# kondratevakate/mri-epilepsy-diagnosis

Measured on AMD Instinct MI355X. Metric: MRI volumes/sec (fwd+bwd) 3D U-Net @160x192x160, higher is better.
Workload: dtype f32; 1 GPU; unet.UNet(c0=8, 3 enc blocks, BN+PReLU, trilinear) fwd+softmax-Dice+bwd+AdamW, batch 2 x 1x160x192x160 fp32 per GPU (BASELINE configs[1]); global_batch=2, parallelism=dp1, launch=eager

## Files before the change

### include/mri3d.h

```cpp
#ifndef MRI3D_H
#define MRI3D_H

#include <stddef.h>
#include <stdint.h>

#ifdef __cplusplus
extern "C" {
#endif

typedef void* mri3d_stream_t;

enum { MRI3D_OK = 0, MRI3D_EINVAL = -1, MRI3D_ENOTSUP = -2, MRI3D_ELAUNCH = -3, MRI3D_EWORKSPACE = -4 };
enum { MRI3D_F32 = 0, MRI3D_BF16 = 1 };
enum { MRI3D_ACT_NONE = 0, MRI3D_ACT_RELU = 1, MRI3D_ACT_LEAKY = 2, MRI3D_ACT_PRELU = 3 };
enum { MRI3D_UP_NEAREST = 0, MRI3D_UP_TRILINEAR = 1 };
enum { MRI3D_PASS_FWD = 0, MRI3D_PASS_DGRAD = 1, MRI3D_PASS_WGRAD = 2 };

int mri3d_version(void);
const char* mri3d_last_error(void);

typedef struct Mri3dConvGeom {
    int32_t n;
    int32_t di, hi, wi, ci;
    int32_t dout, ho, wo, co;
    int32_t kd, kh, kw;
    int32_t sd, sh, sw;
    int32_t pd, ph, pw;
    int32_t dd, dh, dw;
    int32_t x_ld, y_ld;
    int32_t dtype;
} Mri3dConvGeom;

size_t mri3d_conv3d_workspace_bytes(const Mri3dConvGeom* g, int pass);

int mri3d_conv3d_fwd(const Mri3dConvGeom* g, const void* x, const void* w, const void* bias, void* y,
                     void* workspace, size_t ws_bytes, mri3d_stream_t stream);
int32_t mri3d_conv3d_fwd_stats_blocks(const Mri3dConvGeom* g);
int mri3d_conv3d_fwd_stats(const Mri3dConvGeom* g, const void* x, const void* w, const void* bias, void* y,
                           double* stat_partials, void* workspace, size_t ws_bytes, mri3d_stream_t stream);
int mri3d_conv3d_dgrad(const Mri3dConvGeom* g, const void* dy, const void* w, const void* bias, void* dx,
                       void* workspace, size_t ws_bytes, mri3d_stream_t stream);
int mri3d_conv3d_wgrad(const Mri3dConvGeom* g, const void* x, const void* dy, void* dw, void* dbias,
                       void* workspace, size_t ws_bytes, mri3d_stream_t stream);

int32_t mri3d_conv3d_cat_supported(const Mri3dConvGeom* g, int32_t split, int32_t second_ld, int32_t pass);
int32_t mri3d_conv3d_fwd_cat_stats_blocks(const Mri3dConvGeom* g, int32_t split, int32_t second_ld);
int mri3d_conv3d_fwd_cat(const Mri3dConvGeom* g, const void* x, const void* x2, int32_t split, int32_t x2_ld, const void* w,
                         const void* bias, void* y, double* stat_partials, void* workspace, size_t ws_bytes,
                         mri3d_stream_t stream);
int mri3d_conv3d_dgrad_cat(const Mri3dConvGeom* g, const void* dy, const void* w, void* dx, void* dx2, int32_t split,
                           int32_t dx2_ld, void* workspace, size_t ws_bytes, mri3d_stream_t stream);
int mri3d_conv3d_wgrad_cat(const Mri3dConvGeom* g, const void* x, const void* x2, int32_t split, int32_t x2_ld, const void* dy,
                           void* dw, void* dbias, void* workspace, size_t ws_bytes, mri3d_stream_t stream);

int32_t mri3d_conv3d_march_supported(const Mri3dConvGeom* g, int32_t pass);
int32_t mri3d_conv3d_march_stats_blocks(const Mri3dConvGeom* g);
int mri3d_conv3d_fwd_march(const Mri3dConvGeom* g, const void* x, const void* x2, int32_t split, int32_t x2_ld, const void* w,
                           const void* bias, void* y, double* stat_partials, void* workspace, size_t ws_bytes,
                           mri3d_stream_t stream);
int mri3d_conv3d_dgrad_march(const Mri3dConvGeom* g, const void* dy, const void* w, void* dx, void* dx2, int32_t split,
                             int32_t dx2_ld, void* workspace, size_t ws_bytes, mri3d_stream_t stream);

int32_t mri3d_upconv3d_supported(const Mri3dConvGeom* g, int32_t scale);
size_t mri3d_upconv3d_workspace_bytes(const Mri3dConvGeom* g, int32_t scale);
int mri3d_upconv3d_fwd(const Mri3dConvGeom* g, int32_t scale, const void* x, const float* w, const float* bias, void* y,
                       mri3d_stream_t stream);
int mri3d_upconv3d_dgrad(const Mri3dConvGeom* g, int32_t scale, const void* dy, const float* w, void* dx, mri3d_stream_t stream);
int mri3d_upconv3d_wgrad(const Mri3dConvGeom* g, int32_t scale, const void* x, const void* dy, float* dw, float* dbias,
                         void* workspace, size_t ws_bytes, mri3d_stream_t stream);

int32_t mri3d_convpair_supported(const Mri3dConvGeom* first, const Mri3dConvGeom* second);
size_t mri3d_convpair_workspace_bytes(const Mri3dConvGeom* first, const Mri3dConvGeom* second);
int mri3d_convpair_wgrad_first(const Mri3dConvGeom* first, const Mri3dConvGeom* second, const void* x, const void* dy2, const float* w2,
                               float* dw1, float* dbias1, void* workspace, size_t ws_bytes, mri3d_stream_t stream);

typedef struct Mri3dNormGeom {
    int32_t n;
    int64_t vox;
    int32_t c;
    int32_t x_ld;
    int32_t y_ld;
    int32_t instance;
    int32_t act;
    int32_t alpha_n;
    float slope;
    float eps;
    int32_t group_c;
    int32_t dtype;
} Mri3dNormGeom;

size_t mri3d_norm_workspace_bytes(const Mri3dNormGeom* g);

int mri3d_norm_stats(const Mri3dNormGeom* g, const void* x, float* mean, float* invstd,
                     float* running_mean, float* running_var, float momentum,
                     void* workspace, size_t ws_bytes, mri3d_stream_t stream);
int mri3d_norm_stats_from_partials(const Mri3dNormGeom* g, const double* partials, int32_t nblk, const float* shift,
                                   float* mean, float* invstd, float* running_mean, float* running_var, float momentum,
                                   mri3d_stream_t stream);
int mri3d_norm_act_fwd(const Mri3dNormGeom* g, const void* x, const float* mean, const float* invstd,
                       const float* gamma, const float* beta, const float* alpha, void* y,
                       mri3d_stream_t stream);
int mri3d_norm_act_bwd(const Mri3dNormGeom* g, int training, const void* x, const void* dy,
                       const float* mean, const float* invstd, const float* gamma, const float* beta,
                       const float* alpha, void* dx, float* dgamma, float* dbeta, float* dalpha,
                       void* workspace, size_t ws_bytes, mri3d_stream_t stream);

typedef struct Mri3dPoolGeom {
    int32_t n, di, hi, wi, dout, ho, wo, c;
    int32_t kd, kh, kw, sd, sh, sw, pd, ph, pw;
    int32_t x_ld, y_ld;
    int32_t dtype;
} Mri3dPoolGeom;
int mri3d_maxpool3d_fwd(const Mri3dPoolGeom* g, const void* x, void* y, uint8_t* idx, mri3d_stream_t stream);
int mri3d_maxpool3d_bwd(const Mri3dPoolGeom* g, const void* dy, const uint8_t* idx, void* dx, mri3d_stream_t stream);
int mri3d_maxpool3d_bwd_add(const Mri3dPoolGeom* g, const void* dy, const uint8_t* idx, const void* addend,
                            int32_t addend_ld, void* dx, mri3d_stream_t stream);

typedef struct Mri3dUpGeom {
    int32_t n, di, hi, wi, dout, ho, wo, c;
    int32_t x_ld, y_ld;
    int32_t mode;
    int32_t align_corners;
    float rd, rh, rw;
    int32_t dtype;
} Mri3dUpGeom;
size_t mri3d_upsample3d_workspace_bytes(const Mri3dUpGeom* g);
int mri3d_upsample3d_fwd(const Mri3dUpGeom* g, const void* x, void* y, mri3d_stream_t stream);
int mri3d_upsample3d_bwd(const Mri3dUpGeom* g, const void* dy, void* dx, void* workspace, size_t ws_bytes,
                         mri3d_stream_t stream);

typedef struct Mri3dDiceGeom {
    int32_t n;
    int64_t vox;
    int32_t c, ct;
    int32_t x_ld, t_ld;
    float eps;
    int32_t dtype;
} Mri3dDiceGeom;
size_t mri3d_softmax_dice_workspace_bytes(const Mri3dDiceGeom* g);
int mri3d_softmax_dice_fwd(const Mri3dDiceGeom* g, const void* logits, const void* target, float* loss,
                           float* stats, void* workspace, size_t ws_bytes, mri3d_stream_t stream);
int mri3d_softmax_dice_bwd(const Mri3dDiceGeom* g, const void* logits, const void* target, const float* stats,
                           const float* dloss, void* dlogits, mri3d_stream_t stream);

int mri3d_argmax_u8(const void* logits, uint8_t* out, int64_t nvox, int32_t c, int32_t ld, int32_t dtype,
                    mri3d_stream_t stream);

size_t mri3d_mask_overlap_workspace_bytes(void);
int mri3d_mask_overlap(const uint8_t* pred, const uint8_t* gt, int64_t nvox, int64_t* counts, void* workspace,
                       size_t ws_bytes, mri3d_stream_t stream);

size_t mri3d_order_stats_workspace_bytes(void);
int mri3d_order_stats_f32(const float* x, int64_t n, const int64_t* ranks, int32_t nranks, float* out, void* workspace,
                          size_t ws_bytes, mri3d_stream_t stream);
int mri3d_piecewise_linear_f32(const float* x, float* y, int64_t n, const double* edges, const double* slope,
                               const double* intercept, int32_t nseg, mri3d_stream_t stream);
size_t mri3d_znorm_workspace_bytes(void);
int mri3d_znorm_mean_mask_f32(const float* x, float* y, int64_t n, double* stats, void* workspace, size_t ws_bytes,
                              mri3d_stream_t stream);
int mri3d_crop_or_pad_f32(const float* x, float* y, int32_t outer, int32_t di, int32_t hi, int32_t wi, int32_t dout,
                          int32_t ho, int32_t wo, float fill, mri3d_stream_t stream);

size_t mri3d_surface_distance_workspace_bytes(int32_t d, int32_t h, int32_t w);
int mri3d_surface_distance(const uint8_t* gt, const uint8_t* pred, int32_t d, int32_t h, int32_t w,
                           const double* area_table, double* sums, void* workspace, size_t ws_bytes, mri3d_stream_t stream);
int mri3d_surface_elements(const uint8_t* gt, const uint8_t* pred, int32_t d, int32_t h, int32_t w, int32_t* d2_gt,
                           uint8_t* code_gt, int32_t* d2_pred, uint8_t* code_pred, int64_t capacity, uint64_t* counts,
                           void* workspace, size_t ws_bytes, mri3d_stream_t stream);

int mri3d_extract_patches(const void* volumes, int32_t elem_bytes, int32_t nvol, int32_t d, int32_t h, int32_t w,
                          const int32_t* loc_host, int32_t npatch, int32_t pd, int32_t ph, int32_t pw, void* out,
                          mri3d_stream_t stream);
int mri3d_aggregate_patches_u8(const uint8_t* patches, const int32_t* loc_host, int32_t npatch, int32_t pd, int32_t ph,
                               int32_t pw, int32_t bd, int32_t bh, int32_t bw, uint8_t* out, int32_t nvol, int32_t d,
                               int32_t h, int32_t w, mri3d_stream_t stream);
int mri3d_aggregate_patches_argmax(const void* logits, int32_t c, int32_t ld, int32_t dtype, const int32_t* loc_host,
                                   int32_t npatch, int32_t pd, int32_t ph, int32_t pw, int32_t bd, int32_t bh, int32_t bw,
                                   uint8_t* out, int32_t nvol, int32_t d, int32_t h, int32_t w, mri3d_stream_t stream);

int mri3d_copy_channels(const void* src, void* dst, int64_t nvox, int32_t c, int32_t src_ld, int32_t dst_ld,
                        int32_t dtype, mri3d_stream_t stream);
int mri3d_add_channels(const void* a, const void* b, void* dst, int64_t nvox, int32_t c, int32_t a_ld,
                       int32_t b_ld, int32_t dst_ld, int32_t dtype, mri3d_stream_t stream);
int mri3d_convert_channels(const void* src, int32_t src_dtype, void* dst, int32_t dst_dtype, int64_t nvox, int32_t c,
                           int32_t src_ld, int32_t dst_ld, mri3d_stream_t stream);

int mri3d_adam_step(float* p, const float* g, float* m, float* v, int64_t n, float lr, float beta1, float beta2,
                    float eps, float weight_decay, int32_t step, float grad_scale, int32_t decoupled,
                    mri3d_stream_t stream);

#ifdef __cplusplus
}
#endif
#endif
```

### mri_epilepsy_diagnosis_amd/_lib.py

```python
import ctypes
import os
from ctypes import POINTER, Structure, c_char_p, c_float, c_int32, c_int64, c_size_t, c_uint8, c_void_p

_HERE = os.path.dirname(os.path.abspath(__file__))
LIB_PATH = os.path.join(_HERE, "libmri3d_hip.so")

F32, BF16 = 0, 1
ACT_NONE, ACT_RELU, ACT_LEAKY, ACT_PRELU = 0, 1, 2, 3
UP_NEAREST, UP_TRILINEAR = 0, 1
PASS_FWD, PASS_DGRAD, PASS_WGRAD = 0, 1, 2


class ConvGeom(Structure):
    _fields_ = [(n, c_int32) for n in (
        "n", "di", "hi", "wi", "ci", "dout", "ho", "wo", "co", "kd", "kh", "kw", "sd", "sh", "sw",
        "pd", "ph", "pw", "dd", "dh", "dw", "x_ld", "y_ld", "dtype")]


class NormGeom(Structure):
    _fields_ = [("n", c_int32), ("vox", c_int64), ("c", c_int32), ("x_ld", c_int32), ("y_ld", c_int32),
                ("instance", c_int32), ("act", c_int32), ("alpha_n", c_int32), ("slope", c_float),
                ("eps", c_float), ("group_c", c_int32), ("dtype", c_int32)]


class PoolGeom(Structure):
    _fields_ = [(n, c_int32) for n in (
        "n", "di", "hi", "wi", "dout", "ho", "wo", "c", "kd", "kh", "kw", "sd", "sh", "sw", "pd", "ph", "pw",
        "x_ld", "y_ld", "dtype")]


class UpGeom(Structure):
    _fields_ = [(n, c_int32) for n in ("n", "di", "hi", "wi", "dout", "ho", "wo", "c", "x_ld", "y_ld", "mode",
                                       "align_corners")] + \
               [("rd", c_float), ("rh", c_float), ("rw", c_float), ("dtype", c_int32)]


class DiceGeom(Structure):
    _fields_ = [("n", c_int32), ("vox", c_int64), ("c", c_int32), ("ct", c_int32), ("x_ld", c_int32),
                ("t_ld", c_int32), ("eps", c_float), ("dtype", c_int32)]


_P = c_void_p
_FP = c_void_p

SIGNATURES = {
    "mri3d_version": (c_int32, []),
    "mri3d_last_error": (c_char_p, []),
    "mri3d_conv3d_workspace_bytes": (c_size_t, [POINTER(ConvGeom), c_int32]),
    "mri3d_conv3d_fwd": (c_int32, [POINTER(ConvGeom), _P, _P, _P, _P, _P, c_size_t, _P]),
    "mri3d_conv3d_fwd_stats_blocks": (c_int32, [POINTER(ConvGeom)]),
    "mri3d_conv3d_fwd_stats": (c_int32, [POINTER(ConvGeom), _P, _P, _P, _P, _P, _P, c_size_t, _P]),
    "mri3d_conv3d_dgrad": (c_int32, [POINTER(ConvGeom), _P, _P, _P, _P, _P, c_size_t, _P]),
    "mri3d_conv3d_wgrad": (c_int32, [POINTER(ConvGeom), _P, _P, _P, _P, _P, c_size_t, _P]),
    "mri3d_conv3d_cat_supported": (c_int32, [POINTER(ConvGeom), c_int32, c_int32, c_int32]),
    "mri3d_conv3d_fwd_cat_stats_blocks": (c_int32, [POINTER(ConvGeom), c_int32, c_int32]),
    "mri3d_conv3d_fwd_cat": (c_int32, [POINTER(ConvGeom), _P, _P, c_int32, c_int32, _P, _P, _P, _P, _P, c_size_t, _P]),
    "mri3d_conv3d_dgrad_cat": (c_int32, [POINTER(ConvGeom), _P, _P, _P, _P, c_int32, c_int32, _P, c_size_t, _P]),
    "mri3d_conv3d_wgrad_cat": (c_int32, [POINTER(ConvGeom), _P, _P, c_int32, c_int32, _P, _P, _P, _P, c_size_t, _P]),
    "mri3d_conv3d_march_supported": (c_int32, [POINTER(ConvGeom), c_int32]),
    "mri3d_conv3d_march_stats_blocks": (c_int32, [POINTER(ConvGeom)]),
    "mri3d_conv3d_fwd_march": (c_int32, [POINTER(ConvGeom), _P, _P, c_int32, c_int32, _P, _P, _P, _P, _P, c_size_t, _P]),
    "mri3d_conv3d_dgrad_march": (c_int32, [POINTER(ConvGeom), _P, _P, _P, _P, c_int32, c_int32, _P, c_size_t, _P]),
    "mri3d_upconv3d_supported": (c_int32, [POINTER(ConvGeom), c_int32]),
    "mri3d_upconv3d_workspace_bytes": (c_size_t, [POINTER(ConvGeom), c_int32]),
    "mri3d_upconv3d_fwd": (c_int32, [POINTER(ConvGeom), c_int32, _P, _FP, _FP, _P, _P]),
    "mri3d_upconv3d_dgrad": (c_int32, [POINTER(ConvGeom), c_int32, _P, _FP, _P, _P]),
    "mri3d_upconv3d_wgrad": (c_int32, [POINTER(ConvGeom), c_int32, _P, _P, _FP, _FP, _P, c_size_t, _P]),
    "mri3d_convpair_supported": (c_int32, [POINTER(ConvGeom), POINTER(ConvGeom)]),
    "mri3d_convpair_workspace_bytes": (c_size_t, [POINTER(ConvGeom), POINTER(ConvGeom)]),
    "mri3d_convpair_wgrad_first": (c_int32, [POINTER(ConvGeom), POINTER(ConvGeom), _P, _P, _FP, _FP, _FP, _P, c_size_t, _P]),
    "mri3d_norm_workspace_bytes": (c_size_t, [POINTER(NormGeom)]),
    "mri3d_norm_stats": (c_int32, [POINTER(NormGeom), _P, _FP, _FP, _FP, _FP, c_float, _P, c_size_t, _P]),
    "mri3d_norm_stats_from_partials": (c_int32, [POINTER(NormGeom), _P, c_int32, _FP, _FP, _FP, _FP, _FP, c_float, _P]),
    "mri3d_norm_act_fwd": (c_int32, [POINTER(NormGeom), _P, _FP, _FP, _FP, _FP, _FP, _P, _P]),
    "mri3d_norm_act_bwd": (c_int32, [POINTER(NormGeom), c_int32, _P, _P, _FP, _FP, _FP, _FP, _FP, _P, _FP, _FP, _FP,
                                     _P, c_size_t, _P]),
    "mri3d_maxpool3d_fwd": (c_int32, [POINTER(PoolGeom), _P, _P, _P, _P]),
    "mri3d_maxpool3d_bwd": (c_int32, [POINTER(PoolGeom), _P, _P, _P, _P]),
    "mri3d_maxpool3d_bwd_add": (c_int32, [POINTER(PoolGeom), _P, _P, _P, c_int32, _P, _P]),
    "mri3d_upsample3d_workspace_bytes": (c_size_t, [POINTER(UpGeom)]),
    "mri3d_upsample3d_fwd": (c_int32, [POINTER(UpGeom), _P, _P, _P]),
    "mri3d_upsample3d_bwd": (c_int32, [POINTER(UpGeom), _P, _P, _P, c_size_t, _P]),
    "mri3d_softmax_dice_workspace_bytes": (c_size_t, [POINTER(DiceGeom)]),
    "mri3d_softmax_dice_fwd": (c_int32, [POINTER(DiceGeom), _P, _P, _FP, _FP, _P, c_size_t, _P]),
    "mri3d_softmax_dice_bwd": (c_int32, [POINTER(DiceGeom), _P, _P, _FP, _FP, _P, _P]),
    "mri3d_argmax_u8": (c_int32, [_P, _P, c_int64, c_int32, c_int32, c_int32, _P]),
    "mri3d_mask_overlap_workspace_bytes": (c_size_t, []),
    "mri3d_mask_overlap": (c_int32, [_P, _P, c_int64, _P, _P, c_size_t, _P]),
    "mri3d_order_stats_workspace_bytes": (c_size_t, []),
    "mri3d_order_stats_f32": (c_int32, [_P, c_int64, _P, c_int32, _P, _P, c_size_t, _P]),
    "mri3d_piecewise_linear_f32": (c_int32, [_P, _P, c_int64, _P, _P, _P, c_int32, _P]),
    "mri3d_znorm_workspace_bytes": (c_size_t, []),
    "mri3d_znorm_mean_mask_f32": (c_int32, [_P, _P, c_int64, _P, _P, c_size_t, _P]),
    "mri3d_crop_or_pad_f32": (c_int32, [_P, _P, c_int32, c_int32, c_int32, c_int32, c_int32, c_int32, c_int32, c_float, _P]),
    "mri3d_surface_distance_workspace_bytes": (c_size_t, [c_int32, c_int32, c_int32]),
    "mri3d_surface_distance": (c_int32, [_P, _P, c_int32, c_int32, c_int32, _P, _P, _P, c_size_t, _P]),
    "mri3d_surface_elements": (c_int32, [_P, _P, c_int32, c_int32, c_int32, _P, _P, _P, _P, c_int64, _P, _P, c_size_t, _P]),
    "mri3d_extract_patches": (c_int32, [_P, c_int32, c_int32, c_int32, c_int32, c_int32, _P, c_int32, c_int32, c_int32,
                                        c_int32, _P, _P]),
    "mri3d_aggregate_patches_u8": (c_int32, [_P, _P, c_int32, c_int32, c_int32, c_int32, c_int32, c_int32, c_int32, _P,
                                             c_int32, c_int32, c_int32, c_int32, _P]),
    "mri3d_aggregate_patches_argmax": (c_int32, [_P, c_int32, c_int32, c_int32, _P, c_int32, c_int32, c_int32, c_int32,
                                                 c_int32, c_int32, c_int32, _P, c_int32, c_int32, c_int32, c_int32, _P]),
    "mri3d_copy_channels": (c_int32, [_P, _P, c_int64, c_int32, c_int32, c_int32, c_int32, _P]),
    "mri3d_add_channels": (c_int32, [_P, _P, _P, c_int64, c_int32, c_int32, c_int32, c_int32, c_int32, _P]),
    "mri3d_convert_channels": (c_int32, [_P, c_int32, _P, c_int32, c_int64, c_int32, c_int32, c_int32, _P]),
    "mri3d_adam_step": (c_int32, [_FP, _FP, _FP, _FP, c_int64, c_float, c_float, c_float, c_float, c_float, c_int32,
                                  c_float, c_int32, _P]),
}

_lib = None


class Mri3dError(RuntimeError):
    pass


def lib():
    global _lib
    if _lib is None:
        import torch
        if not os.path.exists(LIB_PATH):
            raise Mri3dError(
                "libmri3d_hip.so not found at %s — run `python -m mri_epilepsy_diagnosis_amd.build` "
                "(or __graft_entry__.build()).  There is no PyTorch fallback for device tensors." % LIB_PATH)
        h = ctypes.CDLL(LIB_PATH)
        for name, (res, args) in SIGNATURES.items():
            fn = getattr(h, name)
            fn.restype = res
            fn.argtypes = args
        _lib = h
    return _lib


def check(rc, what=""):
    if rc != 0:
        msg = lib().mri3d_last_error()
        raise Mri3dError("%s failed (rc=%d): %s" % (what, rc, msg.decode() if msg else "?"))
```

### mri_epilepsy_diagnosis_amd/csrc/api.hip

```cpp
#include "common.h"
#include <string.h>

namespace mri3d {

static thread_local char g_err[512] = "";

void set_error(const char* fmt, ...) {
    va_list ap;
    va_start(ap, fmt);
    vsnprintf(g_err, sizeof(g_err), fmt, ap);
    va_end(ap);
}

size_t conv_generic_workspace_bytes(const Mri3dConvGeom& g, int pass);
int conv_generic_fwd(const Mri3dConvGeom& g, const void* x, const float* w, const float* bias, void* y, void* ws,
                     size_t ws_bytes, hipStream_t s);
int conv_generic_dgrad(const Mri3dConvGeom& g, const void* dy, const float* w, const float* bias, void* dx, void* ws,
                       size_t ws_bytes, hipStream_t s);
int conv_generic_wgrad(const Mri3dConvGeom& g, const void* x, const void* dy, float* dw, float* dbias, void* ws,
                       size_t ws_bytes, hipStream_t s);
bool conv_mfma_supported(const Mri3dConvGeom& g, int pass);
size_t conv_mfma_workspace_bytes(const Mri3dConvGeom& g, int pass);
int conv_mfma_fwd(const Mri3dConvGeom& g, const void* x, const float* w, const float* bias, void* y, void* ws,
                  size_t ws_bytes, hipStream_t s);
int conv_mfma_dgrad(const Mri3dConvGeom& g, const void* dy, const float* w, const float* bias, void* dx, void* ws,
                    size_t ws_bytes, hipStream_t s);
int conv_mfma_wgrad(const Mri3dConvGeom& g, const void* x, const void* dy, float* dw, float* dbias, void* ws,
                    size_t ws_bytes, hipStream_t s);
int conv_mfma_fwd_stat_blocks(const Mri3dConvGeom& g, int split = 0, int second_ld = 0);
bool conv_mfma_cat_supported(const Mri3dConvGeom& g, int split, int second_ld, int pass);
int conv_mfma_fwd_cat(const Mri3dConvGeom& g, const void* x, const void* x2, int split, int x2_ld, const float* w, const float* bias,
                      void* y, double* stat_part, void* ws, size_t ws_bytes, hipStream_t s);
int conv_mfma_dgrad_cat(const Mri3dConvGeom& g, const void* dy, const float* w, void* dx, void* dx2, int split, int dx2_ld, void* ws,
                        size_t ws_bytes, hipStream_t s);
int conv_mfma_wgrad_cat(const Mri3dConvGeom& g, const void* x, const void* x2, int split, int x2_ld, const void* dy, float* dw,
                        float* dbias, void* ws, size_t ws_bytes, hipStream_t s);
int conv_mfma_fwd_stats(const Mri3dConvGeom& g, const void* x, const float* w, const float* bias, void* y, double* stat_part,
                        void* ws, size_t ws_bytes, hipStream_t s);

bool conv_march_takes(const Mri3dConvGeom& g, bool dgrad, bool stats, bool force);
int conv_march_stat_blocks(const Mri3dConvGeom& g, bool force);
int conv_march_run(const Mri3dConvGeom& g, bool dgrad, bool force, const void* in_v, const float* w, const float* bias, void* out_v,
                   void* ws, size_t ws_bytes, hipStream_t s, double* stat_part, const void* second, int split, int second_ld);

bool conv_pointwise_supported(const Mri3dConvGeom& g, int pass);
size_t conv_pointwise_workspace_bytes(const Mri3dConvGeom& g, int pass);
int conv_pointwise_fwd(const Mri3dConvGeom& g, const void* x, const float* w, const float* bias, void* y, hipStream_t s);
int conv_pointwise_dgrad(const Mri3dConvGeom& g, const void* dy, const float* w, const float* bias, void* dx,
                         hipStream_t s);
int conv_pointwise_wgrad(const Mri3dConvGeom& g, const void* x, const void* dy, float* dw, float* dbias, void* ws,
                         size_t ws_bytes, hipStream_t s);


static int conv_check(const Mri3dConvGeom* g, const char* who, int first_ci = -1) {
    MRI3D_REQUIRE(g != nullptr, MRI3D_EINVAL, "%s: null geometry", who);
    MRI3D_REQUIRE(g->dtype == MRI3D_F32 || g->dtype == MRI3D_BF16, MRI3D_ENOTSUP, "%s: unknown dtype %d", who, g->dtype);
    MRI3D_REQUIRE(g->n > 0 && g->di > 0 && g->hi > 0 && g->wi > 0 && g->ci > 0 && g->dout > 0 && g->ho > 0 && g->wo > 0 &&
                      g->co > 0,
                  MRI3D_EINVAL, "%s: empty tensor", who);
    MRI3D_REQUIRE(g->kd > 0 && g->kh > 0 && g->kw > 0 && g->sd > 0 && g->sh > 0 && g->sw > 0 && g->dd > 0 && g->dh > 0 &&
                      g->dw > 0 && g->pd >= 0 && g->ph >= 0 && g->pw >= 0,
                  MRI3D_EINVAL, "%s: bad kernel/stride/padding/dilation", who);
    MRI3D_REQUIRE(g->x_ld >= (first_ci >= 0 ? first_ci : g->ci) && g->y_ld >= g->co, MRI3D_EINVAL, "%s: pitch smaller than channel count", who);
    int ed = (g->di + 2 * g->pd - g->dd * (g->kd - 1) - 1) / g->sd + 1;
    int eh = (g->hi + 2 * g->ph - g->dh * (g->kh - 1) - 1) / g->sh + 1;
    int ew = (g->wi + 2 * g->pw - g->dw * (g->kw - 1) - 1) / g->sw + 1;
    MRI3D_REQUIRE(ed == g->dout && eh == g->ho && ew == g->wo, MRI3D_EINVAL,
                  "%s: output dims (%d,%d,%d) do not match conv arithmetic (%d,%d,%d)", who, g->dout, g->ho, g->wo, ed, eh,
                  ew);
    return MRI3D_OK;
}

}

using namespace mri3d;

extern "C" int mri3d_version(void) { return 100; }
extern "C" const char* mri3d_last_error(void) { return g_err; }

extern "C" size_t mri3d_conv3d_workspace_bytes(const Mri3dConvGeom* g, int pass) {
    if (!g) return 0;
    size_t a = conv_generic_workspace_bytes(*g, pass);
    size_t b = conv_mfma_supported(*g, pass) ? conv_mfma_workspace_bytes(*g, pass) : 0;
    size_t c = conv_pointwise_supported(*g, pass) ? conv_pointwise_workspace_bytes(*g, pass) : 0;
    a = a > b ? a : b;
    return align_up(a > c ? a : c, 256);
}

extern "C" int mri3d_conv3d_fwd(const Mri3dConvGeom* g, const void* x, const void* w, const void* bias, void* y,
                                void* workspace, size_t ws_bytes, mri3d_stream_t stream) {
    int rc = conv_check(g, "conv3d_fwd");
    if (rc) return rc;
    MRI3D_REQUIRE(x && w && y, MRI3D_EINVAL, "conv3d_fwd: null pointer");
    hipStream_t s = static_cast<hipStream_t>(stream);
    if (conv_mfma_supported(*g, MRI3D_PASS_FWD) && aligned16(x, y, workspace))
        return conv_mfma_fwd(*g, x, (const float*)w, (const float*)bias, y, workspace, ws_bytes, s);
    if (conv_pointwise_supported(*g, MRI3D_PASS_FWD) && aligned_vec4(g->dtype, x))
        return conv_pointwise_fwd(*g, x, (const float*)w, (const float*)bias, y, s);
    return conv_generic_fwd(*g, x, (const float*)w, (const float*)bias, y, workspace, ws_bytes, s);
}

extern "C" int32_t mri3d_conv3d_fwd_stats_blocks(const Mri3dConvGeom* g) {
    if (!g || conv_check(g, "conv3d_fwd_stats_blocks") != MRI3D_OK) return 0;
    return conv_mfma_supported(*g, MRI3D_PASS_FWD) ? conv_mfma_fwd_stat_blocks(*g) : 0;
}

extern "C" int mri3d_conv3d_fwd_stats(const Mri3dConvGeom* g, const void* x, const void* w, const void* bias, void* y,
                                      double* stat_partials, void* workspace, size_t ws_bytes, mri3d_stream_t stream) {
    int rc = conv_check(g, "conv3d_fwd_stats");
    if (rc) return rc;
    MRI3D_REQUIRE(x && w && y && stat_partials, MRI3D_EINVAL, "conv3d_fwd_stats: null pointer");
    MRI3D_REQUIRE(conv_mfma_supported(*g, MRI3D_PASS_FWD) && conv_mfma_fwd_stat_blocks(*g) > 0 && aligned16(x, y, workspace),
                  MRI3D_ENOTSUP, "conv3d_fwd_stats: geometry not served by the MFMA forward kernel (query mri3d_conv3d_fwd_stats_blocks)");
    return conv_mfma_fwd_stats(*g, x, (const float*)w, (const float*)bias, y, stat_partials, workspace, ws_bytes,
                               static_cast<hipStream_t>(stream));
}

extern "C" int mri3d_conv3d_dgrad(const Mri3dConvGeom* g, const void* dy, const void* w, const void* bias, void* dx,
                                  void* workspace, size_t ws_bytes, mri3d_stream_t stream) {
    int rc = conv_check(g, "conv3d_dgrad");
    if (rc) return rc;
    MRI3D_REQUIRE(dy && w && dx, MRI3D_EINVAL, "conv3d_dgrad: null pointer");
    hipStream_t s = static_cast<hipStream_t>(stream);
    if (conv_pointwise_supported(*g, MRI3D_PASS_DGRAD) && aligned_vec4(g->dtype, dx))
        return conv_pointwise_dgrad(*g, dy, (const float*)w, (const float*)bias, dx, s);
    if (conv_mfma_supported(*g, MRI3D_PASS_DGRAD) && aligned16(dy, dx, workspace))
        return conv_mfma_dgrad(*g, dy, (const float*)w, (const float*)bias, dx, workspace, ws_bytes, s);
    return conv_generic_dgrad(*g, dy, (const float*)w, (const float*)bias, dx, workspace, ws_bytes, s);
}

extern "C" int32_t mri3d_conv3d_cat_supported(const Mri3dConvGeom* g, int32_t split, int32_t second_ld, int32_t pass) {
    if (!g || split <= 0 || conv_check(g, "conv3d_cat_supported", split) != MRI3D_OK) return 0;
    return conv_mfma_cat_supported(*g, split, second_ld, pass) ? 1 : 0;
}

extern "C" int32_t mri3d_conv3d_fwd_cat_stats_blocks(const Mri3dConvGeom* g, int32_t split, int32_t second_ld) {
    if (!g || split <= 0 || conv_check(g, "conv3d_fwd_cat_stats_blocks", split) != MRI3D_OK) return 0;
    return conv_mfma_cat_supported(*g, split, second_ld, MRI3D_PASS_FWD) ? conv_mfma_fwd_stat_blocks(*g, split, second_ld) : 0;
}

extern "C" int mri3d_conv3d_fwd_cat(const Mri3dConvGeom* g, const void* x, const void* x2, int32_t split, int32_t x2_ld,
                                    const void* w, const void* bias, void* y, double* stat_partials, void* workspace,
                                    size_t ws_bytes, mri3d_stream_t stream) {
    int rc = conv_check(g, "conv3d_fwd_cat", split);
    if (rc) return rc;
    MRI3D_REQUIRE(x && x2 && w && y, MRI3D_EINVAL, "conv3d_fwd_cat: null pointer");
    MRI3D_REQUIRE(conv_mfma_cat_supported(*g, split, x2_ld, MRI3D_PASS_FWD) && aligned16(x, y, workspace) && aligned16(x2),
                  MRI3D_ENOTSUP, "conv3d_fwd_cat: geometry / alignment not served (query mri3d_conv3d_cat_supported)");
    MRI3D_REQUIRE(stat_partials == nullptr || conv_mfma_fwd_stat_blocks(*g, split, x2_ld) > 0, MRI3D_ENOTSUP,
                  "conv3d_fwd_cat: no fused statistics for this geometry (query mri3d_conv3d_fwd_cat_stats_blocks)");
    return conv_mfma_fwd_cat(*g, x, x2, split, x2_ld, (const float*)w, (const float*)bias, y, stat_partials, workspace, ws_bytes,
                             static_cast<hipStream_t>(stream));
}

extern "C" int mri3d_conv3d_dgrad_cat(const Mri3dConvGeom* g, const void* dy, const void* w, void* dx, void* dx2, int32_t split,
                                      int32_t dx2_ld, void* workspace, size_t ws_bytes, mri3d_stream_t stream) {
    int rc = conv_check(g, "conv3d_dgrad_cat", split);
    if (rc) return rc;
    MRI3D_REQUIRE(dy && w && dx && dx2, MRI3D_EINVAL, "conv3d_dgrad_cat: null pointer");
    MRI3D_REQUIRE(conv_mfma_cat_supported(*g, split, dx2_ld, MRI3D_PASS_DGRAD) && aligned16(dy, dx, workspace) && aligned16(dx2),
                  MRI3D_ENOTSUP, "conv3d_dgrad_cat: geometry / alignment not served (query mri3d_conv3d_cat_supported)");
    return conv_mfma_dgrad_cat(*g, dy, (const float*)w, dx, dx2, split, dx2_ld, workspace, ws_bytes, static_cast<hipStream_t>(stream));
}

extern "C" int mri3d_conv3d_wgrad_cat(const Mri3dConvGeom* g, const void* x, const void* x2, int32_t split, int32_t x2_ld,
                                      const void* dy, void* dw, void* dbias, void* workspace, size_t ws_bytes,
                                      mri3d_stream_t stream) {
    int rc = conv_check(g, "conv3d_wgrad_cat", split);
    if (rc) return rc;
    MRI3D_REQUIRE(x && x2 && dy && dw, MRI3D_EINVAL, "conv3d_wgrad_cat: null pointer");
    MRI3D_REQUIRE(conv_mfma_cat_supported(*g, split, x2_ld, MRI3D_PASS_WGRAD) && aligned16(x, dy, workspace) && aligned16(x2),
                  MRI3D_ENOTSUP, "conv3d_wgrad_cat: geometry / alignment not served (query mri3d_conv3d_cat_supported)");
    return conv_mfma_wgrad_cat(*g, x, x2, split, x2_ld, dy, (float*)dw, (float*)dbias, workspace, ws_bytes,
                               static_cast<hipStream_t>(stream));
}

extern "C" int32_t mri3d_conv3d_march_supported(const Mri3dConvGeom* g, int32_t pass) {
    if (!g || (pass != MRI3D_PASS_FWD && pass != MRI3D_PASS_DGRAD) || conv_check(g, "conv3d_march_supported") != MRI3D_OK) return 0;
    return conv_march_takes(*g, pass == MRI3D_PASS_DGRAD, false, true) ? 1 : 0;
}

extern "C" int32_t mri3d_conv3d_march_stats_blocks(const Mri3dConvGeom* g) {
    if (!g || conv_check(g, "conv3d_march_stats_blocks") != MRI3D_OK) return 0;
    return conv_march_stat_blocks(*g, true);
}

extern "C" int mri3d_conv3d_fwd_march(const Mri3dConvGeom* g, const void* x, const void* x2, int32_t split, int32_t x2_ld,
                                      const void* w, const void* bias, void* y, double* stat_partials, void* workspace,
                                      size_t ws_bytes, mri3d_stream_t stream) {
    int rc = conv_check(g, "conv3d_fwd_march", x2 ? split : -1);
    if (rc) return rc;
    MRI3D_REQUIRE(x && w && y, MRI3D_EINVAL, "conv3d_fwd_march: null pointer");
    MRI3D_REQUIRE(x2 == nullptr || (split > 0 && split < g->ci && x2_ld >= g->ci - split), MRI3D_EINVAL, "conv3d_fwd_march: bad split");
    return conv_march_run(*g, false, true, x, (const float*)w, (const float*)bias, y, workspace, ws_bytes,
                          static_cast<hipStream_t>(stream), stat_partials, x2, split, x2_ld);
}

extern "C" int mri3d_conv3d_dgrad_march(const Mri3dConvGeom* g, const void* dy, const void* w, void* dx, void* dx2, int32_t split,
                                        int32_t dx2_ld, void* workspace, size_t ws_bytes, mri3d_stream_t stream) {
    int rc = conv_check(g, "conv3d_dgrad_march", dx2 ? split : -1);
    if (rc) return rc;
    MRI3D_REQUIRE(dy && w && dx, MRI3D_EINVAL, "conv3d_dgrad_march: null pointer");
    MRI3D_REQUIRE(dx2 == nullptr || (split > 0 && split < g->ci && dx2_ld >= g->ci - split), MRI3D_EINVAL, "conv3d_dgrad_march: bad split");
    return conv_march_run(*g, true, true, dy, (const float*)w, nullptr, dx, workspace, ws_bytes, static_cast<hipStream_t>(stream),
                          nullptr, dx2, split, dx2_ld);
}

extern "C" int mri3d_conv3d_wgrad(const Mri3dConvGeom* g, const void* x, const void* dy, void* dw, void* dbias,
                                  void* workspace, size_t ws_bytes, mri3d_stream_t stream) {
    int rc = conv_check(g, "conv3d_wgrad");
    if (rc) return rc;
    MRI3D_REQUIRE(x && dy && dw, MRI3D_EINVAL, "conv3d_wgrad: null pointer");
    hipStream_t s = static_cast<hipStream_t>(stream);
    if (conv_pointwise_supported(*g, MRI3D_PASS_WGRAD) && aligned_vec4(g->dtype, x))
        return conv_pointwise_wgrad(*g, x, dy, (float*)dw, (float*)dbias, workspace, ws_bytes, s);
    if (conv_mfma_supported(*g, MRI3D_PASS_WGRAD) && aligned16(x, dy, workspace))
        return conv_mfma_wgrad(*g, x, dy, (float*)dw, (float*)dbias, workspace, ws_bytes, s);
    return conv_generic_wgrad(*g, x, dy, (float*)dw, (float*)dbias, workspace, ws_bytes, s);
}
```

### mri_epilepsy_diagnosis_amd/csrc/common.h

```cpp
#pragma once
#include <hip/hip_runtime.h>
#include <stdint.h>
#include <stdio.h>
#include <stdarg.h>
#include <stdlib.h>
#include "../../include/mri3d.h"

namespace mri3d {

void set_error(const char* fmt, ...);

inline int check_launch(const char* what) {
    hipError_t e = hipGetLastError();
    if (e != hipSuccess) {
        set_error("%s: launch failed: %s", what, hipGetErrorString(e));
        return MRI3D_ELAUNCH;
    }
    return MRI3D_OK;
}

#define MRI3D_REQUIRE(cond, code, ...)      \
    do {                                    \
        if (!(cond)) {                      \
            ::mri3d::set_error(__VA_ARGS__); \
            return (code);                  \
        }                                   \
    } while (0)

#ifdef MRI3D_TUNING
inline int tuning_knob(const char* name, int dflt) {
    const char* v = getenv(name);
    return v ? atoi(v) : dflt;
}
#else
constexpr int tuning_knob(const char*, int dflt) { return dflt; }
#endif

inline int64_t cdiv64(int64_t a, int64_t b) { return (a + b - 1) / b; }
inline int cdiv(int a, int b) { return (a + b - 1) / b; }
inline size_t align_up(size_t x, size_t a) { return (x + a - 1) / a * a; }

constexpr int kMaxStreamBlocks = 2048;

inline int stream_grid(int64_t work_items, int per_block) {
    int64_t b = cdiv64(work_items, per_block);
    if (b > kMaxStreamBlocks) b = kMaxStreamBlocks;
    if (b < 1) b = 1;
    return (int)b;
}

typedef __bf16 bf16_t;
typedef __attribute__((ext_vector_type(4))) __bf16 bf16x4_t;
typedef __attribute__((ext_vector_type(8))) __bf16 bf16x8_t;

template <typename T> __device__ __forceinline__ float ldf(const T* p) { return (float)*p; }
template <typename T> __device__ __forceinline__ void stf(T* p, float v) { *p = (T)v; }

__device__ __forceinline__ float4 ldf4(const float* p) { return *reinterpret_cast<const float4*>(p); }
__device__ __forceinline__ float4 ldf4(const bf16_t* p) {
    const bf16x4_t v = *reinterpret_cast<const bf16x4_t*>(p);
    return make_float4((float)v[0], (float)v[1], (float)v[2], (float)v[3]);
}
__device__ __forceinline__ void stf4(float* p, float4 v) { *reinterpret_cast<float4*>(p) = v; }
__device__ __forceinline__ void stf4(bf16_t* p, float4 v) {
    bf16x4_t o;
    o[0] = (bf16_t)v.x, o[1] = (bf16_t)v.y, o[2] = (bf16_t)v.z, o[3] = (bf16_t)v.w;
    *reinterpret_cast<bf16x4_t*>(p) = o;
}

inline size_t dtype_size(int dtype) { return dtype == MRI3D_BF16 ? 2 : 4; }
inline bool aligned_vec4(int dtype, const void* a, const void* b = nullptr, const void* c = nullptr) {
    const uintptr_t m = dtype == MRI3D_BF16 ? 7 : 15;
    return ((reinterpret_cast<uintptr_t>(a) | reinterpret_cast<uintptr_t>(b) | reinterpret_cast<uintptr_t>(c)) & m) == 0;
}

inline bool aligned16(const void* a, const void* b = nullptr, const void* c = nullptr) {
    return ((reinterpret_cast<uintptr_t>(a) | reinterpret_cast<uintptr_t>(b) | reinterpret_cast<uintptr_t>(c)) & 15) == 0;
}

#define MRI3D_DISPATCH_DTYPE(dtype, T, ...)  \
    do {                                     \
        if ((dtype) == MRI3D_BF16) {         \
            using T = ::mri3d::bf16_t;       \
            __VA_ARGS__                      \
        } else {                             \
            using T = float;                 \
            __VA_ARGS__                      \
        }                                    \
    } while (0)

__device__ __forceinline__ float wave_sum(float v) {
#pragma unroll
    for (int off = 32; off > 0; off >>= 1) v += __shfl_xor(v, off, 64);
    return v;
}

__device__ __forceinline__ double wave_sum_d(double v) {
#pragma unroll
    for (int off = 32; off > 0; off >>= 1) v += __shfl_xor(v, off, 64);
    return v;
}

__device__ __forceinline__ float apply_act(float v, int act, float slope) {
    if (act == MRI3D_ACT_RELU) return v > 0.f ? v : 0.f;
    if (act == MRI3D_ACT_LEAKY || act == MRI3D_ACT_PRELU) return v > 0.f ? v : v * slope;
    return v;
}

}
```

### mri_epilepsy_diagnosis_amd/csrc/conv_pointwise.hip

```cpp
#include "common.h"

namespace mri3d {

template <typename T, int CO>
__global__ void __launch_bounds__(256)
pw_dgrad_kernel(const T* __restrict__ dy, const float* __restrict__ w, const float* __restrict__ bias,
                T* __restrict__ dx, int64_t nvox, int Ci, int Co, int x_ld, int y_ld) {
    const int QC = Ci >> 2;
    const int q = threadIdx.x % QC, vl = threadIdx.x / QC, VL = 256 / QC;
    float4 wq[CO];
#pragma unroll
    for (int co = 0; co < CO; ++co) {
        const float* wr = w + (size_t)(co < Co ? co : 0) * Ci + 4 * q;
        wq[co] = co < Co ? make_float4(wr[0], wr[1], wr[2], wr[3]) : make_float4(0.f, 0.f, 0.f, 0.f);
    }
    const float4 b4 = bias ? make_float4(bias[4 * q], bias[4 * q + 1], bias[4 * q + 2], bias[4 * q + 3])
                           : make_float4(0.f, 0.f, 0.f, 0.f);
    constexpr int U = 4;
    const int64_t stride = (int64_t)gridDim.x * VL;
    for (int64_t v0 = (int64_t)blockIdx.x * VL + vl; v0 < nvox; v0 += stride * U) {
        float gv[U][CO];
#pragma unroll
        for (int u = 0; u < U; ++u) {
            const int64_t v = v0 + u * stride;
#pragma unroll
            for (int co = 0; co < CO; ++co) gv[u][co] = (v < nvox && co < Co) ? ldf(dy + v * y_ld + co) : 0.f;
        }
#pragma unroll
        for (int u = 0; u < U; ++u) {
            const int64_t v = v0 + u * stride;
            if (v >= nvox) break;
            float4 acc = b4;
#pragma unroll
            for (int co = 0; co < CO; ++co) {
                acc.x = fmaf(gv[u][co], wq[co].x, acc.x);
                acc.y = fmaf(gv[u][co], wq[co].y, acc.y);
                acc.z = fmaf(gv[u][co], wq[co].z, acc.z);
                acc.w = fmaf(gv[u][co], wq[co].w, acc.w);
            }
            stf4(dx + v * x_ld + 4 * q, acc);
        }
    }
}

template <typename T, int CO>
__global__ void __launch_bounds__(256)
pw_fwd_kernel(const T* __restrict__ x, const float* __restrict__ w, const float* __restrict__ bias, T* __restrict__ y,
              int64_t nvox, int Ci, int Co, int x_ld, int y_ld) {
    const int QC = Ci >> 2;
    const int q = threadIdx.x % QC, vl = threadIdx.x / QC, VL = 256 / QC;
    float4 wq[CO];
    float bq[CO];
#pragma unroll
    for (int co = 0; co < CO; ++co) {
        const float* wr = w + (size_t)(co < Co ? co : 0) * Ci + 4 * q;
        wq[co] = co < Co ? make_float4(wr[0], wr[1], wr[2], wr[3]) : make_float4(0.f, 0.f, 0.f, 0.f);
        bq[co] = (bias != nullptr && co < Co) ? bias[co] : 0.f;
    }
    constexpr int U = 4;
    const int64_t stride = (int64_t)gridDim.x * VL;
    for (int64_t v0 = (int64_t)blockIdx.x * VL + vl; v0 < nvox; v0 += stride * U) {
        float4 xv[U];
#pragma unroll
        for (int u = 0; u < U; ++u) {
            const int64_t v = v0 + u * stride;
            xv[u] = ldf4(x + (v < nvox ? v : nvox - 1) * x_ld + 4 * q);
        }
#pragma unroll
        for (int u = 0; u < U; ++u) {
            const int64_t v = v0 + u * stride;
            float acc[CO];
#pragma unroll
            for (int co = 0; co < CO; ++co) {
                float a = xv[u].x * wq[co].x;
                a = fmaf(xv[u].y, wq[co].y, a);
                a = fmaf(xv[u].z, wq[co].z, a);
                a = fmaf(xv[u].w, wq[co].w, a);
                for (int d = 1; d < QC; d <<= 1) a += __shfl_xor(a, d, 64);
                acc[co] = a + bq[co];
            }
            if (q == 0 && v < nvox) {
                T* yp = y + v * y_ld;
#pragma unroll
                for (int co = 0; co < CO; ++co)
                    if (co < Co) stf(yp + co, acc[co]);
            }
        }
    }
}

constexpr int kPwMaxBlocks = 1024;

template <typename T, int CO, int VX, bool DYV>
__global__ void __launch_bounds__(256)
pw_wgrad_kernel(const T* __restrict__ x, const T* __restrict__ dy, double* __restrict__ part,
                double* __restrict__ bias_part, int64_t nvox, int Ci, int Co, int x_ld, int y_ld) {
    extern __shared__ __attribute__((aligned(16))) double redd[];
    const int QC = Ci / VX;
    const int VL = 256 / QC;
    const int tid = threadIdx.x;
    const int q = tid % QC, vl = tid / QC;
    double acc[VX][CO], bsum[CO];
#pragma unroll
    for (int c = 0; c < CO; ++c) {
        bsum[c] = 0.0;
#pragma unroll
        for (int a = 0; a < VX; ++a) acc[a][c] = 0.0;
    }
    if (vl < VL) {
        constexpr int U = 4;
        const int64_t stride = (int64_t)gridDim.x * VL;
        for (int64_t v0 = (int64_t)blockIdx.x * VL + vl; v0 < nvox; v0 += stride * U) {
            float xv[U][VX];
            float gv[U][CO];
#pragma unroll
            for (int u = 0; u < U; ++u) {
                const int64_t v = v0 + u * stride;
                const bool ok = v < nvox;
                const T* xp = x + (ok ? v : 0) * x_ld + VX * q;
                if constexpr (VX == 8) {
                    const bf16x8_t t = *reinterpret_cast<const bf16x8_t*>(xp);
#pragma unroll
                    for (int a = 0; a < 8; ++a) xv[u][a] = ok ? (float)t[a] : 0.f;
                } else {
                    const float4 t = ldf4(xp);
                    xv[u][0] = ok ? t.x : 0.f, xv[u][1] = ok ? t.y : 0.f, xv[u][2] = ok ? t.z : 0.f, xv[u][3] = ok ? t.w : 0.f;
                }
                const T* gp = dy + (ok ? v : 0) * y_ld;
                if constexpr (DYV) {
                    typedef T tvec __attribute__((ext_vector_type(CO)));
                    const tvec t = *reinterpret_cast<const tvec*>(gp);
#pragma unroll
                    for (int c = 0; c < CO; ++c) gv[u][c] = ok ? (float)t[c] : 0.f;
                } else {
#pragma unroll
                    for (int c = 0; c < CO; ++c) gv[u][c] = (ok && c < Co) ? ldf(gp + c) : 0.f;
                }
            }
#pragma unroll
            for (int u = 0; u < U; ++u) {
#pragma unroll
                for (int c = 0; c < CO; ++c) {
#pragma unroll
                    for (int a = 0; a < VX; ++a) acc[a][c] += (double)(xv[u][a] * gv[u][c]);
                    if (q == 0) bsum[c] += (double)gv[u][c];
                }
            }
        }
    }
    constexpr int S = (VX + 1) * CO;
#pragma unroll
    for (int c = 0; c < CO; ++c) {
#pragma unroll
        for (int a = 0; a < VX; ++a) redd[tid * S + a * CO + c] = acc[a][c];
        redd[tid * S + VX * CO + c] = bsum[c];
    }
    __syncthreads();
    for (int o = tid; o < QC * VX * CO; o += 256) {
        const int c = o % CO, a = (o / CO) % VX, qq = o / (VX * CO);
        double s = 0.0;
        for (int l = 0; l < VL; ++l) s += redd[(l * QC + qq) * S + a * CO + c];
        if (c < Co) part[((size_t)blockIdx.x * Co + c) * Ci + VX * qq + a] = s;
    }
    if (bias_part != nullptr && tid < Co) {
        double s = 0.0;
        for (int l = 0; l < VL; ++l) s += redd[(l * QC) * S + VX * CO + tid];
        bias_part[(size_t)blockIdx.x * Co + tid] = s;
    }
}

__global__ void __launch_bounds__(256)
pw_wgrad_reduce_kernel(const double* __restrict__ part, const double* __restrict__ bias_part, float* __restrict__ dw,
                       float* __restrict__ dbias, int nb, int Ci, int Co) {
    __shared__ double red[256];
    const int el = threadIdx.x >> 5, ql = threadIdx.x & 31;
    const int nw = Co * Ci, ntot = nw + (dbias != nullptr ? Co : 0);
    const int i = blockIdx.x * 8 + el;
    double s = 0.0;
    if (i < nw)
        for (int b = ql; b < nb; b += 32) s += part[(size_t)b * nw + i];
    else if (i < ntot)
        for (int b = ql; b < nb; b += 32) s += bias_part[(size_t)b * Co + (i - nw)];
    red[threadIdx.x] = s;
    __syncthreads();
    if (ql == 0 && i < ntot) {
        double t = 0.0;
        for (int k = 0; k < 32; ++k) t += red[el * 32 + k];
        if (i < nw) dw[i] = (float)t;
        else dbias[i - nw] = (float)t;
    }
}

static bool is_pointwise(const Mri3dConvGeom& g) {
    return g.kd == 1 && g.kh == 1 && g.kw == 1 && g.sd == 1 && g.sh == 1 && g.sw == 1 && g.pd == 0 && g.ph == 0 &&
           g.pw == 0;
}

static int pw_blocks(const Mri3dConvGeom& g) {
    const int64_t nvox = (int64_t)g.n * g.dout * g.ho * g.wo;
    const int VL = 256 / (g.ci >> 2);
    int64_t want = cdiv64(nvox, (int64_t)VL * 16);
    return (int)std::max<int64_t>(1, std::min<int64_t>(want, kPwMaxBlocks));
}

bool conv_pointwise_supported(const Mri3dConvGeom& g, int pass) {
    if (!is_pointwise(g) || g.ci % 4 != 0 || g.x_ld % 4 != 0 || g.ci > 256) return false;
    if (pass == MRI3D_PASS_DGRAD) return g.co <= 8 && 256 % (g.ci >> 2) == 0;
    if (pass == MRI3D_PASS_FWD) {
        const int qc = g.ci >> 2;
        return g.co <= 4 && qc >= 1 && qc <= 16 && (qc & (qc - 1)) == 0;
    }
    if (pass == MRI3D_PASS_WGRAD) return g.co <= 8 && g.ci <= 64;
    return false;
}

size_t conv_pointwise_workspace_bytes(const Mri3dConvGeom& g, int pass) {
    if (pass != MRI3D_PASS_WGRAD) return 0;
    return (size_t)pw_blocks(g) * (g.co * g.ci + g.co) * sizeof(double);
}

int conv_pointwise_dgrad(const Mri3dConvGeom& g, const void* dy, const float* w, const float* bias, void* dx,
                         hipStream_t s) {
    MRI3D_REQUIRE(aligned_vec4(g.dtype, dx), MRI3D_EINVAL, "conv3d_dgrad(pointwise): dx must be aligned to 4 elements");
    const int64_t nvox = (int64_t)g.n * g.di * g.hi * g.wi;
    const int VL = 256 / (g.ci >> 2);
    const unsigned grid = (unsigned)std::max<int64_t>(1, std::min<int64_t>(cdiv64(nvox, (int64_t)VL * 4), 2048));
#define PW_DGRAD(CO)                                                                                                   \
    hipLaunchKernelGGL((pw_dgrad_kernel<T, CO>), dim3(grid), dim3(256), 0, s, (const T*)dy, w, bias, (T*)dx, nvox, g.ci, g.co, \
                       g.x_ld, g.y_ld)
    MRI3D_DISPATCH_DTYPE(g.dtype, T, {
        if (g.co <= 2) PW_DGRAD(2);
        else if (g.co <= 4) PW_DGRAD(4);
        else PW_DGRAD(8);
    });
#undef PW_DGRAD
    return check_launch("conv3d_dgrad(pointwise)");
}

int conv_pointwise_fwd(const Mri3dConvGeom& g, const void* x, const float* w, const float* bias, void* y, hipStream_t s) {
    MRI3D_REQUIRE(aligned_vec4(g.dtype, x), MRI3D_EINVAL, "conv3d_fwd(pointwise): x must be aligned to 4 elements");
    const int64_t nvox = (int64_t)g.n * g.di * g.hi * g.wi;
    const int VL = 256 / (g.ci >> 2);
    const unsigned grid = (unsigned)std::max<int64_t>(1, std::min<int64_t>(cdiv64(nvox, (int64_t)VL * 4), 2048));
#define PW_FWD(CO)                                                                                                     \
    hipLaunchKernelGGL((pw_fwd_kernel<T, CO>), dim3(grid), dim3(256), 0, s, (const T*)x, w, bias, (T*)y, nvox, g.ci, g.co,     \
                       g.x_ld, g.y_ld)
    MRI3D_DISPATCH_DTYPE(g.dtype, T, {
        if (g.co <= 2) PW_FWD(2);
        else PW_FWD(4);
    });
#undef PW_FWD
    return check_launch("conv3d_fwd(pointwise)");
}

int conv_pointwise_wgrad(const Mri3dConvGeom& g, const void* x, const void* dy, float* dw, float* dbias, void* ws,
                         size_t ws_bytes, hipStream_t s) {
    const int nb = pw_blocks(g);
    const size_t need = conv_pointwise_workspace_bytes(g, MRI3D_PASS_WGRAD);
    MRI3D_REQUIRE(ws && ws_bytes >= need, MRI3D_EWORKSPACE, "conv3d_wgrad(pointwise): workspace %zu < %zu", ws_bytes, need);
    MRI3D_REQUIRE(aligned_vec4(g.dtype, x) && (reinterpret_cast<uintptr_t>(ws) & 7) == 0, MRI3D_EINVAL,
                  "conv3d_wgrad(pointwise): x must be aligned to 4 elements");
    double* part = static_cast<double*>(ws);
    double* bias_part = dbias ? part + (size_t)nb * g.co * g.ci : nullptr;
    const int64_t nvox = (int64_t)g.n * g.di * g.hi * g.wi;
    const int CO = g.co <= 2 ? 2 : (g.co <= 4 ? 4 : 8);
    const bool v8 = g.dtype == MRI3D_BF16 && g.ci % 8 == 0 && g.x_ld % 8 == 0 && 256 % (g.ci / 8) == 0 && aligned16(x) && CO <= 4;
    const bool dyv = g.co == CO && g.y_ld == CO && (reinterpret_cast<uintptr_t>(dy) & 15) == 0;
    const size_t smem = (size_t)256 * ((v8 ? 8 : 4) + 1) * CO * sizeof(double);
#define PW_WGRAD(CO_, VX_, DV_)                                                                                        \
    do {                                                                                                               \
        auto kern = pw_wgrad_kernel<T, CO_, VX_, DV_>;                                                                 \
        static const hipError_t attr_ = hipFuncSetAttribute(reinterpret_cast<const void*>(kern),                       \
                                                            hipFuncAttributeMaxDynamicSharedMemorySize, 256 * 9 * 8 * 8); \
        (void)attr_;                                                                                                   \
        hipLaunchKernelGGL(kern, dim3(nb), dim3(256), smem, s, (const T*)x, (const T*)dy, part, bias_part, nvox, g.ci,  \
                           g.co, g.x_ld, g.y_ld);                                                                      \
    } while (0)
#define PW_WGRAD_CO(CO_)                                                                                               \
    do {                                                                                                               \
        if constexpr (sizeof(T) == 2 && CO_ <= 4) {                                                                    \
            if (v8 && dyv) { PW_WGRAD(CO_, 8, true); break; }                                                          \
            if (v8) { PW_WGRAD(CO_, 8, false); break; }                                                                \
        }                                                                                                              \
        if (dyv) PW_WGRAD(CO_, 4, true);                                                                               \
        else PW_WGRAD(CO_, 4, false);                                                                                  \
    } while (0)
    MRI3D_DISPATCH_DTYPE(g.dtype, T, {
        if (CO == 2) PW_WGRAD_CO(2);
        else if (CO == 4) PW_WGRAD_CO(4);
        else PW_WGRAD_CO(8);
    });
#undef PW_WGRAD_CO
#undef PW_WGRAD
    hipLaunchKernelGGL(pw_wgrad_reduce_kernel, dim3(cdiv(g.co * g.ci + g.co, 8)), dim3(256), 0, s, part, bias_part, dw, dbias,
                       nb, g.ci, g.co);
    return check_launch("conv3d_wgrad(pointwise)");
}

}
```

### mri_epilepsy_diagnosis_amd/csrc/norm.hip

```cpp
#include "common.h"

namespace mri3d {

struct NormPlan {
    int vec;
    int CL;
    int VT;
    int cy;
    int nblk;
    int groups;
    int64_t gvox;
};

constexpr int kNormMaxBlocks = 1024;
constexpr int kFinQL = 64;

static NormPlan norm_plan(const Mri3dNormGeom& g, bool al, bool al16 = false) {
    NormPlan p;
    p.vec = (g.c % 4 == 0 && g.x_ld % 4 == 0 && g.y_ld % 4 == 0 && al) ? 4 : 1;
    if (p.vec == 4 && g.dtype == MRI3D_BF16 && g.c % 8 == 0 && g.x_ld % 8 == 0 && g.y_ld % 8 == 0 && al16) p.vec = 8;
    int lanes = g.c / p.vec;
    p.CL = lanes < 256 ? lanes : 256;
    p.cy = cdiv(lanes, p.CL);
    p.VT = 256 / p.CL;
// ... 483 lines not shown
extern "C" size_t mri3d_norm_workspace_bytes(const Mri3dNormGeom* g) {
    if (!g) return 0;
    return norm_workspace_floats(*g) * sizeof(float);
}

static int norm_check(const Mri3dNormGeom* g, const char* who) {
    MRI3D_REQUIRE(g != nullptr, MRI3D_EINVAL, "%s: null geometry", who);
    MRI3D_REQUIRE(g->dtype == MRI3D_F32 || g->dtype == MRI3D_BF16, MRI3D_ENOTSUP, "%s: unknown dtype %d", who, g->dtype);
    MRI3D_REQUIRE(g->n > 0 && g->vox > 0 && g->c > 0 && g->x_ld >= g->c && g->y_ld >= g->c, MRI3D_EINVAL,
                  "%s: bad geometry n=%d vox=%lld c=%d x_ld=%d y_ld=%d", who, g->n, (long long)g->vox, g->c, g->x_ld,
                  g->y_ld);
    MRI3D_REQUIRE(g->act != MRI3D_ACT_PRELU || g->alpha_n == 1 || g->alpha_n == g->c, MRI3D_EINVAL,
                  "%s: PReLU alpha_n=%d must be 1 or C=%d", who, g->alpha_n, g->c);
    MRI3D_REQUIRE(g->group_c == 0 || (g->group_c > 0 && g->instance && g->c % g->group_c == 0), MRI3D_EINVAL,
                  "%s: group_c=%d needs instance mode and must divide C=%d", who, g->group_c, g->c);
    return MRI3D_OK;
}

extern "C" int mri3d_norm_stats(const Mri3dNormGeom* g, const void* x, float* mean, float* invstd, float* running_mean,
                                float* running_var, float momentum, void* workspace, size_t ws_bytes,
                                mri3d_stream_t stream) {
    int rc = norm_check(g, "norm_stats");
    if (rc) return rc;
    MRI3D_REQUIRE(x && mean && invstd, MRI3D_EINVAL, "norm_stats: null pointer");
    MRI3D_REQUIRE(workspace && ws_bytes >= mri3d_norm_workspace_bytes(g), MRI3D_EWORKSPACE,
                  "norm_stats: workspace %zu < %zu", ws_bytes, mri3d_norm_workspace_bytes(g));
    hipStream_t s = static_cast<hipStream_t>(stream);
    Mri3dNormGeom gg = *g;
    gg.y_ld = gg.x_ld;
    NormPlan p = norm_plan(gg, aligned_vec4(g->dtype, x));
    double* part = static_cast<double*>(workspace);
    dim3 grid(p.nblk, p.cy, p.groups);
    const int tot = p.groups * g->c;
    MRI3D_DISPATCH_DTYPE(g->dtype, T, {
        const T* xf = static_cast<const T*>(x);
        if (p.vec == 4)
            hipLaunchKernelGGL((norm_stats_kernel<T, 4>), grid, dim3(256), 0, s, xf, part, g->c, g->x_ld, p.gvox, p.CL, p.VT);
        else if (p.vec == 1)
            hipLaunchKernelGGL((norm_stats_kernel<T, 1>), grid, dim3(256), 0, s, xf, part, g->c, g->x_ld, p.gvox, p.CL, p.VT);
        hipLaunchKernelGGL(norm_stats_finalize_kernel<T>, dim3(cdiv(tot, 256 / kFinQL)), dim3(256), 0, s, xf, part, mean,
                           invstd, running_mean, running_var, momentum, g->eps, g->c, g->x_ld, p.gvox, p.nblk, p.groups);
        if (g->group_c > 0) {
            const int ng = p.groups * (g->c / g->group_c);
            hipLaunchKernelGGL(norm_stats_group_finalize_kernel<T>, dim3(cdiv(ng, 64)), dim3(64), 0, s, xf, part, mean,
                               invstd, g->eps, g->c, g->x_ld, p.gvox, p.nblk, p.groups, g->group_c);
        }
    });
    return check_launch("norm_stats");
}

extern "C" int mri3d_norm_stats_from_partials(const Mri3dNormGeom* g, const double* partials, int32_t nblk, const float* shift,
                                              float* mean, float* invstd, float* running_mean, float* running_var,
                                              float momentum, mri3d_stream_t stream) {
    int rc = norm_check(g, "norm_stats_from_partials");
    if (rc) return rc;
    MRI3D_REQUIRE(partials && mean && invstd && nblk > 0, MRI3D_EINVAL, "norm_stats_from_partials: null pointer / no partials");
    MRI3D_REQUIRE(!g->instance && g->group_c == 0, MRI3D_ENOTSUP,
                  "norm_stats_from_partials: batch statistics only (one group over N x voxels)");
    hipStream_t s = static_cast<hipStream_t>(stream);
    const int64_t gvox = (int64_t)g->n * g->vox;
    hipLaunchKernelGGL(norm_stats_finalize_kernel<float>, dim3(cdiv(g->c, 256 / kFinQL)), dim3(256), 0, s,
                       static_cast<const float*>(nullptr), partials, mean, invstd, running_mean, running_var, momentum, g->eps,
                       g->c, g->x_ld, gvox, nblk, 1, shift, 1);
    return check_launch("norm_stats_from_partials");
}

extern "C" int mri3d_norm_act_fwd(const Mri3dNormGeom* g, const void* x, const float* mean, const float* invstd,
                                  const float* gamma, const float* beta, const float* alpha, void* y,
                                  mri3d_stream_t stream) {
    int rc = norm_check(g, "norm_act_fwd");
    if (rc) return rc;
    MRI3D_REQUIRE(x && y, MRI3D_EINVAL, "norm_act_fwd: null pointer");
    MRI3D_REQUIRE((mean == nullptr) == (invstd == nullptr), MRI3D_EINVAL, "norm_act_fwd: mean/invstd must both be set");
    MRI3D_REQUIRE(g->act != MRI3D_ACT_PRELU || alpha, MRI3D_EINVAL, "norm_act_fwd: PReLU needs alpha");
    hipStream_t s = static_cast<hipStream_t>(stream);
    NormPlan p = norm_plan(*g, aligned_vec4(g->dtype, x, y), aligned16(x, y));
    dim3 grid(p.nblk, p.cy, p.groups);
    MRI3D_DISPATCH_DTYPE(g->dtype, T, {
        const T* xf = static_cast<const T*>(x);
        T* yf = static_cast<T*>(y);
        if constexpr (sizeof(T) == 2) {
            if (p.vec == 8) hipLaunchKernelGGL((norm_act_fwd_kernel<T, 8>), grid, dim3(256), 0, s, xf, yf, mean, invstd, gamma, beta, alpha,
                               g->alpha_n, g->act, g->slope, g->c, g->x_ld, g->y_ld, p.gvox, p.CL, p.VT);
        }
        if (p.vec == 4)
            hipLaunchKernelGGL((norm_act_fwd_kernel<T, 4>), grid, dim3(256), 0, s, xf, yf, mean, invstd, gamma, beta, alpha,
                               g->alpha_n, g->act, g->slope, g->c, g->x_ld, g->y_ld, p.gvox, p.CL, p.VT);
        else if (p.vec == 1)
            hipLaunchKernelGGL((norm_act_fwd_kernel<T, 1>), grid, dim3(256), 0, s, xf, yf, mean, invstd, gamma, beta, alpha,
                               g->alpha_n, g->act, g->slope, g->c, g->x_ld, g->y_ld, p.gvox, p.CL, p.VT);
    });
    return check_launch("norm_act_fwd");
}

extern "C" int mri3d_norm_act_bwd(const Mri3dNormGeom* g, int training, const void* x, const void* dy,
                                  const float* mean, const float* invstd, const float* gamma, const float* beta,
                                  const float* alpha, void* dx, float* dgamma, float* dbeta, float* dalpha,
                                  void* workspace, size_t ws_bytes, mri3d_stream_t stream) {
    int rc = norm_check(g, "norm_act_bwd");
    if (rc) return rc;
    MRI3D_REQUIRE(x && dy && dx, MRI3D_EINVAL, "norm_act_bwd: null pointer");
    MRI3D_REQUIRE((mean == nullptr) == (invstd == nullptr), MRI3D_EINVAL, "norm_act_bwd: mean/invstd must both be set");
    MRI3D_REQUIRE(!(training && mean == nullptr), MRI3D_EINVAL, "norm_act_bwd: training mode needs statistics");
    MRI3D_REQUIRE(g->act != MRI3D_ACT_PRELU || alpha, MRI3D_EINVAL, "norm_act_bwd: PReLU needs alpha");
    MRI3D_REQUIRE(workspace && ws_bytes >= mri3d_norm_workspace_bytes(g), MRI3D_EWORKSPACE,
                  "norm_act_bwd: workspace %zu < %zu", ws_bytes, mri3d_norm_workspace_bytes(g));
    hipStream_t s = static_cast<hipStream_t>(stream);
    NormPlan p = norm_plan(*g, aligned_vec4(g->dtype, x, dy, dx));
    dim3 grid(p.nblk, p.cy, p.groups);
    double* part = static_cast<double*>(workspace);
    float* sums = reinterpret_cast<float*>(part + (size_t)p.groups * p.nblk * g->c * 3);
    const bool need_reduce = training || dgamma || dbeta || dalpha;
    bool params_done = false;
    MRI3D_DISPATCH_DTYPE(g->dtype, T, {
        const T* xf = static_cast<const T*>(x);
        const T* df = static_cast<const T*>(dy);
        T* of = static_cast<T*>(dx);
        if (need_reduce) {
            if (p.vec == 4)
                hipLaunchKernelGGL((norm_act_bwd_reduce_kernel<T, 4>), grid, dim3(256), 0, s, xf, df, part, mean, invstd,
                                   gamma, beta, alpha, g->alpha_n, g->act, g->slope, g->c, g->x_ld, g->y_ld, p.gvox, p.CL,
                                   p.VT);
            else if (p.vec == 1)
                hipLaunchKernelGGL((norm_act_bwd_reduce_kernel<T, 1>), grid, dim3(256), 0, s, xf, df, part, mean, invstd,
                                   gamma, beta, alpha, g->alpha_n, g->act, g->slope, g->c, g->x_ld, g->y_ld, p.gvox, p.CL,
                                   p.VT);
            hipLaunchKernelGGL(norm_act_bwd_sums_kernel, dim3(cdiv(p.groups * g->c, 256 / kFinQL)), dim3(256), 0, s, part,
                               sums, g->c, p.nblk, p.groups);
            if ((dgamma || dbeta || dalpha) && g->group_c > 0) {
                hipLaunchKernelGGL(norm_act_bwd_params_kernel, dim3(1), dim3(256), 0, s, sums, dgamma, dbeta, dalpha,
                                   g->alpha_n, g->c, p.groups);
                params_done = true;
            }
            if (g->group_c > 0 && training) {
                const int ng = p.groups * (g->c / g->group_c);
                hipLaunchKernelGGL(norm_act_bwd_group_combine_kernel, dim3(cdiv(ng, 64)), dim3(64), 0, s, sums, gamma,
                                   g->c, p.groups, g->group_c);
            }
        }
        float* pg = params_done ? nullptr : dgamma;
        float* pb = params_done ? nullptr : dbeta;
        float* pa = params_done ? nullptr : dalpha;
        if (p.vec == 4)
            hipLaunchKernelGGL((norm_act_bwd_apply_kernel<T, 4>), grid, dim3(256), 0, s, xf, df, of, sums, mean, invstd,
                               gamma, beta, alpha, g->alpha_n, g->act, g->slope, training, g->c, g->x_ld, g->y_ld, p.gvox,
                               p.CL, p.VT, g->group_c, pg, pb, pa);
        else if (p.vec == 1)
            hipLaunchKernelGGL((norm_act_bwd_apply_kernel<T, 1>), grid, dim3(256), 0, s, xf, df, of, sums, mean, invstd,
                               gamma, beta, alpha, g->alpha_n, g->act, g->slope, training, g->c, g->x_ld, g->y_ld, p.gvox,
                               p.CL, p.VT, g->group_c, pg, pb, pa);
    });
    return check_launch("norm_act_bwd");
}
```

### mri_epilepsy_diagnosis_amd/csrc/resample.hip

```cpp
#include "common.h"
#include <limits.h>
#include <algorithm>
#include <stdlib.h>

namespace mri3d {

template <int VEC>
struct V {
    float v[VEC];
    template <typename T>
    __device__ __forceinline__ void load(const T* p) {
        if constexpr (VEC == 8) {
            const bf16x8_t t = *reinterpret_cast<const bf16x8_t*>(p);
#pragma unroll
            for (int j = 0; j < 8; ++j) v[j] = (float)t[j];
        } else if constexpr (VEC == 4) {
            float4 t = ldf4(p);
            v[0] = t.x; v[1] = t.y; v[2] = t.z; v[3] = t.w;
        } else {
            v[0] = ldf(p);
        }
    }
    template <typename T>
    __device__ __forceinline__ void store(T* p) const {
        if constexpr (VEC == 8) {
            bf16x8_t o;
#pragma unroll
            for (int j = 0; j < 8; ++j) o[j] = (bf16_t)v[j];
            *reinterpret_cast<bf16x8_t*>(p) = o;
        } else if constexpr (VEC == 4) stf4(p, make_float4(v[0], v[1], v[2], v[3]));
        else stf(p, v[0]);
    }
};


template <typename T, int VEC>
__global__ void __launch_bounds__(256)
maxpool_fwd_kernel(Mri3dPoolGeom g, const T* __restrict__ x, T* __restrict__ y, uint8_t* __restrict__ idx, int hch) {
    const unsigned CV = g.c / VEC;
    const int hchunks = (g.ho + hch - 1) / hch;
    const int slabs = g.n * g.dout * hchunks;
    for (int slab = blockIdx.x; slab < slabs; slab += gridDim.x) {
        const int hc = slab % hchunks, nd = slab / hchunks;
        const int n = nd / g.dout, od = nd - n * g.dout;
        const int h0 = hc * hch, hn = min(hch, g.ho - h0);
        const unsigned inner = (unsigned)hn * g.wo * CV;
        const T* xn = x + (int64_t)n * g.di * g.hi * g.wi * g.x_ld;
        const int64_t obase = ((int64_t)nd * g.ho + h0) * g.wo;
        for (unsigned e = threadIdx.x; e < inner; e += blockDim.x) {
            const unsigned cv = e % CV, pix = e / CV;
            const int ow = pix % g.wo, oh = h0 + pix / g.wo;
            float best[VEC];
            int bi[VEC];
#pragma unroll
            for (int j = 0; j < VEC; ++j) { best[j] = -INFINITY; bi[j] = 0; }
            bool first = true;
            for (int kd = 0; kd < g.kd; ++kd) {
                const int id = od * g.sd - g.pd + kd;
                if ((unsigned)id >= (unsigned)g.di) continue;
                for (int kh = 0; kh < g.kh; ++kh) {
                    const int ih = oh * g.sh - g.ph + kh;
                    if ((unsigned)ih >= (unsigned)g.hi) continue;
                    for (int kw = 0; kw < g.kw; ++kw) {
                        const int iw = ow * g.sw - g.pw + kw;
                        if ((unsigned)iw >= (unsigned)g.wi) continue;
                        V<VEC> xv;
                        xv.load(xn + (((int64_t)id * g.hi + ih) * g.wi + iw) * g.x_ld + cv * VEC);
                        const int tap = (kd * g.kh + kh) * g.kw + kw;
#pragma unroll
                        for (int j = 0; j < VEC; ++j) {
                            if (first || xv.v[j] > best[j] || xv.v[j] != xv.v[j]) {
                                best[j] = xv.v[j];
                                bi[j] = tap;
                            }
                        }
                        first = false;
                    }
                }
            }
            V<VEC> o;
#pragma unroll
            for (int j = 0; j < VEC; ++j) o.v[j] = best[j];
            const int64_t ov = obase + pix;
            o.store(y + ov * g.y_ld + cv * VEC);
            uint8_t* ip = idx + ov * g.c + cv * VEC;
            if constexpr (VEC == 8) {
                uint2 pk;
                pk.x = (uint32_t)bi[0] | ((uint32_t)bi[1] << 8) | ((uint32_t)bi[2] << 16) | ((uint32_t)bi[3] << 24);
                pk.y = (uint32_t)bi[4] | ((uint32_t)bi[5] << 8) | ((uint32_t)bi[6] << 16) | ((uint32_t)bi[7] << 24);
                *reinterpret_cast<uint2*>(ip) = pk;
            } else if constexpr (VEC == 4) {
                *reinterpret_cast<uint32_t*>(ip) = (uint32_t)bi[0] | ((uint32_t)bi[1] << 8) |
                                                   ((uint32_t)bi[VEC > 2 ? 2 : 0] << 16) | ((uint32_t)bi[VEC > 3 ? 3 : 0] << 24);
            } else {
                ip[0] = (uint8_t)bi[0];
            }
        }
    }
}

template <typename T, int VEC>
__global__ void __launch_bounds__(256)
maxpool_bwd_kernel(Mri3dPoolGeom g, const T* __restrict__ dy, const uint8_t* __restrict__ idx,
                   T* __restrict__ dx, int hch, const T* __restrict__ addend, int a_ld) {
    const unsigned CV = g.c / VEC;
    const int hchunks = (g.hi + hch - 1) / hch;
    const int slabs = g.n * g.di * hchunks;
    for (int slab = blockIdx.x; slab < slabs; slab += gridDim.x) {
        const int hc = slab % hchunks, nd = slab / hchunks;
        const int n = nd / g.di, id = nd - n * g.di;
        const int h0 = hc * hch, hn = min(hch, g.hi - h0);
        const unsigned inner = (unsigned)hn * g.wi * CV;
        int od_lo = id + g.pd - g.kd + 1; od_lo = od_lo <= 0 ? 0 : (od_lo + g.sd - 1) / g.sd;
        int od_hi = (id + g.pd) / g.sd; if (od_hi > g.dout - 1) od_hi = g.dout - 1;
        const int64_t ibase = ((int64_t)nd * g.hi + h0) * g.wi;
        for (unsigned e = threadIdx.x; e < inner; e += blockDim.x) {
            const unsigned cv = e % CV, pix = e / CV;
            const int iw = pix % g.wi, ih = h0 + pix / g.wi;
            float acc[VEC];
#pragma unroll
            for (int j = 0; j < VEC; ++j) acc[j] = 0.f;
            if (addend != nullptr) {
                V<VEC> av;
                av.load(addend + (ibase + pix) * a_ld + cv * VEC);
#pragma unroll
                for (int j = 0; j < VEC; ++j) acc[j] = av.v[j];
            }
            int oh_lo = ih + g.ph - g.kh + 1; oh_lo = oh_lo <= 0 ? 0 : (oh_lo + g.sh - 1) / g.sh;
            int oh_hi = (ih + g.ph) / g.sh; if (oh_hi > g.ho - 1) oh_hi = g.ho - 1;
            int ow_lo = iw + g.pw - g.kw + 1; ow_lo = ow_lo <= 0 ? 0 : (ow_lo + g.sw - 1) / g.sw;
            int ow_hi = (iw + g.pw) / g.sw; if (ow_hi > g.wo - 1) ow_hi = g.wo - 1;
            for (int od = od_lo; od <= od_hi; ++od) {
                const int kd = id - (od * g.sd - g.pd);
                for (int oh = oh_lo; oh <= oh_hi; ++oh) {
                    const int kh = ih - (oh * g.sh - g.ph);
                    for (int ow = ow_lo; ow <= ow_hi; ++ow) {
                        const int kw = iw - (ow * g.sw - g.pw);
                        const int tap = (kd * g.kh + kh) * g.kw + kw;
                        const int64_t ov = (((int64_t)n * g.dout + od) * g.ho + oh) * g.wo + ow;
                        V<VEC> gv;
                        gv.load(dy + ov * g.y_ld + cv * VEC);
                        const uint8_t* ip = idx + ov * g.c + cv * VEC;
                        if constexpr (VEC == 8) {
                            const uint2 pk = *reinterpret_cast<const uint2*>(ip);
#pragma unroll
                            for (int j = 0; j < 4; ++j) {
                                if ((int)((pk.x >> (8 * j)) & 0xff) == tap) acc[j] += gv.v[j];
                                if ((int)((pk.y >> (8 * j)) & 0xff) == tap) acc[4 + j] += gv.v[4 + j];
                            }
                        } else if constexpr (VEC == 4) {
                            const uint32_t pk = *reinterpret_cast<const uint32_t*>(ip);
#pragma unroll
                            for (int j = 0; j < VEC; ++j)
                                if ((int)((pk >> (8 * j)) & 0xff) == tap) acc[j] += gv.v[j];
                        } else {
                            if ((int)ip[0] == tap) acc[0] += gv.v[0];
                        }
                    }
                }
            }
            V<VEC> o;
#pragma unroll
            for (int j = 0; j < VEC; ++j) o.v[j] = acc[j];
            o.store(dx + (ibase + pix) * g.x_ld + cv * VEC);
        }
    }
}

template <typename T, int VEC>
__global__ void __launch_bounds__(256)
maxpool2_fwd_kernel(Mri3dPoolGeom g, const T* __restrict__ x, T* __restrict__ y, uint8_t* __restrict__ idx, int hch) {
    const unsigned CV = g.c / VEC;
    const int hchunks = (g.ho + hch - 1) / hch;
    const int slabs = g.n * g.dout * hchunks;
    const unsigned row = (unsigned)g.wi * g.x_ld, plane = (unsigned)g.hi * row;
    for (int slab = blockIdx.x; slab < slabs; slab += gridDim.x) {
        const int hc = slab % hchunks, nd = slab / hchunks;
        const int n = nd / g.dout, od = nd - n * g.dout;
        const int h0 = hc * hch, hn = min(hch, g.ho - h0);
        const unsigned inner = (unsigned)hn * g.wi * CV;
        const T* xs = x + ((int64_t)n * g.di + 2 * od) * g.hi * g.wi * g.x_ld;
        const int64_t obase = ((int64_t)nd * g.ho + h0) * g.wo;
        for (unsigned e0 = 0; e0 < inner; e0 += blockDim.x) {
            const unsigned e = e0 + threadIdx.x;
            const bool live = e < inner;
            const unsigned ee = live ? e : 0;
            const unsigned cv = ee % CV, col = ee / CV;
            const unsigned iw = col % g.wi, ohl = col / g.wi;
            const unsigned kw = iw & 1, ow = iw >> 1, oh = h0 + ohl;
            const T* p0 = xs + (2 * oh) * row + iw * (unsigned)g.x_ld + cv * VEC;
            V<VEC> v[4];
#pragma unroll
            for (int t = 0; t < 4; ++t) v[t].load(p0 + (t >> 1) * plane + (t & 1) * row);
            float best[VEC];
            int bi[VEC];
#pragma unroll
            for (int j = 0; j < VEC; ++j) { best[j] = v[0].v[j]; bi[j] = (int)kw; }
#pragma unroll
            for (int t = 1; t < 4; ++t)
#pragma unroll
                for (int j = 0; j < VEC; ++j)
                    if (v[t].v[j] > best[j] || v[t].v[j] != v[t].v[j]) { best[j] = v[t].v[j]; bi[j] = 2 * t + (int)kw; }
            V<VEC> o;
            int oi[VEC];
#pragma unroll
            for (int j = 0; j < VEC; ++j) {
                const float pb = __shfl_xor(best[j], (int)CV, 64);
                const int pi = __shfl_xor(bi[j], (int)CV, 64);
                const bool mine_nan = best[j] != best[j], his_nan = pb != pb;
                bool take_his;
                if (mine_nan || his_nan) take_his = his_nan && (!mine_nan || pi > bi[j]);
                else take_his = pb > best[j] || (pb == best[j] && pi < bi[j]);
                o.v[j] = take_his ? pb : best[j];
                oi[j] = take_his ? pi : bi[j];
            }
            if (live && kw == 0) {
                const int64_t ov = obase + (int64_t)ohl * g.wo + ow;
                o.store(y + ov * g.y_ld + cv * VEC);
                uint8_t* ip = idx + ov * g.c + cv * VEC;
                if constexpr (VEC == 8) {
                    uint2 pk;
                    pk.x = (uint32_t)oi[0] | ((uint32_t)oi[1] << 8) | ((uint32_t)oi[2] << 16) | ((uint32_t)oi[3] << 24);
                    pk.y = (uint32_t)oi[4] | ((uint32_t)oi[5] << 8) | ((uint32_t)oi[6] << 16) | ((uint32_t)oi[7] << 24);
                    *reinterpret_cast<uint2*>(ip) = pk;
                } else {
                    *reinterpret_cast<uint32_t*>(ip) = (uint32_t)oi[0] | ((uint32_t)oi[1] << 8) | ((uint32_t)oi[2] << 16) | ((uint32_t)oi[3] << 24);
                }
            }
        }
    }
}

static inline bool pool2_ok(const Mri3dPoolGeom& g, int vec) {
    const int cv = g.c / vec;
    return g.kd == 2 && g.kh == 2 && g.kw == 2 && g.sd == 2 && g.sh == 2 && g.sw == 2 && g.pd == 0 && g.ph == 0 && g.pw == 0 &&
           g.di == 2 * g.dout && g.hi == 2 * g.ho && g.wi == 2 * g.wo && cv >= 1 && cv <= 32 && (cv & (cv - 1)) == 0 &&
           (int64_t)g.di * g.hi * g.wi * g.x_ld < ((int64_t)1 << 31);
}

struct Lin { int i0, i1; float l0, l1; };
__device__ __forceinline__ Lin lin_src(int o, float r, int in_size, int align_corners) {
    float src = align_corners ? r * (float)o : fmaf(r, (float)o + 0.5f, -0.5f);
    if (!align_corners && src < 0.f) src = 0.f;
    Lin L;
    L.i0 = (int)src;
    if (L.i0 > in_size - 1) L.i0 = in_size - 1;
    L.i1 = L.i0 + (L.i0 < in_size - 1 ? 1 : 0);
    L.l1 = src - (float)L.i0;
    if (L.l1 < 0.f) L.l1 = 0.f;
    if (L.l1 > 1.f) L.l1 = 1.f;
    L.l0 = 1.f - L.l1;
    return L;
}
__device__ __forceinline__ int near_src(int o, float r, int in_size) {
    int i = (int)floorf((float)o * r);
    return i < in_size - 1 ? i : in_size - 1;
}

template <typename T, int VEC>
__global__ void __launch_bounds__(256)
upsample_fwd_kernel(Mri3dUpGeom g, const T* __restrict__ x, T* __restrict__ y, int hch) {
    const unsigned CV = g.c / VEC;
    const int hchunks = (g.ho + hch - 1) / hch;
    const int slabs = g.n * g.dout * hchunks;
    for (int slab = blockIdx.x; slab < slabs; slab += gridDim.x) {
        const int hc = slab % hchunks, nd = slab / hchunks;
        const int n = nd / g.dout, od = nd - n * g.dout;
        const int h0 = hc * hch, hn = min(hch, g.ho - h0);
        const unsigned inner = (unsigned)hn * g.wo * CV;
        const T* xn = x + (int64_t)n * g.di * g.hi * g.wi * g.x_ld;
        const int64_t obase = ((int64_t)nd * g.ho + h0) * g.wo;
        int idn = 0;
        Lin Ld_ = {0, 0, 1.f, 0.f};
        if (g.mode == MRI3D_UP_NEAREST) idn = near_src(od, g.rd, g.di);
        else Ld_ = lin_src(od, g.rd, g.di, g.align_corners);
        for (unsigned e = threadIdx.x; e < inner; e += blockDim.x) {
            const unsigned cv = e % CV, pix = e / CV;
            const int ow = pix % g.wo, oh = h0 + pix / g.wo;
            const T* xc = xn + cv * VEC;
            V<VEC> o;
            if (g.mode == MRI3D_UP_NEAREST) {
                const int ih = near_src(oh, g.rh, g.hi), iw = near_src(ow, g.rw, g.wi);
                o.load(xc + (((int64_t)idn * g.hi + ih) * g.wi + iw) * g.x_ld);
            } else {
                const Lin Lh = lin_src(oh, g.rh, g.hi, g.align_corners);
                const Lin Lw = lin_src(ow, g.rw, g.wi, g.align_corners);
#pragma unroll
                for (int j = 0; j < VEC; ++j) o.v[j] = 0.f;
#pragma unroll
                for (int a = 0; a < 2; ++a) {
                    const int id = a ? Ld_.i1 : Ld_.i0;
                    const float wd = a ? Ld_.l1 : Ld_.l0;
#pragma unroll
                    for (int b = 0; b < 2; ++b) {
                        const int ih = b ? Lh.i1 : Lh.i0;
                        const float wh = wd * (b ? Lh.l1 : Lh.l0);
#pragma unroll
                        for (int c = 0; c < 2; ++c) {
                            const int iw = c ? Lw.i1 : Lw.i0;
                            const float w = wh * (c ? Lw.l1 : Lw.l0);
                            V<VEC> xv;
                            xv.load(xc + (((int64_t)id * g.hi + ih) * g.wi + iw) * g.x_ld);
#pragma unroll
                            for (int j = 0; j < VEC; ++j) o.v[j] = fmaf(w, xv.v[j], o.v[j]);
                        }
                    }
                }
            }
            o.store(y + (obase + pix) * g.y_ld + cv * VEC);
        }
    }
}

__global__ void upsample_tables_kernel(Mri3dUpGeom g, int* __restrict__ tab) {
    int axis = blockIdx.x;
    int in_size = axis == 0 ? g.di : (axis == 1 ? g.hi : g.wi);
    int out_size = axis == 0 ? g.dout : (axis == 1 ? g.ho : g.wo);
    float r = axis == 0 ? g.rd : (axis == 1 ? g.rh : g.rw);
    int* lo = tab + (axis == 0 ? 0 : (axis == 1 ? 2 * g.di : 2 * g.di + 2 * g.hi));
// ... 383 lines not shown
            const int fwl = pos % (2 * UTW), fhl = pos / (2 * UTW);
            const int hw0 = (fwl >> 1) + 1, hw1 = hw0 + ((fwl & 1) ? 1 : -1), hh0 = (fhl >> 1) + 1, hh1 = hh0 + ((fhl & 1) ? 1 : -1);
            ia[k] = ((hh0 * UHW + hw0) * NPV + pc) * VEC;
            ib[k] = ((hh0 * UHW + hw1) * NPV + pc) * VEC;
            ic[k] = ((hh1 * UHW + hw0) * NPV + pc) * VEC;
            id[k] = ((hh1 * UHW + hw1) * NPV + pc) * VEC;
            const int oh = 2 * h0 + fhl, ow = 2 * w0 + fwl;
            const bool ok = oh < g.ho && ow < g.wo && c0 + pc * VEC < g.c;
            okm |= ok ? (1u << k) : 0u;
            yoff[k] = ok ? (oh * g.wo + ow) * g.y_ld + c0 + pc * VEC : 0;
        }
        T* yn = y + (int64_t)n * g.dout * g.ho * g.wo * g.y_ld;
        const int64_t yplane = (int64_t)g.ho * g.wo * g.y_ld;

        __syncthreads();
        fetch(d0 - 1);
        stash(0);
        __syncthreads();
        V<VEC> pp[NPV];
        for (int c = d0 - 1; c <= d1; ++c) {
            const int buf = (c - (d0 - 1)) & 1;
            if (c < d1) fetch(c + 1);
#pragma unroll
            for (int k = 0; k < NPV; ++k) {
                V<VEC> pc_;
#pragma unroll
                for (int e = 0; e < VEC; e += 4) {
                    const float4 a = *reinterpret_cast<const float4*>(&cbuf[buf][ia[k] + e]);
                    const float4 bq = *reinterpret_cast<const float4*>(&cbuf[buf][ib[k] + e]);
                    const float4 cq = *reinterpret_cast<const float4*>(&cbuf[buf][ic[k] + e]);
                    const float4 dq = *reinterpret_cast<const float4*>(&cbuf[buf][id[k] + e]);
                    pc_.v[e + 0] = 0.75f * fmaf(0.75f, a.x, 0.25f * bq.x) + 0.25f * fmaf(0.75f, cq.x, 0.25f * dq.x);
                    pc_.v[e + 1] = 0.75f * fmaf(0.75f, a.y, 0.25f * bq.y) + 0.25f * fmaf(0.75f, cq.y, 0.25f * dq.y);
                    pc_.v[e + 2] = 0.75f * fmaf(0.75f, a.z, 0.25f * bq.z) + 0.25f * fmaf(0.75f, cq.z, 0.25f * dq.z);
                    pc_.v[e + 3] = 0.75f * fmaf(0.75f, a.w, 0.25f * bq.w) + 0.25f * fmaf(0.75f, cq.w, 0.25f * dq.w);
                }
                if (c >= d0 && ((okm >> k) & 1u)) {
                    V<VEC> o;
                    if (c > d0) {
#pragma unroll
                        for (int e = 0; e < VEC; ++e) o.v[e] = fmaf(0.75f, pp[k].v[e], 0.25f * pc_.v[e]);
                        o.store(yn + (int64_t)(2 * c - 1) * yplane + yoff[k]);
                    }
                    if (c < d1) {
#pragma unroll
                        for (int e = 0; e < VEC; ++e) o.v[e] = fmaf(0.75f, pc_.v[e], 0.25f * pp[k].v[e]);
                        o.store(yn + (int64_t)(2 * c) * yplane + yoff[k]);
                    }
                }
                pp[k] = pc_;
            }
            if (c < d1) stash(buf ^ 1);
            __syncthreads();
        }
    }
}

static inline bool up2x_fast_ok(const Mri3dUpGeom& g) {
    return g.mode == MRI3D_UP_TRILINEAR && !g.align_corners && g.dout == 2 * g.di && g.ho == 2 * g.hi && g.wo == 2 * g.wi &&
           g.rd == 0.5f && g.rh == 0.5f && g.rw == 0.5f && g.c % 4 == 0 && g.x_ld % 4 == 0 && g.y_ld % 4 == 0;
}

static inline void slab_plan(int nd, int h, int w, int cv, int& hch, int& grid) {
    int64_t per_row = (int64_t)w * cv;
    hch = (int)std::max<int64_t>(1, std::min<int64_t>(h, 2048 / std::max<int64_t>(per_row, 1)));
    int64_t slabs = (int64_t)nd * ((h + hch - 1) / hch);
    grid = (int)std::min<int64_t>(slabs, 8192);
}

static inline bool vec_ok(int dtype, int c, int a_ld, int b_ld, const void* a, const void* b) {
    return c % 4 == 0 && a_ld % 4 == 0 && b_ld % 4 == 0 && aligned_vec4(dtype, a, b);
}

}

using namespace mri3d;

static int pool_check(const Mri3dPoolGeom* g, const char* who) {
    MRI3D_REQUIRE(g != nullptr, MRI3D_EINVAL, "%s: null geometry", who);
    MRI3D_REQUIRE(g->dtype == MRI3D_F32 || g->dtype == MRI3D_BF16, MRI3D_ENOTSUP, "%s: unknown dtype %d", who, g->dtype);
    MRI3D_REQUIRE(g->n > 0 && g->c > 0 && g->di > 0 && g->hi > 0 && g->wi > 0 && g->dout > 0 && g->ho > 0 && g->wo > 0,
                  MRI3D_EINVAL, "%s: empty tensor", who);
    MRI3D_REQUIRE(g->kd * g->kh * g->kw <= 256 && g->kd > 0 && g->kh > 0 && g->kw > 0, MRI3D_ENOTSUP,
                  "%s: window volume must be <= 256", who);
    MRI3D_REQUIRE(g->sd > 0 && g->sh > 0 && g->sw > 0 && g->x_ld >= g->c && g->y_ld >= g->c, MRI3D_EINVAL,
                  "%s: bad stride/pitch", who);
    MRI3D_REQUIRE((g->dout - 1) * g->sd - g->pd < g->di && (g->ho - 1) * g->sh - g->ph < g->hi &&
                      (g->wo - 1) * g->sw - g->pw < g->wi && 2 * g->pd <= g->kd && 2 * g->ph <= g->kh && 2 * g->pw <= g->kw,
                  MRI3D_EINVAL, "%s: output dims inconsistent with input", who);
    return MRI3D_OK;
}

extern "C" int mri3d_maxpool3d_fwd(const Mri3dPoolGeom* g, const void* x, void* y, uint8_t* idx,
                                   mri3d_stream_t stream) {
    int rc = pool_check(g, "maxpool3d_fwd");
    if (rc) return rc;
    MRI3D_REQUIRE(x && y && idx, MRI3D_EINVAL, "maxpool3d_fwd: null pointer");
    hipStream_t s = static_cast<hipStream_t>(stream);
    bool v4 = vec_ok(g->dtype, g->c, g->x_ld, g->y_ld, x, y) && (reinterpret_cast<uintptr_t>(idx) & 3) == 0;
    int hch, grid;
    const bool v8 = v4 && g->dtype == MRI3D_BF16 && g->c % 8 == 0 && g->x_ld % 8 == 0 && g->y_ld % 8 == 0 && aligned16(x, y) &&
                    (reinterpret_cast<uintptr_t>(idx) & 7) == 0;
    slab_plan(g->n * g->dout, g->ho, g->wo, g->c / (v8 ? 8 : (v4 ? 4 : 1)), hch, grid);
    if (v4 && pool2_ok(*g, v8 ? 8 : 4)) {
        slab_plan(g->n * g->dout, g->ho, g->wi, g->c / (v8 ? 8 : 4), hch, grid);
        MRI3D_DISPATCH_DTYPE(g->dtype, T, {
            if constexpr (sizeof(T) == 2) {
                if (v8) hipLaunchKernelGGL((maxpool2_fwd_kernel<T, 8>), dim3(grid), dim3(256), 0, s, *g, (const T*)x, (T*)y, idx, hch);
            }
            if (!v8) hipLaunchKernelGGL((maxpool2_fwd_kernel<T, 4>), dim3(grid), dim3(256), 0, s, *g, (const T*)x, (T*)y, idx, hch);
        });
        return check_launch("maxpool3d_fwd");
    }
    MRI3D_DISPATCH_DTYPE(g->dtype, T, {
        if constexpr (sizeof(T) == 2) {
            if (v8) hipLaunchKernelGGL((maxpool_fwd_kernel<T, 8>), dim3(grid), dim3(256), 0, s, *g, (const T*)x, (T*)y, idx, hch);
        }
        if (v8) {
        } else if (v4)
            hipLaunchKernelGGL((maxpool_fwd_kernel<T, 4>), dim3(grid), dim3(256), 0, s, *g, (const T*)x, (T*)y, idx, hch);
        else
            hipLaunchKernelGGL((maxpool_fwd_kernel<T, 1>), dim3(grid), dim3(256), 0, s, *g, (const T*)x, (T*)y, idx, hch);
    });
    return check_launch("maxpool3d_fwd");
}

static int maxpool_bwd_impl(const Mri3dPoolGeom* g, const void* dy, const uint8_t* idx, const void* addend, int32_t a_ld,
                            void* dx, mri3d_stream_t stream) {
    int rc = pool_check(g, "maxpool3d_bwd");
    if (rc) return rc;
    MRI3D_REQUIRE(dy && dx && idx, MRI3D_EINVAL, "maxpool3d_bwd: null pointer");
    MRI3D_REQUIRE(addend == nullptr || a_ld >= g->c, MRI3D_EINVAL, "maxpool3d_bwd: addend pitch %d < %d channels", a_ld, g->c);
    hipStream_t s = static_cast<hipStream_t>(stream);
    bool v4 = vec_ok(g->dtype, g->c, g->x_ld, g->y_ld, dx, dy) && (reinterpret_cast<uintptr_t>(idx) & 3) == 0 &&
              (addend == nullptr || (a_ld % 4 == 0 && aligned_vec4(g->dtype, addend)));
    int hch, grid;
    const bool v8 = v4 && g->dtype == MRI3D_BF16 && g->c % 8 == 0 && g->x_ld % 8 == 0 && g->y_ld % 8 == 0 && aligned16(dx, dy) &&
                    (reinterpret_cast<uintptr_t>(idx) & 7) == 0 && (addend == nullptr || (a_ld % 8 == 0 && aligned16(addend)));
    slab_plan(g->n * g->di, g->hi, g->wi, g->c / (v8 ? 8 : (v4 ? 4 : 1)), hch, grid);
    MRI3D_DISPATCH_DTYPE(g->dtype, T, {
        if constexpr (sizeof(T) == 2) {
            if (v8) hipLaunchKernelGGL((maxpool_bwd_kernel<T, 8>), dim3(grid), dim3(256), 0, s, *g, (const T*)dy, idx, (T*)dx, hch,
                                       (const T*)addend, a_ld);
        }
        if (v8) {
        } else if (v4)
            hipLaunchKernelGGL((maxpool_bwd_kernel<T, 4>), dim3(grid), dim3(256), 0, s, *g, (const T*)dy, idx, (T*)dx, hch,
                               (const T*)addend, a_ld);
        else
            hipLaunchKernelGGL((maxpool_bwd_kernel<T, 1>), dim3(grid), dim3(256), 0, s, *g, (const T*)dy, idx, (T*)dx, hch,
                               (const T*)addend, a_ld);
    });
    return check_launch("maxpool3d_bwd");
}

extern "C" int mri3d_maxpool3d_bwd(const Mri3dPoolGeom* g, const void* dy, const uint8_t* idx, void* dx,
                                   mri3d_stream_t stream) {
    return maxpool_bwd_impl(g, dy, idx, nullptr, 0, dx, stream);
}

extern "C" int mri3d_maxpool3d_bwd_add(const Mri3dPoolGeom* g, const void* dy, const uint8_t* idx, const void* addend,
                                       int32_t addend_ld, void* dx, mri3d_stream_t stream) {
    MRI3D_REQUIRE(addend != nullptr, MRI3D_EINVAL, "maxpool3d_bwd_add: null addend");
    return maxpool_bwd_impl(g, dy, idx, addend, addend_ld, dx, stream);
}

static int up_check(const Mri3dUpGeom* g, const char* who) {
    MRI3D_REQUIRE(g != nullptr, MRI3D_EINVAL, "%s: null geometry", who);
    MRI3D_REQUIRE(g->dtype == MRI3D_F32 || g->dtype == MRI3D_BF16, MRI3D_ENOTSUP, "%s: unknown dtype %d", who, g->dtype);
    MRI3D_REQUIRE(g->n > 0 && g->c > 0 && g->di > 0 && g->hi > 0 && g->wi > 0 && g->dout > 0 && g->ho > 0 && g->wo > 0,
                  MRI3D_EINVAL, "%s: empty tensor", who);
    MRI3D_REQUIRE(g->mode == MRI3D_UP_NEAREST || g->mode == MRI3D_UP_TRILINEAR, MRI3D_EINVAL, "%s: bad mode %d", who,
                  g->mode);
    MRI3D_REQUIRE(g->x_ld >= g->c && g->y_ld >= g->c, MRI3D_EINVAL, "%s: bad pitch", who);
    MRI3D_REQUIRE(g->rd >= 0.f && g->rh >= 0.f && g->rw >= 0.f, MRI3D_EINVAL, "%s: negative scale", who);
    return MRI3D_OK;
}

extern "C" size_t mri3d_upsample3d_workspace_bytes(const Mri3dUpGeom* g) {
    if (!g) return 0;
    return (size_t)2 * (g->di + g->hi + g->wi) * sizeof(int);
}

extern "C" int mri3d_upsample3d_fwd(const Mri3dUpGeom* g, const void* x, void* y, mri3d_stream_t stream) {
    int rc = up_check(g, "upsample3d_fwd");
    if (rc) return rc;
    MRI3D_REQUIRE(x && y, MRI3D_EINVAL, "upsample3d_fwd: null pointer");
    hipStream_t s = static_cast<hipStream_t>(stream);
    static const int no_fast_f = tuning_knob("MRI3D_UP_GENERIC", 0);
    if (!no_fast_f && up2x_fast_ok(*g) && aligned_vec4(g->dtype, x, y)) {
        const bool oct = g->dtype == MRI3D_BF16 && g->c % 8 == 0 && g->x_ld % 8 == 0 && g->y_ld % 8 == 0 &&
                         ((reinterpret_cast<uintptr_t>(x) | reinterpret_cast<uintptr_t>(y)) & 15) == 0;
        const int vec = oct ? 8 : 4, pieces = g->c / vec;
        const int npv = pieces >= 8 ? 8 : pieces >= 4 ? 4 : pieces >= 2 ? 2 : 1;
        const int mtilesH = cdiv(g->hi, UTH), mtilesW = cdiv(g->wi, UTW), mpasses = cdiv(pieces, npv);
        int segl = UMD;
        while (segl > 4 && (int64_t)g->n * cdiv(g->di, segl) * mpasses * mtilesH * mtilesW < 1024) segl /= 2;
        const int segsD = cdiv(g->di, segl);
        const int64_t items = (int64_t)g->n * segsD * mpasses * mtilesH * mtilesW;
        if (items <= 0x7ffffff0 && (int64_t)g->ho * g->wo * g->y_ld <= 0x7fffffff &&
            (int64_t)g->hi * g->wi * g->x_ld <= 0x7fffffff) {
            const int grid = (int)std::min<int64_t>((items + 7) / 8 * 8, 256 * 4 * 8);
#define MRI3D_UPF(Tv, VECv, NPVv)                                                                                      \
    hipLaunchKernelGGL((upsample2x_fwd_march_kernel<Tv, VECv, NPVv>), dim3(grid), dim3(256), 0, s, *g, (const Tv*)x,  \
                       (Tv*)y, segsD, segl, mtilesH, mtilesW, mpasses, (int)items)
#define MRI3D_UPF_N(Tv, VECv)                                                                                          \
    do {                                                                                                              \
        if (npv == 8) MRI3D_UPF(Tv, VECv, 8);                                                                         \
        else if (npv == 4) MRI3D_UPF(Tv, VECv, 4);                                                                    \
        else if (npv == 2) MRI3D_UPF(Tv, VECv, 2);                                                                    \
        else MRI3D_UPF(Tv, VECv, 1);                                                                                  \
    } while (0)
            if (g->dtype == MRI3D_F32) MRI3D_UPF_N(float, 4);
            else if (oct) MRI3D_UPF_N(bf16_t, 8);
            else MRI3D_UPF_N(bf16_t, 4);
#undef MRI3D_UPF_N
#undef MRI3D_UPF
            return check_launch("upsample3d_fwd(2x march)");
        }
    }
    bool v4 = vec_ok(g->dtype, g->c, g->x_ld, g->y_ld, x, y);
    int hch, grid;
    slab_plan(g->n * g->dout, g->ho, g->wo, g->c / (v4 ? 4 : 1), hch, grid);
    MRI3D_DISPATCH_DTYPE(g->dtype, T, {
        if (v4)
            hipLaunchKernelGGL((upsample_fwd_kernel<T, 4>), dim3(grid), dim3(256), 0, s, *g, (const T*)x, (T*)y, hch);
        else
            hipLaunchKernelGGL((upsample_fwd_kernel<T, 1>), dim3(grid), dim3(256), 0, s, *g, (const T*)x, (T*)y, hch);
    });
    return check_launch("upsample3d_fwd");
}

extern "C" int mri3d_upsample3d_bwd(const Mri3dUpGeom* g, const void* dy, void* dx, void* workspace, size_t ws_bytes,
                                    mri3d_stream_t stream) {
    int rc = up_check(g, "upsample3d_bwd");
    if (rc) return rc;
    MRI3D_REQUIRE(dy && dx, MRI3D_EINVAL, "upsample3d_bwd: null pointer");
    MRI3D_REQUIRE(workspace && ws_bytes >= mri3d_upsample3d_workspace_bytes(g), MRI3D_EWORKSPACE,
                  "upsample3d_bwd: workspace %zu < %zu", ws_bytes, mri3d_upsample3d_workspace_bytes(g));
    hipStream_t s = static_cast<hipStream_t>(stream);
    static const int no_fast = tuning_knob("MRI3D_UP_GENERIC", 0);
    if (!no_fast && up2x_fast_ok(*g) && aligned_vec4(g->dtype, dx, dy)) {
        static const int march = tuning_knob("MRI3D_UP_MARCH", 1);
        if (march && g->c % 16 == 0) {
            const int segsD = cdiv(g->di, MD), tilesH = cdiv(g->hi, MTH), tilesW = cdiv(g->wi, MTW), cpasses = g->c / 16;
            const int64_t items = (int64_t)g->n * segsD * cpasses * tilesH * tilesW;
            if (items <= 0x7ffffff0 && (int64_t)g->ho * g->wo * g->y_ld <= 0x7fffffff) {
                const int grid = (int)std::min<int64_t>((items + 7) / 8 * 8, 256 * 3 * 8);
                MRI3D_DISPATCH_DTYPE(g->dtype, T, {
                    hipLaunchKernelGGL(upsample2x_bwd_march_kernel<T>, dim3(grid), dim3(256), 0, s, *g, (const T*)dy, (T*)dx,
                                       segsD, tilesH, tilesW, cpasses, (int)items);
                });
                return check_launch("upsample3d_bwd(2x march)");
            }
        }
        const bool wide = g->c % 16 == 0 && g->dtype == MRI3D_F32;
        const int utd = wide ? Up2Tile<4>::TD : Up2Tile<2>::TD, uth = wide ? Up2Tile<4>::TH : Up2Tile<2>::TH, utw = 16;
        const int tilesD = cdiv(g->di, utd), tilesH = cdiv(g->hi, uth), tilesW = cdiv(g->wi, utw);
        const int64_t nt = (int64_t)g->n * tilesD * tilesH * tilesW;
        if (nt <= 0x7fffffff) {
            const size_t smem = (size_t)(2 * utd + 2) * (2 * uth + 2) * (2 * utw + 2) * (wide ? 4 : 2) * sizeof(float4);
            const int grid = (int)std::min<int64_t>(nt, 2048);
#define MRI3D_UP2B(CQv)                                                                                               \
    {                                                                                                                 \
        auto kern = upsample2x_bwd_kernel<T, CQv>;                                                                    \
        static const hipError_t attr_ = hipFuncSetAttribute(reinterpret_cast<const void*>(kern),                      \
                                                            hipFuncAttributeMaxDynamicSharedMemorySize, (int)smem);   \
        (void)attr_;                   \
        hipLaunchKernelGGL(kern, dim3(grid), dim3(256), smem, s, *g, (const T*)dy, (T*)dx, tilesD, tilesH, tilesW,    \
                           (int)nt);                                                                                  \
    }
            MRI3D_DISPATCH_DTYPE(g->dtype, T, {
                if (wide) MRI3D_UP2B(4) else MRI3D_UP2B(2)
            });
#undef MRI3D_UP2B
            return check_launch("upsample3d_bwd(2x)");
        }
    }
    bool v4 = vec_ok(g->dtype, g->c, g->x_ld, g->y_ld, dx, dy);
    int hch, grid;
    slab_plan(g->n * g->di, g->hi, g->wi, g->c / (v4 ? 4 : 1), hch, grid);
    const int sc = g->di > 0 ? g->dout / g->di : 0;
    if (!no_fast && g->mode == MRI3D_UP_NEAREST && v4 && (sc == 2 || sc == 4) && g->dout == sc * g->di && g->ho == sc * g->hi &&
        g->wo == sc * g->wi) {
        MRI3D_DISPATCH_DTYPE(g->dtype, T, {
            if (sc == 4)
                hipLaunchKernelGGL((upsample_nearest_int_bwd_kernel<T, 4>), dim3(grid), dim3(256), 0, s, *g, (const T*)dy, (T*)dx, hch);
            else
                hipLaunchKernelGGL((upsample_nearest_int_bwd_kernel<T, 2>), dim3(grid), dim3(256), 0, s, *g, (const T*)dy, (T*)dx, hch);
        });
        return check_launch("upsample3d_bwd(nearest, integer scale)");
    }
    int* tab = static_cast<int*>(workspace);
    hipLaunchKernelGGL(upsample_tables_kernel, dim3(3), dim3(256), 0, s, *g, tab);
    MRI3D_DISPATCH_DTYPE(g->dtype, T, {
        if (v4)
            hipLaunchKernelGGL((upsample_bwd_kernel<T, 4>), dim3(grid), dim3(256), 0, s, *g, (const T*)dy, (T*)dx, tab, hch);
        else
            hipLaunchKernelGGL((upsample_bwd_kernel<T, 1>), dim3(grid), dim3(256), 0, s, *g, (const T*)dy, (T*)dx, tab, hch);
    });
    return check_launch("upsample3d_bwd");
}
```

### mri_epilepsy_diagnosis_amd/ops.py

```python
import ctypes
import math

import torch

from . import _lib
from ._lib import (ACT_LEAKY, ACT_NONE, ACT_PRELU, ACT_RELU, BF16, F32, PASS_DGRAD, PASS_FWD, PASS_WGRAD, UP_NEAREST,
                   UP_TRILINEAR, ConvGeom, DiceGeom, NormGeom, PoolGeom, UpGeom, check)

CL3D = torch.channels_last_3d



def _require_device(*ts):
    for t in ts:
        if t is None:
            continue
        if not t.is_cuda:
            raise RuntimeError(
                "mri_epilepsy_diagnosis_amd ops run only on a ROCm device tensor (got %s); there is no CPU fallback"
                % t.device)
        if t.dtype not in (torch.float32, torch.bfloat16):
            raise RuntimeError("mri_epilepsy_diagnosis_amd ops: only float32 / bfloat16 tensors are supported, got %s"
                               % t.dtype)


def _require_param(*ts):
    for t in ts:
        if t is None:
            continue
        _require_device(t)
        if t.dtype != torch.float32:
            raise RuntimeError("mri_epilepsy_diagnosis_amd ops: parameters must be float32, got %s" % t.dtype)


def _dt(t):
    return BF16 if t.dtype == torch.bfloat16 else F32


def _esz(t):
    return 2.0 if t.dtype == torch.bfloat16 else 4.0


_autocast_dtype = None


def autocast_dtype():
    return _autocast_dtype


class autocast:
    def __init__(self, enabled=True, dtype=torch.bfloat16):
        if dtype is not torch.bfloat16:
            raise RuntimeError("mri_epilepsy_diagnosis_amd.autocast: only torch.bfloat16 is supported")
        self.new = dtype if enabled else None

    def __enter__(self):
        global _autocast_dtype
        self.prev = _autocast_dtype
        _autocast_dtype = self.new
        return self

    def __exit__(self, *exc):
        global _autocast_dtype
        _autocast_dtype = self.prev
        return False


def convert(x, dtype):
    return _ConvertFn.apply(x, dtype)


def _convert_raw(x, dtype):
    L = _lib.lib()
    x, x_ld = _nd(x)
    n, c, d, h, w = x.shape
    y = torch.empty(x.shape, dtype=dtype, device=x.device, memory_format=CL3D)
    check(L.mri3d_convert_channels(_ptr(x), _dt(x), _ptr(y), _dt(y), n * d * h * w, c, x_ld, c, _stream()),
          "convert_channels")
    return y


class _ConvertFn(torch.autograd.Function):
    @staticmethod
    def forward(ctx, x, dtype):
        _require_device(x)
        ctx.src_dtype = x.dtype
        if x.dtype == dtype:
            return x.view_as(x)
        return _convert_raw(x, dtype)

    @staticmethod
    def backward(ctx, dy):
        if dy.dtype == ctx.src_dtype:
            return dy, None
        return _convert_raw(dy, ctx.src_dtype), None


def _is_ndhwc_dense(x):
    n, c, d, h, w = x.shape
    exp = (d * h * w * c, 1, h * w * c, w * c, c)
    for dim in range(5):
        if x.shape[dim] > 1 and x.stride(dim) != exp[dim]:
            return False
    return True


def _cl(x):
    if x.dim() != 5:
        raise RuntimeError("expected a 5-D (N,C,D,H,W) tensor, got shape %s" % (tuple(x.shape),))
    if _is_ndhwc_dense(x):
        return x
    return x.contiguous(memory_format=CL3D)


def _pitch_of(x):
    n, c, d, h, w = x.shape
    if c > 1 and x.stride(1) != 1:
        return None
    ld = None
    for size, stride, inner in ((w, x.stride(4), 1), (h, x.stride(3), w), (d, x.stride(2), h * w), (n, x.stride(0), d * h * w)):
        if size > 1:
            if stride % inner:
                return None
            cand = stride // inner
            if ld is None:
                ld = cand
            elif cand != ld:
                return None
    if ld is None:
        ld = c
    return ld if ld >= c else None


def _nd(x):
    if x.dim() != 5:
        raise RuntimeError("expected a 5-D (N,C,D,H,W) tensor, got shape %s" % (tuple(x.shape),))
    ld = _pitch_of(x)
    if ld is not None:
        return x, ld
    x = x.contiguous(memory_format=CL3D)
    return x, x.shape[1]


def _slice_view(buf, off, c):
    return buf.narrow(1, off, c)


def _new(shape, like):
    return torch.empty(shape, dtype=like.dtype, device=like.device, memory_format=CL3D)


def _ptr(t, byte_offset=0):
    if t is None:
        return None
    return ctypes.c_void_p(t.data_ptr() + byte_offset)


def _stream():
    return ctypes.c_void_p(torch.cuda.current_stream().cuda_stream)


_workspaces = {}


def _workspace(nbytes, device):
    key = (device.index, torch.cuda.current_stream(device).cuda_stream)
    ws = _workspaces.get(key)
    if ws is None or ws.numel() < nbytes:
        ws = torch.empty(max(int(nbytes), 1 << 20), dtype=torch.uint8, device=device)
        _workspaces[key] = ws
    return ws


def release_workspaces():
    _workspaces.clear()


class KernelTimer:

    MAX_LIVE = 512

    def __init__(self, only=None):
        self.records = []
        self.only = None if only is None else frozenset(only)
        self.agg = {}

    def fold(self):
        if not self.records:
            return
        torch.cuda.synchronize()
        for tag, work, e0, e1 in self.records:
            a = self.agg.setdefault(tag, {"ms": 0.0, "calls": 0, "work": work})
            a["ms"] += e0.elapsed_time(e1)
            a["calls"] += 1
        self.records.clear()

    def summary(self):
        self.fold()
        return {k: dict(v) for k, v in self.agg.items()}


_timer = None


def set_timer(t):
    global _timer
    _timer = t


_roctx = None


def set_roctx(enabled=True):
    global _roctx
    if not enabled:
        _roctx = None
        return
    h = ctypes.CDLL("libroctx64.so")
    h.roctxRangePushA.argtypes = [ctypes.c_char_p]
    h.roctxRangePushA.restype = ctypes.c_int
    h.roctxRangePop.restype = ctypes.c_int
    _roctx = h


class _timed:

    __slots__ = ("tag_fn", "work_fn", "e0", "tag")

    def __init__(self, tag_fn, work_fn=None):
        self.tag_fn, self.work_fn = tag_fn, work_fn

    def __enter__(self):
        if _timer is None and _roctx is None:
            self.e0 = None
            return
        self.tag = self.tag_fn()
        if _roctx is not None:
            _roctx.roctxRangePushA(self.tag.encode())
        self.e0 = None
        if _timer is not None and (_timer.only is None or self.tag in _timer.only):
            self.e0 = torch.cuda.Event(enable_timing=True)
            self.e0.record()

    def __exit__(self, *exc):
        if _timer is not None and self.e0 is not None:
            e1 = torch.cuda.Event(enable_timing=True)
            e1.record()
            _timer.records.append((self.tag, self.work_fn() if self.work_fn is not None else None, self.e0, e1))
            if len(_timer.records) >= _timer.MAX_LIVE:
                _timer.fold()
        if _roctx is not None:
            _roctx.roctxRangePop()
        return False


def _conv_tag(kind, g):
    def axes(a, b, c):
        return "%d" % a if a == b == c else "%dx%dx%d" % (a, b, c)
    return "conv3d_%s %dx%dx%d s%s d%s %d->%d @%dx%dx%d n%d%s" % (kind, g.kd, g.kh, g.kw, axes(g.sd, g.sh, g.sw),
                                                               axes(g.dd, g.dh, g.dw), g.ci, g.co, g.dout, g.ho, g.wo, g.n,
                                                               " bf16" if g.dtype == BF16 else "")


def _conv_work(g, kind):
    flops = 2.0 * g.n * g.co * g.ci * g.kd * g.kh * g.kw * g.dout * g.ho * g.wo
    esz = 2.0 if g.dtype == BF16 else 4.0
    xin = esz * g.n * g.di * g.hi * g.wi * g.ci
    yout = esz * g.n * g.dout * g.ho * g.wo * g.co
    wts = 4.0 * g.co * g.ci * g.kd * g.kh * g.kw
    return {"flops": flops, "bytes": xin + yout + wts}


def _triple(v):
    if isinstance(v, (tuple, list)):
        if len(v) == 1:
            return (int(v[0]),) * 3
        return tuple(int(a) for a in v)
    return (int(v),) * 3




def _conv_geom(xshape, wshape, stride, padding, dilation, x_ld=None, y_ld=None, dtype=F32):
    n, ci, di, hi, wi = xshape
    co, ci_w, kd, kh, kw = wshape
    if ci_w != ci:
        raise RuntimeError("conv3d: weight expects %d input channels, input has %d (groups are not supported)" % (ci_w, ci))
    sd, sh, sw = stride
    pd, ph, pw = padding
    dd, dh, dw = dilation
    do = (di + 2 * pd - dd * (kd - 1) - 1) // sd + 1
    ho = (hi + 2 * ph - dh * (kh - 1) - 1) // sh + 1
    wo = (wi + 2 * pw - dw * (kw - 1) - 1) // sw + 1
    if do <= 0 or ho <= 0 or wo <= 0:
        raise RuntimeError("Kernel size can't be greater than actual input size")
    return ConvGeom(n, di, hi, wi, ci, do, ho, wo, co, kd, kh, kw, sd, sh, sw, pd, ph, pw, dd, dh, dw,
                    ci if x_ld is None else x_ld, co if y_ld is None else y_ld, dtype)


def _conv_fwd(g, x, w, b):
    L = _lib.lib()
    y = _new((g.n, g.co, g.dout, g.ho, g.wo), x)
    nb = L.mri3d_conv3d_workspace_bytes(ctypes.byref(g), PASS_FWD)
    ws = _workspace(nb, x.device)
    with _timed(lambda: _conv_tag("fwd", g), lambda: _conv_work(g, "fwd")):
        check(L.mri3d_conv3d_fwd(ctypes.byref(g), _ptr(x), _ptr(w), _ptr(b), _ptr(y), _ptr(ws), ws.numel(), _stream()),
              "conv3d_fwd")
    return y


def _conv_dgrad(g, dy, w, b, like):
    L = _lib.lib()
    dx = _new((g.n, g.ci, g.di, g.hi, g.wi), like)
    nb = L.mri3d_conv3d_workspace_bytes(ctypes.byref(g), PASS_DGRAD)
    ws = _workspace(nb, dy.device)
    with _timed(lambda: _conv_tag("dgrad", g), lambda: _conv_work(g, "dgrad")):
        check(L.mri3d_conv3d_dgrad(ctypes.byref(g), _ptr(dy), _ptr(w), _ptr(b), _ptr(dx), _ptr(ws), ws.numel(),
                                   _stream()), "conv3d_dgrad")
    return dx


class GradSink:

    __slots__ = ("view", "fresh")

    def __init__(self, view):
        self.view, self.fresh = view, True


_sinks_suspended = 0


class suspend_grad_sinks:

    def __enter__(self):
        global _sinks_suspended
        _sinks_suspended += 1
        return self

    def __exit__(self, *exc):
        global _sinks_suspended
        _sinks_suspended -= 1
        return False


def _live_sink(param):
    if _sinks_suspended:
        return None
    sink = getattr(param, "_mri3d_grad_sink", None) if param is not None else None
    if sink is None or param.grad is None or param.grad.data_ptr() != sink.view.data_ptr() or sink.view.shape != param.shape:
        return None
    return sink


def _sink_take(param):
    sink = _live_sink(param)
    if sink is None or not sink.fresh:
        return None
    sink.fresh = False
    return sink.view


def _sink_done(param, grad, out):
    if grad is None or out is not None:
        return None
    sink = _live_sink(param)
    if sink is None or sink.view.shape != grad.shape:
        return grad
    sink.view.add_(grad)
    return None


def _conv_wgrad(g, x, dy, w_like, want_bias, dw_out=None, db_out=None):
    L = _lib.lib()
    dw = dw_out if dw_out is not None else torch.empty_like(w_like, memory_format=torch.contiguous_format)
    db = (db_out if db_out is not None else torch.empty(g.co, dtype=w_like.dtype, device=w_like.device)) if want_bias else None
    nb = L.mri3d_conv3d_workspace_bytes(ctypes.byref(g), PASS_WGRAD)
    ws = _workspace(nb, x.device)
    with _timed(lambda: _conv_tag("wgrad", g), lambda: _conv_work(g, "wgrad")):
        check(L.mri3d_conv3d_wgrad(ctypes.byref(g), _ptr(x), _ptr(dy), _ptr(dw), _ptr(db), _ptr(ws), ws.numel(),
                                   _stream()), "conv3d_wgrad")
    return dw, db


def _stuffed_wgrad_ok(g):
    return ((g.kd, g.kh, g.kw) == (3, 3, 3) and (g.sd, g.sh, g.sw) == (2, 2, 2) and (g.pd, g.ph, g.pw) == (1, 1, 1)
            and (g.dd, g.dh, g.dw) == (1, 1, 1) and g.ci % 8 == 0 and g.co % 4 == 0 and g.x_ld % 4 == 0)


class _Conv3dFn(torch.autograd.Function):
    @staticmethod
    def forward(ctx, x, weight, bias, stride, padding, dilation, stats_holder=None):
        _require_device(x)
        _require_param(weight, bias)
        x, x_ld = _nd(x)
        w = weight.contiguous()
        g = _conv_geom(x.shape, w.shape, stride, padding, dilation, x_ld=x_ld, dtype=_dt(x))
        y = None
        if stats_holder is not None:
            L = _lib.lib()
            blocks = L.mri3d_conv3d_fwd_stats_blocks(ctypes.byref(g))
            if blocks > 0:
                y = _new((g.n, g.co, g.dout, g.ho, g.wo), x)
                part = torch.empty(blocks * g.co * 2, dtype=torch.float64, device=x.device)
                ws = _workspace(L.mri3d_conv3d_workspace_bytes(ctypes.byref(g), PASS_FWD), x.device)
                with _timed(lambda: _conv_tag("fwd", g) + " +bn-stats", lambda: _conv_work(g, "fwd")):
                    check(L.mri3d_conv3d_fwd_stats(ctypes.byref(g), _ptr(x), _ptr(w), _ptr(bias), _ptr(y), _ptr(part), _ptr(ws),
                                                   ws.numel(), _stream()), "conv3d_fwd_stats")
                stats_holder.append((part, blocks, bias.detach() if bias is not None else None))
        if y is None:
            y = _conv_fwd(g, x, w, bias)
        ctx.save_for_backward(x, w)
        ctx.geom = g
        ctx.has_bias = bias is not None
        ctx.params = (weight, bias)
        return y

    @staticmethod
    def backward(ctx, dy):
        x, w = ctx.saved_tensors
        g = ctx.geom
        dy, y_ld = _nd(dy)
        dx = dw = db = None
        if ctx.needs_input_grad[0]:
            gd = _conv_geom(x.shape, w.shape, (g.sd, g.sh, g.sw), (g.pd, g.ph, g.pw), (g.dd, g.dh, g.dw), y_ld=y_ld,
                            dtype=g.dtype)
            dx = _conv_dgrad(gd, dy, w, None, x)
        if ctx.needs_input_grad[1] or (ctx.has_bias and ctx.needs_input_grad[2]):
            gw = _conv_geom(x.shape, w.shape, (g.sd, g.sh, g.sw), (g.pd, g.ph, g.pw), (g.dd, g.dh, g.dw), x_ld=g.x_ld,
                            y_ld=y_ld, dtype=g.dtype)
            wp, bp = ctx.params
            want_b = ctx.has_bias and ctx.needs_input_grad[2]
            dw_out = _sink_take(wp) if ctx.needs_input_grad[1] else None
            db_out = _sink_take(bp) if want_b else None
            xw, dyw = x, dy
            if (_stuffed_wgrad_ok(g) and dy.dtype == x.dtype):
                dyw = torch.empty((g.n, g.co, g.di, g.hi, g.wi), dtype=dy.dtype, device=dy.device, memory_format=CL3D).zero_()
                dyw[:, :, ::2, ::2, ::2].copy_(dy)
                gw = _conv_geom(x.shape, w.shape, (1, 1, 1), (1, 1, 1), (1, 1, 1), x_ld=g.x_ld, y_ld=g.co, dtype=g.dtype)
            dw, db = _conv_wgrad(gw, xw, dyw, w, ctx.has_bias, dw_out, db_out)
            dw = _sink_done(wp, dw, dw_out) if ctx.needs_input_grad[1] else None
            db = _sink_done(bp, db, db_out) if want_b else None
        return dx, dw, db, None, None, None, None


class _Conv3dCatFn(torch.autograd.Function):

    @staticmethod
    def forward(ctx, xa, xb, weight, bias, stats_holder=None):
        _require_device(xa, xb)
        _require_param(weight, bias)
        L = _lib.lib()
        xa, a_ld = _nd(xa)
        xb, b_ld = _nd(xb)
        w = weight.contiguous()
        ca, cb = xa.shape[1], xb.shape[1]
        g = _conv_geom((xa.shape[0], ca + cb) + tuple(xa.shape[2:]), w.shape, (1, 1, 1), (1, 1, 1), (1, 1, 1), x_ld=a_ld, dtype=_dt(xa))
        y = _new((g.n, g.co, g.dout, g.ho, g.wo), xa)
        ws = _workspace(L.mri3d_conv3d_workspace_bytes(ctypes.byref(g), PASS_FWD), xa.device)
        part = None
        if stats_holder is not None:
            blocks = L.mri3d_conv3d_fwd_cat_stats_blocks(ctypes.byref(g), ca, b_ld)
            if blocks > 0:
                part = torch.empty(blocks * g.co * 2, dtype=torch.float64, device=xa.device)
                stats_holder.append((part, blocks, bias.detach() if bias is not None else None))
        with _timed(lambda: _conv_tag("fwd", g) + " cat" + (" +bn-stats" if part is not None else ""), lambda: _conv_work(g, "fwd")):
            check(L.mri3d_conv3d_fwd_cat(ctypes.byref(g), _ptr(xa), _ptr(xb), ca, b_ld, _ptr(w), _ptr(bias), _ptr(y), _ptr(part),
                                         _ptr(ws), ws.numel(), _stream()), "conv3d_fwd_cat")
        ctx.save_for_backward(xa, xb, w)
        ctx.geom, ctx.b_ld, ctx.has_bias, ctx.params = g, b_ld, bias is not None, (weight, bias)
        return y

    @staticmethod
    def backward(ctx, dy):
        xa, xb, w = ctx.saved_tensors
        g, L = ctx.geom, _lib.lib()
        dy, y_ld = _nd(dy)
        ca, cb = xa.shape[1], xb.shape[1]
        dxa = dxb = dw = db = None
        if ctx.needs_input_grad[0] or ctx.needs_input_grad[1]:
            gd = _conv_geom((g.n, g.ci, g.di, g.hi, g.wi), w.shape, (1, 1, 1), (1, 1, 1), (1, 1, 1), x_ld=ca, y_ld=y_ld, dtype=g.dtype)
            dxa, dxb = _new(xa.shape, xa), _new(xb.shape, xb)
            ws = _workspace(L.mri3d_conv3d_workspace_bytes(ctypes.byref(gd), PASS_DGRAD), dy.device)
            with _timed(lambda: _conv_tag("dgrad", gd) + " cat", lambda: _conv_work(gd, "dgrad")):
                check(L.mri3d_conv3d_dgrad_cat(ctypes.byref(gd), _ptr(dy), _ptr(w), _ptr(dxa), _ptr(dxb), ca, cb, _ptr(ws),
                                               ws.numel(), _stream()), "conv3d_dgrad_cat")
        if ctx.needs_input_grad[2] or (ctx.has_bias and ctx.needs_input_grad[3]):
            gw = _conv_geom((g.n, g.ci, g.di, g.hi, g.wi), w.shape, (1, 1, 1), (1, 1, 1), (1, 1, 1), x_ld=g.x_ld, y_ld=y_ld, dtype=g.dtype)
            wp, bp = ctx.params
            want_b = ctx.has_bias and ctx.needs_input_grad[3]
            dw_out = _sink_take(wp) if ctx.needs_input_grad[2] else None
            db_out = _sink_take(bp) if want_b else None
            dw = dw_out if dw_out is not None else torch.empty_like(w, memory_format=torch.contiguous_format)
            db = (db_out if db_out is not None else torch.empty(g.co, dtype=w.dtype, device=w.device)) if ctx.has_bias else None
            ws = _workspace(L.mri3d_conv3d_workspace_bytes(ctypes.byref(gw), PASS_WGRAD), dy.device)
            with _timed(lambda: _conv_tag("wgrad", gw) + " cat", lambda: _conv_work(gw, "wgrad")):
                check(L.mri3d_conv3d_wgrad_cat(ctypes.byref(gw), _ptr(xa), _ptr(xb), ca, ctx.b_ld, _ptr(dy), _ptr(dw), _ptr(db), _ptr(ws),
                                               ws.numel(), _stream()), "conv3d_wgrad_cat")
            dw = _sink_done(wp, dw, dw_out) if ctx.needs_input_grad[2] else None
            db = _sink_done(bp, db, db_out) if want_b else None
        return dxa, dxb, dw, db, None


def conv3d_cat(xa, xb, weight, bias=None, padding=1, bn_stats=False):
    if _autocast_dtype is not None:
        xa = convert(xa, _autocast_dtype) if xa.dtype != _autocast_dtype else xa
        xb = convert(xb, _autocast_dtype) if xb.dtype != _autocast_dtype else xb
    ok = (xa.is_cuda and xa.dim() == 5 and xb.shape[0] == xa.shape[0] and xb.shape[2:] == xa.shape[2:] and xa.dtype == xb.dtype
          and tuple(weight.shape[2:]) == (3, 3, 3) and _triple(padding) == (1, 1, 1) and weight.shape[1] == xa.shape[1] + xb.shape[1])
    if ok:
        L = _lib.lib()
        a_nd, a_ld = _nd(xa)
        b_nd, b_ld = _nd(xb)
        ca, cb = xa.shape[1], xb.shape[1]
        shape = (xa.shape[0], ca + cb) + tuple(xa.shape[2:])
        gf = _conv_geom(shape, weight.shape, (1, 1, 1), (1, 1, 1), (1, 1, 1), x_ld=a_ld, dtype=_dt(a_nd))
        gd = _conv_geom(shape, weight.shape, (1, 1, 1), (1, 1, 1), (1, 1, 1), x_ld=ca, dtype=_dt(a_nd))
        ok = (a_nd.data_ptr() % 16 == 0 and b_nd.data_ptr() % 16 == 0
              and L.mri3d_conv3d_cat_supported(ctypes.byref(gf), ca, b_ld, PASS_FWD)
              and L.mri3d_conv3d_cat_supported(ctypes.byref(gf), ca, b_ld, PASS_WGRAD)
              and L.mri3d_conv3d_cat_supported(ctypes.byref(gd), ca, cb, PASS_DGRAD))
    if not ok:
        return conv3d(cat_channels([xa, xb]), weight, bias, 1, padding, 1, bn_stats=bn_stats)
    holder = [] if bn_stats else None
    y = _Conv3dCatFn.apply(xa, xb, weight, bias, holder)
    if holder:
        y._mri3d_bn_stats = holder[0]
    return y


def conv3d(x, weight, bias=None, stride=1, padding=0, dilation=1, bn_stats=False):
    if _autocast_dtype is not None and x.dtype != _autocast_dtype:
        x = convert(x, _autocast_dtype)
    holder = [] if bn_stats else None
    y = _Conv3dFn.apply(x, weight, bias, _triple(stride), _triple(padding), _triple(dilation), holder)
    if holder:
        y._mri3d_bn_stats = holder[0]
    return y


class _ConvPairFn(torch.autograd.Function):

    @staticmethod
    def forward(ctx, x, w1, b1, w2, b2, conv1, conv2):
        _require_device(x)
        _require_param(w1, b1)
        _require_param(w2, b2)
        x, x_ld = _nd(x)
        w1c, w2c = w1.contiguous(), w2.contiguous()
        g1 = _conv_geom(x.shape, w1c.shape, conv1[0], conv1[1], (1, 1, 1), x_ld=x_ld, dtype=_dt(x))
        a1 = _conv_fwd(g1, x, w1c, b1)
        g2 = _conv_geom(a1.shape, w2c.shape, conv2[0], conv2[1], (1, 1, 1), dtype=_dt(x))
        y = _conv_fwd(g2, a1, w2c, b2)
        ctx.save_for_backward(x, a1, w2c)
        ctx.geoms = (g1, g2)
        ctx.params = (w1, b1, w2, b2)
        return y

    @staticmethod
    def backward(ctx, dy):
        L = _lib.lib()
        x, a1, w2c = ctx.saved_tensors
        g1, g2 = ctx.geoms
        w1, b1, w2, b2 = ctx.params
        dy, y_ld = _nd(dy)
        stride2, pad2 = (g2.sd, g2.sh, g2.sw), (g2.pd, g2.ph, g2.pw)
        gw2 = _conv_geom(a1.shape, w2c.shape, stride2, pad2, (1, 1, 1), y_ld=y_ld, dtype=g2.dtype)
        need_w2, need_b2 = ctx.needs_input_grad[3], b2 is not None and ctx.needs_input_grad[4]
        dw2 = db2 = None
        if need_w2 or need_b2:
            dw2_out = _sink_take(w2) if need_w2 else None
            db2_out = _sink_take(b2) if need_b2 else None
            dw2, db2 = _conv_wgrad(gw2, a1, dy, w2c, b2 is not None, dw2_out, db2_out)
            dw2 = _sink_done(w2, dw2, dw2_out) if need_w2 else None
            db2 = _sink_done(b2, db2, db2_out) if need_b2 else None
        need_w1, need_b1 = ctx.needs_input_grad[1], b1 is not None and ctx.needs_input_grad[2]
        dw1 = db1 = None
        if need_w1 or need_b1:
            dw1_out = _sink_take(w1) if need_w1 else None
            db1_out = _sink_take(b1) if need_b1 else None
            dw1 = dw1_out if dw1_out is not None else torch.empty_like(w1, memory_format=torch.contiguous_format)
            db1 = (db1_out if db1_out is not None else torch.empty(g1.co, dtype=w1.dtype, device=w1.device)) if b1 is not None else None
            ws = _workspace(L.mri3d_convpair_workspace_bytes(ctypes.byref(g1), ctypes.byref(gw2)), x.device)
            with _timed(lambda: _conv_tag("wgrad", g1) + " through " + _conv_tag("dgrad", gw2),
                        lambda: {"flops": _conv_work(g1, "wgrad")["flops"] + _conv_work(gw2, "dgrad")["flops"],
                                 "bytes": _esz(dy) * (x.numel() + dy.numel())}):
                check(L.mri3d_convpair_wgrad_first(ctypes.byref(g1), ctypes.byref(gw2), _ptr(x), _ptr(dy), _ptr(w2c), _ptr(dw1), _ptr(db1),
                                                   _ptr(ws), ws.numel(), _stream()), "convpair_wgrad_first")
            dw1 = _sink_done(w1, dw1, dw1_out) if need_w1 else None
            db1 = _sink_done(b1, db1, db1_out) if need_b1 else None
        return None, dw1, db1, dw2, db2, None, None


def conv3d_pair_supported(x, conv1, conv2):
    if not (torch.is_tensor(x) and x.dim() == 5 and x.is_cuda) or x.requires_grad or _autocast_dtype is not None:
        return False
    if _triple(conv1.dilation) != (1, 1, 1) or _triple(conv2.dilation) != (1, 1, 1) or conv1.weight.shape[1] != x.shape[1]:
        return False
    try:
        g1 = _conv_geom(tuple(x.shape), tuple(conv1.weight.shape), _triple(conv1.stride), _triple(conv1.padding), (1, 1, 1),
                        x_ld=_pitch_of(x) or x.shape[1], dtype=_dt(x))
        g2 = _conv_geom((g1.n, g1.co, g1.dout, g1.ho, g1.wo), tuple(conv2.weight.shape), _triple(conv2.stride), _triple(conv2.padding),
                        (1, 1, 1), dtype=_dt(x))
    except RuntimeError:
        return False
    return bool(_lib.lib().mri3d_convpair_supported(ctypes.byref(g1), ctypes.byref(g2)))


def conv3d_pair(x, conv1, conv2):
    if conv3d_pair_supported(x, conv1, conv2):
        return _ConvPairFn.apply(x, conv1.weight, conv1.bias, conv2.weight, conv2.bias,
                                 (_triple(conv1.stride), _triple(conv1.padding)), (_triple(conv2.stride), _triple(conv2.padding)))
    y = conv3d(x, conv1.weight, conv1.bias, conv1.stride, conv1.padding, conv1.dilation)
    return conv3d(y, conv2.weight, conv2.bias, conv2.stride, conv2.padding, conv2.dilation)


def _channel_sum(t):
    L = _lib.lib()
    n, c, d, h, w = t.shape
    g = NormGeom(n, d * h * w, c, c, c, 0, ACT_NONE, 1, 0.0, 0.0, 0, _dt(t))
    mean = torch.empty(c, dtype=torch.float32, device=t.device)
    invstd = torch.empty(c, dtype=torch.float32, device=t.device)
    ws = _workspace(L.mri3d_norm_workspace_bytes(ctypes.byref(g)), t.device)
    check(L.mri3d_norm_stats(ctypes.byref(g), _ptr(t), _ptr(mean), _ptr(invstd), None, None, 0.0, _ptr(ws), ws.numel(),
                             _stream()), "norm_stats")
    return mean * float(n * d * h * w)


class _ConvTranspose3dFn(torch.autograd.Function):

    @staticmethod
    def forward(ctx, x, weight, bias, stride, padding, output_padding, dilation):
        _require_device(x)
        _require_param(weight, bias)
        x = _cl(x)
        w = weight.contiguous()
        n, cin_t, di, hi, wi = x.shape
        if w.shape[0] != cin_t:
            raise RuntimeError("conv_transpose3d: weight expects %d input channels, got %d" % (w.shape[0], cin_t))
        cout_t, kd, kh, kw = w.shape[1], w.shape[2], w.shape[3], w.shape[4]
        od = (di - 1) * stride[0] - 2 * padding[0] + dilation[0] * (kd - 1) + output_padding[0] + 1
        oh = (hi - 1) * stride[1] - 2 * padding[1] + dilation[1] * (kh - 1) + output_padding[1] + 1
        ow = (wi - 1) * stride[2] - 2 * padding[2] + dilation[2] * (kw - 1) + output_padding[2] + 1
        g = _conv_geom((n, cout_t, od, oh, ow), w.shape, stride, padding, dilation, dtype=_dt(x))
        if (g.dout, g.ho, g.wo) != (di, hi, wi):
            raise RuntimeError("conv_transpose3d: inconsistent output_padding")
        y = _conv_dgrad(g, x, w, bias, x)
        ctx.save_for_backward(x, w)
        ctx.geom = g
        ctx.has_bias = bias is not None
        return y

    @staticmethod
    def backward(ctx, dy):
        x, w = ctx.saved_tensors
        g = ctx.geom
        dy = _cl(dy)
        dx = dw = db = None
        if ctx.needs_input_grad[0]:
            dx = _conv_fwd(g, dy, w, None)
        if ctx.needs_input_grad[1]:
            dw, _ = _conv_wgrad(g, dy, x, w, False)
        if ctx.has_bias and ctx.needs_input_grad[2]:
            db = _channel_sum(dy)
        return dx, dw, db, None, None, None, None


def conv_transpose3d(x, weight, bias=None, stride=1, padding=0, output_padding=0, dilation=1):
    if _autocast_dtype is not None and x.dtype != _autocast_dtype:
        x = convert(x, _autocast_dtype)
    return _ConvTranspose3dFn.apply(x, weight, bias, _triple(stride), _triple(padding), _triple(output_padding),
                                    _triple(dilation))



_ACT_CODES = {None: ACT_NONE, "none": ACT_NONE, "relu": ACT_RELU, "leaky_relu": ACT_LEAKY, "prelu": ACT_PRELU}

_sync_bn_reducer = None


def set_sync_batchnorm(reducer):
    global _sync_bn_reducer
    prev, _sync_bn_reducer = _sync_bn_reducer, reducer
    return prev


def sync_batchnorm_reducer():
    return _sync_bn_reducer


class _NormActFn(torch.autograd.Function):

    @staticmethod
    def forward(ctx, x, gamma, beta, alpha, running_mean, running_var, stats_mode, momentum, eps, act, slope, out, group_c=0,
                fused_stats=None):
        _require_device(x)
        _require_param(gamma, beta, alpha)
        ctx.params = (gamma, beta, alpha)
        L = _lib.lib()
        x, x_ld = _nd(x)
        n, c, d, h, w = x.shape
        act_code = _ACT_CODES[act]
        alpha_n = alpha.numel() if (act_code == ACT_PRELU) else 1
        instance = 1 if stats_mode in ("instance", "group") else 0
        if stats_mode == "group" and (group_c <= 0 or c % group_c):
            raise RuntimeError("group norm: channels per group %d must divide C=%d" % (group_c, c))
        group_c = group_c if stats_mode == "group" else 0
        if out is None:
            y, y_ld, y_off = _new(x.shape, x), c, 0
        else:
            buf, y_off = out
            y_ld = _pitch_of(buf)
            if (y_ld != buf.shape[1] or tuple(buf.shape[2:]) != (d, h, w) or buf.shape[0] != n or y_off + c > buf.shape[1]
                    or buf.dtype != x.dtype):
                raise RuntimeError("norm_act(out=): buffer %s cannot hold a %s slice at channel %d"
                                   % (tuple(buf.shape), tuple(x.shape), y_off))
            y = _slice_view(buf, y_off, c)
        g = NormGeom(n, d * h * w, c, x_ld, y_ld, instance, act_code, alpha_n, float(slope), float(eps), group_c, _dt(x))
        mean = invstd = None
        if stats_mode in ("batch", "instance", "group"):
            groups = n if instance else 1
            mean = torch.empty(groups * c, dtype=torch.float32, device=x.device)
            invstd = torch.empty(groups * c, dtype=torch.float32, device=x.device)
            upd = stats_mode == "batch" and running_mean is not None
            if fused_stats is not None and fused_stats[0].numel() == fused_stats[1] * c * 2:
                part, blocks, shift = fused_stats
                with _timed(lambda: "norm_stats(from conv partials) c%d" % c, lambda: {"flops": 0.0, "bytes": 8.0 * part.numel()}):
                    check(L.mri3d_norm_stats_from_partials(ctypes.byref(g), _ptr(part), blocks, _ptr(shift), _ptr(mean),
                                                           _ptr(invstd), _ptr(running_mean) if upd else None,
                                                           _ptr(running_var) if upd else None, float(momentum), _stream()),
                          "norm_stats_from_partials")
            else:
                ws = _workspace(L.mri3d_norm_workspace_bytes(ctypes.byref(g)), x.device)
                with _timed(lambda: "norm_stats c%d vox%d n%d" % (c, g.vox, n), lambda: {"flops": 0.0, "bytes": _esz(x) * x.numel()}):
                    check(L.mri3d_norm_stats(ctypes.byref(g), _ptr(x), _ptr(mean), _ptr(invstd),
                                             _ptr(running_mean) if upd else None, _ptr(running_var) if upd else None,
                                             float(momentum), _ptr(ws), ws.numel(), _stream()), "norm_stats")
        elif stats_mode == "sync":
            reducer = _sync_bn_reducer
            if reducer is None:
                raise RuntimeError("norm_act(stats_mode='sync') needs ops.set_sync_batchnorm(reducer)")
            mean_l = torch.empty(c, dtype=torch.float32, device=x.device)
            invstd_l = torch.empty(c, dtype=torch.float32, device=x.device)
            ws = _workspace(L.mri3d_norm_workspace_bytes(ctypes.byref(g)), x.device)
            with _timed(lambda: "norm_stats c%d vox%d n%d" % (c, g.vox, n), lambda: {"flops": 0.0, "bytes": _esz(x) * x.numel()}):
                check(L.mri3d_norm_stats(ctypes.byref(g), _ptr(x), _ptr(mean_l), _ptr(invstd_l), None, None, float(momentum),
                                         _ptr(ws), ws.numel(), _stream()), "norm_stats")
            cnt_l = float(n * g.vox)
            shift = running_mean.detach().double() if running_mean is not None else torch.zeros(c, dtype=torch.float64, device=x.device)
            m64 = mean_l.double() - shift
            var_l = (1.0 / invstd_l.double() ** 2 - float(eps)).clamp_(min=0.0)
            pack = torch.cat([torch.full((1,), cnt_l, dtype=torch.float64, device=x.device), cnt_l * m64,
                              cnt_l * (var_l + m64 * m64)])
            pack = reducer.all_reduce(pack)
            cnt = pack[0]
            gm_s = pack[1:1 + c] / cnt
            gmean = gm_s + shift
            gvar = (pack[1 + c:] / cnt - gm_s * gm_s).clamp_(min=0.0)
            mean = gmean.to(torch.float32).contiguous()
            invstd = torch.rsqrt(gvar + float(eps)).to(torch.float32).contiguous()
            if running_mean is not None:
                with torch.no_grad():
                    unb = gvar * (cnt / torch.clamp(cnt - 1.0, min=1.0))
                    running_mean.mul_(1.0 - momentum).add_(momentum * gmean.to(running_mean.dtype))
                    running_var.mul_(1.0 - momentum).add_(momentum * unb.to(running_var.dtype))
            ctx.sync_count = cnt
        elif stats_mode == "running":
            mean = running_mean.detach().to(torch.float32).contiguous()
            invstd = torch.rsqrt(running_var.detach().to(torch.float32) + eps).contiguous()
        with _timed(lambda: "norm_act_fwd c%d vox%d n%d" % (c, g.vox, n), lambda: {"flops": 0.0, "bytes": 2 * _esz(x) * x.numel()}):
            check(L.mri3d_norm_act_fwd(ctypes.byref(g), _ptr(x), _ptr(mean), _ptr(invstd), _ptr(gamma), _ptr(beta),
                                       _ptr(alpha) if act_code == ACT_PRELU else None, _ptr(y), _stream()),
                  "norm_act_fwd")
        ctx.save_for_backward(x, mean, invstd, gamma, beta, alpha)
        ctx.geom = g
        ctx.training_stats = stats_mode in ("batch", "instance", "group")
        ctx.sync = _sync_bn_reducer if stats_mode == "sync" else None
        return y

    @staticmethod
    def backward(ctx, dy):
        L = _lib.lib()
        x, mean, invstd, gamma, beta, alpha = ctx.saved_tensors
        g0 = ctx.geom
        dy, dy_ld = _nd(dy)
        dx = _new(x.shape, x) if g0.x_ld == g0.c else None
        if dx is None:
            x = x.contiguous(memory_format=CL3D)
            dx = _new(x.shape, x)
        if dy.dtype != x.dtype:
            raise RuntimeError("norm_act backward: gradient dtype %s does not match activation dtype %s" % (dy.dtype, x.dtype))
        g = NormGeom(g0.n, g0.vox, g0.c, g0.c, dy_ld, g0.instance, g0.act, g0.alpha_n, g0.slope, g0.eps, g0.group_c, g0.dtype)
        pg, pb, pa = ctx.params
        prelu = g.act == ACT_PRELU
        want = (gamma is not None and ctx.needs_input_grad[1], beta is not None and ctx.needs_input_grad[2],
                prelu and ctx.needs_input_grad[3])
        sg = _sink_take(pg) if want[0] else None
        sb = _sink_take(pb) if want[1] else None
        sa = _sink_take(pa) if want[2] else None
        dgamma = (sg if sg is not None else torch.empty_like(gamma)) if want[0] else None
        dbeta = (sb if sb is not None else torch.empty_like(beta)) if want[1] else None
        dalpha = (sa if sa is not None else torch.empty_like(alpha)) if want[2] else None
        sync = ctx.sync
        if sync is not None:
            c_ = g.c
            s1 = dbeta if dbeta is not None else torch.empty(c_, dtype=torch.float32, device=x.device)
            s2 = dgamma if dgamma is not None else torch.empty(c_, dtype=torch.float32, device=x.device)
            dbeta_k, dgamma_k = s1, s2
        else:
            dbeta_k, dgamma_k = dbeta, dgamma
        ws = _workspace(L.mri3d_norm_workspace_bytes(ctypes.byref(g)), x.device)
        with _timed(lambda: "norm_act_bwd c%d vox%d n%d" % (g.c, g.vox, g.n), lambda: {"flops": 0.0, "bytes": 5 * _esz(x) * x.numel()}):
            check(L.mri3d_norm_act_bwd(ctypes.byref(g), 1 if ctx.training_stats else 0, _ptr(x), _ptr(dy), _ptr(mean),
                                       _ptr(invstd), _ptr(gamma), _ptr(beta), _ptr(alpha) if prelu else None, _ptr(dx),
                                       _ptr(dgamma_k), _ptr(dbeta_k), _ptr(dalpha), _ptr(ws), ws.numel(), _stream()),
                  "norm_act_bwd")
        if sync is not None:
            tot = sync.all_reduce(torch.cat([dbeta_k.double(), dgamma_k.double()]))
            cnt = ctx.sync_count
            gam = gamma.double() if gamma is not None else torch.ones(g.c, dtype=torch.float64, device=x.device)
            a0 = (-gam * invstd.double() * tot[:g.c] / cnt).to(torch.float32).contiguous()
            b1 = (-gam * invstd.double() ** 2 * tot[g.c:] / cnt).to(torch.float32).contiguous()
            ones = torch.ones(g.c, dtype=torch.float32, device=x.device)
            corr = _new(x.shape, x)
            ga = NormGeom(g.n, g.vox, g.c, g.c, g.c, 0, ACT_NONE, 1, 0.0, 0.0, 0, g.dtype)
            check(L.mri3d_norm_act_fwd(ctypes.byref(ga), _ptr(x), _ptr(mean), _ptr(ones), _ptr(b1), _ptr(a0), None, _ptr(corr),
                                       _stream()), "norm_act_fwd")
            check(L.mri3d_add_channels(_ptr(dx), _ptr(corr), _ptr(dx), g.n * g.vox, g.c, g.c, g.c, g.c, g.dtype, _stream()),
                  "add_channels")
        return (dx, _sink_done(pg, dgamma, sg), _sink_done(pb, dbeta, sb), _sink_done(pa, dalpha, sa), None, None, None, None,
                None, None, None, None, None, None)


def norm_act(x, gamma=None, beta=None, alpha=None, running_mean=None, running_var=None, stats_mode="batch",
             momentum=0.1, eps=1e-5, act=None, slope=0.01, out=None, group_c=0):
    if momentum is None:
        raise RuntimeError("cumulative moving average (momentum=None) is not supported")
    fused = getattr(x, "_mri3d_bn_stats", None) if stats_mode == "batch" else None
    return _NormActFn.apply(x, gamma, beta, alpha, running_mean, running_var, stats_mode, momentum, eps, act, slope, out,
                            group_c, fused)


def activation(x, act, alpha=None, slope=0.01):
    return norm_act(x, None, None, alpha, None, None, "none", 0.1, 0.0, act, slope)


class _ScaleInstanceFn(torch.autograd.Function):

    @staticmethod
    def forward(ctx, x, scale):
        _require_device(x)
        _require_param(scale)
        L = _lib.lib()
        x = _cl(x)
        n, c, d, h, w = x.shape
        g = NormGeom(n, d * h * w, c, c, c, 1, ACT_NONE, 1, 0.0, 0.0, 0, _dt(x))
        scale = scale.reshape(n * c).contiguous()
        zeros = torch.zeros_like(scale)
        y = _new(x.shape, x)
        check(L.mri3d_norm_act_fwd(ctypes.byref(g), _ptr(x), _ptr(zeros), _ptr(scale), None, None, None, _ptr(y),
                                   _stream()), "norm_act_fwd")
        ctx.save_for_backward(scale, zeros)
        ctx.geom = g
        return y

    @staticmethod
    def backward(ctx, dy):
        L = _lib.lib()
        scale, zeros = ctx.saved_tensors
        g = ctx.geom
        dy = _cl(dy)
        dx = _new(dy.shape, dy)
        check(L.mri3d_norm_act_fwd(ctypes.byref(g), _ptr(dy), _ptr(zeros), _ptr(scale), None, None, None, _ptr(dx),
                                   _stream()), "norm_act_fwd")
        return dx, None


def dropout3d(x, p, training):
    if not training or p == 0.0:
        return x
    n, c = x.shape[0], x.shape[1]
    keep = torch.empty(n, c, device=x.device, dtype=torch.float32).bernoulli_(1.0 - p)
    return _ScaleInstanceFn.apply(x, keep / (1.0 - p))




def _pool_out(i, k, s, p, ceil_mode):
    if ceil_mode:
        o = -(-(i + 2 * p - k) // s) + 1
        if (o - 1) * s >= i + p:
            o -= 1
        return o
    return (i + 2 * p - k) // s + 1


class _MaxPool3dFn(torch.autograd.Function):
    @staticmethod
    def forward(ctx, x, kernel, stride, padding):
        _require_device(x)
        L = _lib.lib()
        x, x_ld = _nd(x)
        n, c, d, h, w = x.shape
        do, ho, wo = (_pool_out(i, k, s, p, False) for i, k, s, p in zip((d, h, w), kernel, stride, padding))
        if do <= 0 or ho <= 0 or wo <= 0:
            raise RuntimeError("max_pool3d: output size is too small (input %s, kernel %s)" % ((d, h, w), kernel))
        g = PoolGeom(n, d, h, w, do, ho, wo, c, *kernel, *stride, *padding, x_ld, c, _dt(x))
        y = _new((n, c, do, ho, wo), x)
        idx = torch.empty(n * do * ho * wo * c, dtype=torch.uint8, device=x.device)
        with _timed(lambda: "maxpool_fwd c%d" % c, lambda: {"flops": 0.0, "bytes": _esz(x) * x.numel() + (_esz(x) + 1) * y.numel()}):
            check(L.mri3d_maxpool3d_fwd(ctypes.byref(g), _ptr(x), _ptr(y), _ptr(idx), _stream()), "maxpool3d_fwd")
        ctx.save_for_backward(idx)
        ctx.geom = g
        ctx.xshape = tuple(x.shape)
        return y

    @staticmethod
    def backward(ctx, dy):
        L = _lib.lib()
        (idx,) = ctx.saved_tensors
        dy, dy_ld = _nd(dy)
        dx = _new(ctx.xshape, dy)
        g0 = ctx.geom
        g = PoolGeom(g0.n, g0.di, g0.hi, g0.wi, g0.dout, g0.ho, g0.wo, g0.c, g0.kd, g0.kh, g0.kw, g0.sd, g0.sh, g0.sw,
                     g0.pd, g0.ph, g0.pw, g0.c, dy_ld, _dt(dy))
        with _timed(lambda: "maxpool_bwd c%d" % g.c, lambda: {"flops": 0.0, "bytes": _esz(dy) * dx.numel() + (_esz(dy) + 1) * dy.numel()}):
            check(L.mri3d_maxpool3d_bwd(ctypes.byref(g), _ptr(dy), _ptr(idx), _ptr(dx), _stream()), "maxpool3d_bwd")
        return dx, None, None, None


class _MaxPoolSkipFn(torch.autograd.Function):

    @staticmethod
    def forward(ctx, x, kernel, stride, padding):
        y = _MaxPool3dFn.forward(ctx, x, kernel, stride, padding)
        return y, x.view_as(x)

    @staticmethod
    def backward(ctx, dy, dskip):
        if dskip is None:
            return _MaxPool3dFn.backward(ctx, dy)
        if dy is None:
            return dskip, None, None, None
        L = _lib.lib()
        (idx,) = ctx.saved_tensors
        dy, dy_ld = _nd(dy)
        dskip, ds_ld = _nd(dskip)
        if tuple(dskip.shape) != ctx.xshape or dskip.dtype != dy.dtype:
            raise RuntimeError("max_pool3d_skip backward: skip gradient %s %s does not match the input %s %s"
                               % (tuple(dskip.shape), dskip.dtype, ctx.xshape, dy.dtype))
        dx = _new(ctx.xshape, dy)
        g0 = ctx.geom
        g = PoolGeom(g0.n, g0.di, g0.hi, g0.wi, g0.dout, g0.ho, g0.wo, g0.c, g0.kd, g0.kh, g0.kw, g0.sd, g0.sh, g0.sw,
                     g0.pd, g0.ph, g0.pw, g0.c, dy_ld, _dt(dy))
        with _timed(lambda: "maxpool_bwd+skip c%d" % g.c, lambda: {"flops": 0.0, "bytes": _esz(dy) * 2 * dx.numel() + (_esz(dy) + 1) * dy.numel()}):
            check(L.mri3d_maxpool3d_bwd_add(ctypes.byref(g), _ptr(dy), _ptr(idx), _ptr(dskip), ds_ld, _ptr(dx), _stream()),
                  "maxpool3d_bwd_add")
        return dx, None, None, None


def max_pool3d_skip(x, kernel_size, stride=None, padding=0):
    k = _triple(kernel_size)
    s = _triple(stride) if stride is not None else k
    return _MaxPoolSkipFn.apply(x, k, s, _triple(padding))


def max_pool3d(x, kernel_size, stride=None, padding=0):
    k = _triple(kernel_size)
    s = _triple(stride) if stride is not None else k
    return _MaxPool3dFn.apply(x, k, s, _triple(padding))




class _Upsample3dFn(torch.autograd.Function):
    @staticmethod
    def forward(ctx, x, out_size, mode, align_corners, ratios, out):
        _require_device(x)
        L = _lib.lib()
        x, x_ld = _nd(x)
        n, c, d, h, w = x.shape
        do, ho, wo = out_size
        if out is None:
            y, y_ld = _new((n, c, do, ho, wo), x), c
        else:
            buf, y_off = out
            y_ld = _pitch_of(buf)
            if (y_ld != buf.shape[1] or tuple(buf.shape[2:]) != (do, ho, wo) or buf.shape[0] != n
                    or y_off + c > buf.shape[1] or buf.dtype != x.dtype):
                raise RuntimeError("upsample3d(out=): buffer %s cannot hold a %s slice at channel %d"
                                   % (tuple(buf.shape), (n, c, do, ho, wo), y_off))
            y = _slice_view(buf, y_off, c)
        g = UpGeom(n, d, h, w, do, ho, wo, c, x_ld, y_ld, mode, 1 if align_corners else 0, ratios[0], ratios[1], ratios[2],
                   _dt(x))
        with _timed(lambda: "upsample_fwd c%d" % c, lambda: {"flops": 0.0, "bytes": _esz(x) * (x.numel() + y.numel())}):
            check(L.mri3d_upsample3d_fwd(ctypes.byref(g), _ptr(x), _ptr(y), _stream()), "upsample3d_fwd")
        ctx.geom = g
        ctx.xshape = tuple(x.shape)
        return y

    @staticmethod
    def backward(ctx, dy):
        L = _lib.lib()
        g0 = ctx.geom
        dy, dy_ld = _nd(dy)
        dx = _new(ctx.xshape, dy)
        g = UpGeom(g0.n, g0.di, g0.hi, g0.wi, g0.dout, g0.ho, g0.wo, g0.c, g0.c, dy_ld, g0.mode, g0.align_corners, g0.rd,
                   g0.rh, g0.rw, _dt(dy))
        ws = _workspace(L.mri3d_upsample3d_workspace_bytes(ctypes.byref(g)), dy.device)
        with _timed(lambda: "upsample_bwd c%d" % g.c, lambda: {"flops": 0.0, "bytes": _esz(dy) * (dx.numel() + dy.numel())}):
            check(L.mri3d_upsample3d_bwd(ctypes.byref(g), _ptr(dy), _ptr(dx), _ptr(ws), ws.numel(), _stream()),
                  "upsample3d_bwd")
        return dx, None, None, None, None, None


def upsample3d(x, size=None, scale_factor=None, mode="nearest", align_corners=None, out=None):
    if mode == "linear":
        mode = "trilinear"
    if mode not in ("nearest", "trilinear"):
        raise NotImplementedError("upsample3d: mode %r is not supported" % (mode,))
    if mode == "nearest" and align_corners is not None:
        raise ValueError("align_corners option can only be set with the interpolating modes")
    in_sz = tuple(x.shape[2:])
    if (size is None) == (scale_factor is None):
        raise ValueError("exactly one of size or scale_factor must be given")
    if size is not None:
        out_sz = _triple(size)
        sf = None
    else:
        sf = tuple(float(s) for s in (scale_factor if isinstance(scale_factor, (tuple, list)) else (scale_factor,) * 3))
        out_sz = tuple(int(math.floor(float(i) * s)) for i, s in zip(in_sz, sf))
    ac = bool(align_corners)
    ratios = []
    for a in range(3):
        i, o = in_sz[a], out_sz[a]
        if mode == "trilinear" and ac:
            r = (i - 1) / (o - 1) if o > 1 else 0.0
        elif sf is not None:
            r = 1.0 / sf[a]
        else:
            r = i / o
        ratios.append(float(r))
    code = UP_NEAREST if mode == "nearest" else UP_TRILINEAR
    return _Upsample3dFn.apply(x, out_sz, code, ac, tuple(ratios), out)


class _UpConv3dFn(torch.autograd.Function):

    @staticmethod
    def forward(ctx, x, weight, bias, scale, padding):
        _require_device(x)
        _require_param(weight, bias)
        L = _lib.lib()
        x, x_ld = _nd(x)
        w = weight.contiguous()
        n, c, d, h, wd = x.shape
        g = _conv_geom((n, c, d * scale, h * scale, wd * scale), w.shape, (1, 1, 1), padding, (1, 1, 1), x_ld=x_ld, dtype=_dt(x))
        y = _new((g.n, g.co, g.dout, g.ho, g.wo), x)
        with _timed(lambda: _conv_tag("fwd", g) + " of nearest x%d" % scale,
                    lambda: {"flops": _conv_work(g, "fwd")["flops"], "bytes": _esz(x) * (x.numel() + y.numel())}):
            check(L.mri3d_upconv3d_fwd(ctypes.byref(g), scale, _ptr(x), _ptr(w), _ptr(bias), _ptr(y), _stream()), "upconv3d_fwd")
        ctx.save_for_backward(x, w)
        ctx.geom, ctx.scale, ctx.padding = g, scale, padding
        ctx.has_bias = bias is not None
        ctx.params = (weight, bias)
        return y

    @staticmethod
    def backward(ctx, dy):
        L = _lib.lib()
        x, w = ctx.saved_tensors
        g0, scale = ctx.geom, ctx.scale
        dy, y_ld = _nd(dy)
        fine = (g0.n, g0.ci, g0.di, g0.hi, g0.wi)
        dx = dw = db = None
        if ctx.needs_input_grad[0]:
            gd = _conv_geom(fine, w.shape, (1, 1, 1), ctx.padding, (1, 1, 1), x_ld=g0.ci, y_ld=y_ld, dtype=g0.dtype)
            dx = _new(tuple(x.shape), x)
            with _timed(lambda: _conv_tag("dgrad", gd) + " onto nearest x%d" % scale,
                        lambda: {"flops": _conv_work(gd, "dgrad")["flops"], "bytes": _esz(dy) * (dx.numel() + dy.numel())}):
                check(L.mri3d_upconv3d_dgrad(ctypes.byref(gd), scale, _ptr(dy), _ptr(w), _ptr(dx), _stream()), "upconv3d_dgrad")
        if ctx.needs_input_grad[1] or (ctx.has_bias and ctx.needs_input_grad[2]):
            gw = _conv_geom(fine, w.shape, (1, 1, 1), ctx.padding, (1, 1, 1), x_ld=g0.x_ld, y_ld=y_ld, dtype=g0.dtype)
            wp, bp = ctx.params
            want_b = ctx.has_bias and ctx.needs_input_grad[2]
            dw_out = _sink_take(wp) if ctx.needs_input_grad[1] else None
            db_out = _sink_take(bp) if want_b else None
            dw = dw_out if dw_out is not None else torch.empty_like(w, memory_format=torch.contiguous_format)
            db = (db_out if db_out is not None else torch.empty(gw.co, dtype=w.dtype, device=w.device)) if ctx.has_bias else None
            ws = _workspace(L.mri3d_upconv3d_workspace_bytes(ctypes.byref(gw), scale), x.device)
            with _timed(lambda: _conv_tag("wgrad", gw) + " of nearest x%d" % scale,
                        lambda: {"flops": _conv_work(gw, "wgrad")["flops"], "bytes": _esz(dy) * (x.numel() + dy.numel())}):
                check(L.mri3d_upconv3d_wgrad(ctypes.byref(gw), scale, _ptr(x), _ptr(dy), _ptr(dw), _ptr(db), _ptr(ws), ws.numel(),
                                             _stream()), "upconv3d_wgrad")
            dw = _sink_done(wp, dw, dw_out) if ctx.needs_input_grad[1] else None
            db = _sink_done(bp, db, db_out) if want_b else None
        return dx, dw, db, None, None


def upsample_conv3d_supported(x, weight, scale, stride=1, padding=0, dilation=1):
    if not (isinstance(scale, int) or (isinstance(scale, float) and float(scale).is_integer())):
        return False
    scale = int(scale)
    if _triple(stride) != (1, 1, 1) or _triple(dilation) != (1, 1, 1) or x.dim() != 5 or not x.is_cuda:
        return False
    if x.data_ptr() % 16:
        return False
    n, c, d, h, w = x.shape
    if weight.shape[1] != c:
        return False
    try:
        g = _conv_geom((n, c, d * scale, h * scale, w * scale), tuple(weight.shape), (1, 1, 1), _triple(padding), (1, 1, 1),
                       x_ld=_pitch_of(x) or c, dtype=_dt(x))
    except RuntimeError:
        return False
    return bool(_lib.lib().mri3d_upconv3d_supported(ctypes.byref(g), scale))

# ... 192 lines not shown
```

Baseline: 65.93 volumes/s.

## Fuse BN+PReLU backward channel reductions into producer dgrad and maxpool-backward kernels

The pointwise conv dgrad and maxpool-backward-with-skip kernels now also compute the per-block channel partial sums (sum of dy, dy*xhat, and the PReLU alpha term) that the following norm_act backward needs, writing them to a float64 partials buffer. A new norm_act_bwd_from_partials entry point reduces these partials and runs only the apply pass. This skips the separate reduction read of x and dy in norm backward. In exchange it adds float64 accumulation, a large LDS buffer in the producer kernels, and autograd plumbing that links forward norm outputs to their consumers.

```diff
diff --git a/include/mri3d.h b/include/mri3d.h
--- a/include/mri3d.h
+++ b/include/mri3d.h
@@ -116,6 +116,33 @@
 int mri3d_maxpool3d_bwd_add(const Mri3dPoolGeom* g, const void* dy, const uint8_t* idx, const void* addend,
                             int32_t addend_ld, void* dx, mri3d_stream_t stream);
 
+typedef struct Mri3dNormRed {
+    const void* x;
+    const float* mean;
+    const float* invstd;
+    const float* gamma;
+    const float* beta;
+    const float* alpha;
+    double* partials;
+    int32_t x_ld;
+    int32_t alpha_n;
+    int32_t act;
+    float slope;
+} Mri3dNormRed;
+
+int32_t mri3d_maxpool3d_bwd_add_normred_blocks(const Mri3dPoolGeom* g, const void* dy, const uint8_t* idx, const void* addend,
+                                               int32_t addend_ld, const void* dx, const Mri3dNormRed* r);
+int mri3d_maxpool3d_bwd_add_normred(const Mri3dPoolGeom* g, const void* dy, const uint8_t* idx, const void* addend,
+                                    int32_t addend_ld, void* dx, const Mri3dNormRed* r, mri3d_stream_t stream);
+int32_t mri3d_conv3d_dgrad_normred_blocks(const Mri3dConvGeom* g, const void* dy, const void* dx, const void* workspace,
+                                          const Mri3dNormRed* r);
+int mri3d_conv3d_dgrad_normred(const Mri3dConvGeom* g, const void* dy, const void* w, void* dx, void* workspace,
+                               size_t ws_bytes, const Mri3dNormRed* r, mri3d_stream_t stream);
+int mri3d_norm_act_bwd_from_partials(const Mri3dNormGeom* g, int training, const void* x, const void* dy, const double* partials,
+                                     int32_t nblk, const float* mean, const float* invstd, const float* gamma, const float* beta,
+                                     const float* alpha, void* dx, float* dgamma, float* dbeta, float* dalpha, void* workspace,
+                                     size_t ws_bytes, mri3d_stream_t stream);
+
 typedef struct Mri3dUpGeom {
     int32_t n, di, hi, wi, dout, ho, wo, c;
     int32_t x_ld, y_ld;
diff --git a/mri_epilepsy_diagnosis_amd/_lib.py b/mri_epilepsy_diagnosis_amd/_lib.py
--- a/mri_epilepsy_diagnosis_amd/_lib.py
+++ b/mri_epilepsy_diagnosis_amd/_lib.py
@@ -27,6 +27,12 @@
     _fields_ = [(n, c_int32) for n in (
         "n", "di", "hi", "wi", "dout", "ho", "wo", "c", "kd", "kh", "kw", "sd", "sh", "sw", "pd", "ph", "pw",
         "x_ld", "y_ld", "dtype")]
+
+
+class NormRed(Structure):
+    _fields_ = [("x", c_void_p), ("mean", c_void_p), ("invstd", c_void_p), ("gamma", c_void_p), ("beta", c_void_p),
+                ("alpha", c_void_p), ("partials", c_void_p), ("x_ld", c_int32), ("alpha_n", c_int32), ("act", c_int32),
+                ("slope", c_float)]
 
 
 class UpGeom(Structure):
@@ -78,6 +84,12 @@
     "mri3d_maxpool3d_fwd": (c_int32, [POINTER(PoolGeom), _P, _P, _P, _P]),
     "mri3d_maxpool3d_bwd": (c_int32, [POINTER(PoolGeom), _P, _P, _P, _P]),
     "mri3d_maxpool3d_bwd_add": (c_int32, [POINTER(PoolGeom), _P, _P, _P, c_int32, _P, _P]),
+    "mri3d_maxpool3d_bwd_add_normred_blocks": (c_int32, [POINTER(PoolGeom), _P, _P, _P, c_int32, _P, POINTER(NormRed)]),
+    "mri3d_maxpool3d_bwd_add_normred": (c_int32, [POINTER(PoolGeom), _P, _P, _P, c_int32, _P, POINTER(NormRed), _P]),
+    "mri3d_conv3d_dgrad_normred_blocks": (c_int32, [POINTER(ConvGeom), _P, _P, _P, POINTER(NormRed)]),
+    "mri3d_conv3d_dgrad_normred": (c_int32, [POINTER(ConvGeom), _P, _P, _P, _P, c_size_t, POINTER(NormRed), _P]),
+    "mri3d_norm_act_bwd_from_partials": (c_int32, [POINTER(NormGeom), c_int32, _P, _P, _P, c_int32, _FP, _FP, _FP, _FP, _FP,
+                                                   _P, _FP, _FP, _FP, _P, c_size_t, _P]),
     "mri3d_upsample3d_workspace_bytes": (c_size_t, [POINTER(UpGeom)]),
     "mri3d_upsample3d_fwd": (c_int32, [POINTER(UpGeom), _P, _P, _P]),
     "mri3d_upsample3d_bwd": (c_int32, [POINTER(UpGeom), _P, _P, _P, c_size_t, _P]),
diff --git a/mri_epilepsy_diagnosis_amd/csrc/api.hip b/mri_epilepsy_diagnosis_amd/csrc/api.hip
--- a/mri_epilepsy_diagnosis_amd/csrc/api.hip
+++ b/mri_epilepsy_diagnosis_amd/csrc/api.hip
@@ -50,6 +50,9 @@
                          hipStream_t s);
 int conv_pointwise_wgrad(const Mri3dConvGeom& g, const void* x, const void* dy, float* dw, float* dbias, void* ws,
                          size_t ws_bytes, hipStream_t s);
+int conv_pointwise_dgrad_normred_blocks(const Mri3dConvGeom& g, const void* dx, const Mri3dNormRed* r);
+int conv_pointwise_dgrad_normred(const Mri3dConvGeom& g, const void* dy, const float* w, void* dx, const Mri3dNormRed* r,
+                                 hipStream_t s);
 
 
 static int conv_check(const Mri3dConvGeom* g, const char* who, int first_ci = -1) {
@@ -129,6 +132,40 @@
     return conv_generic_dgrad(*g, dy, (const float*)w, (const float*)bias, dx, workspace, ws_bytes, s);
 }
 
+enum { kRedNone = 0, kRedPointwise = 1 };
+static int dgrad_normred_route(const Mri3dConvGeom& g, const void* dy, const void* dx, const void* workspace, const Mri3dNormRed* r,
+                               int& blocks) {
+    blocks = 0;
+    if (!dy || !dx || !r) return kRedNone;
+    if (conv_pointwise_supported(g, MRI3D_PASS_DGRAD) && aligned_vec4(g.dtype, dx)) {
+        blocks = conv_pointwise_dgrad_normred_blocks(g, dx, r);
+        return blocks > 0 ? kRedPointwise : kRedNone;
+    }
+    (void)workspace;
+    return kRedNone;
+}
+
+extern "C" int32_t mri3d_conv3d_dgrad_normred_blocks(const Mri3dConvGeom* g, const void* dy, const void* dx, const void* workspace,
+                                                     const Mri3dNormRed* r) {
+    if (!g || conv_check(g, "conv3d_dgrad_normred_blocks") != MRI3D_OK) return 0;
+    int blocks;
+    dgrad_normred_route(*g, dy, dx, workspace, r, blocks);
+    return blocks;
+}
+
+extern "C" int mri3d_conv3d_dgrad_normred(const Mri3dConvGeom* g, const void* dy, const void* w, void* dx, void* workspace,
+                                          size_t ws_bytes, const Mri3dNormRed* r, mri3d_stream_t stream) {
+    int rc = conv_check(g, "conv3d_dgrad_normred");
+    if (rc) return rc;
+    MRI3D_REQUIRE(dy && w && dx && normred_partials_ok(r), MRI3D_EINVAL, "conv3d_dgrad_normred: null pointer");
+    int blocks;
+    const int route = dgrad_normred_route(*g, dy, dx, workspace, r, blocks);
+    MRI3D_REQUIRE(route != kRedNone, MRI3D_ENOTSUP,
+                  "conv3d_dgrad_normred: geometry / alignment not served (query mri3d_conv3d_dgrad_normred_blocks)");
+    (void)ws_bytes;
+    return conv_pointwise_dgrad_normred(*g, dy, (const float*)w, dx, r, static_cast<hipStream_t>(stream));
+}
+
 extern "C" int32_t mri3d_conv3d_cat_supported(const Mri3dConvGeom* g, int32_t split, int32_t second_ld, int32_t pass) {
     if (!g || split <= 0 || conv_check(g, "conv3d_cat_supported", split) != MRI3D_OK) return 0;
     return conv_mfma_cat_supported(*g, split, second_ld, pass) ? 1 : 0;
diff --git a/mri_epilepsy_diagnosis_amd/csrc/common.h b/mri_epilepsy_diagnosis_amd/csrc/common.h
--- a/mri_epilepsy_diagnosis_amd/csrc/common.h
+++ b/mri_epilepsy_diagnosis_amd/csrc/common.h
@@ -107,4 +107,74 @@
     return v;
 }
 
+struct NormRedArgs {
+    const float* x;
+    const float *mean, *invstd, *gamma, *beta, *alpha;
+    double* part;
+    int x_ld, alpha_n, act;
+    float slope;
+};
+
+inline NormRedArgs normred_args(const Mri3dNormRed& r) {
+    return NormRedArgs{static_cast<const float*>(r.x), r.mean, r.invstd, r.gamma, r.beta, r.alpha, r.partials, r.x_ld, r.alpha_n,
+                       r.act, r.slope};
 }
+
+inline bool normred_desc_ok(const Mri3dNormRed* r, int c) {
+    return r != nullptr && r->x != nullptr && (r->mean == nullptr) == (r->invstd == nullptr) &&
+           c % 4 == 0 && r->x_ld >= c && r->x_ld % 4 == 0 && aligned16(r->x) && (reinterpret_cast<uintptr_t>(r->partials) & 7) == 0 &&
+           r->act >= MRI3D_ACT_NONE && r->act <= MRI3D_ACT_PRELU && (r->act != MRI3D_ACT_PRELU || (r->alpha != nullptr && (r->alpha_n == 1 || r->alpha_n == c)));
+}
+
+inline bool normred_partials_ok(const Mri3dNormRed* r) { return r != nullptr && r->partials != nullptr; }
+
+struct NormRedLane {
+    float mu[4], is[4], gm[4], bt[4], al[4];
+    double s0[4], s1[4], s2[4];
+    __device__ __forceinline__ void init(const NormRedArgs& r, int c0) {
+#pragma unroll
+        for (int j = 0; j < 4; ++j) {
+            const int c = c0 + j;
+            gm[j] = r.gamma ? r.gamma[c] : 1.f;
+            bt[j] = r.beta ? r.beta[c] : 0.f;
+            mu[j] = r.mean ? r.mean[c] : 0.f;
+            is[j] = r.invstd ? r.invstd[c] : 1.f;
+            al[j] = (r.act == MRI3D_ACT_PRELU) ? r.alpha[r.alpha_n == 1 ? 0 : c]
+                                               : (r.act == MRI3D_ACT_LEAKY ? r.slope : (r.act == MRI3D_ACT_RELU ? 0.f : 1.f));
+            s0[j] = 0.0;
+            s1[j] = 0.0;
+            s2[j] = 0.0;
+        }
+    }
+    __device__ __forceinline__ void add(const float4 xv, const float4 gv) {
+        const float xa[4] = {xv.x, xv.y, xv.z, xv.w}, ga[4] = {gv.x, gv.y, gv.z, gv.w};
+#pragma unroll
+        for (int j = 0; j < 4; ++j) {
+            const float xh = (xa[j] - mu[j]) * is[j];
+            const float u = fmaf(gm[j], xh, bt[j]);
+            const bool pos = u > 0.f;
+            const float du = pos ? ga[j] : ga[j] * al[j];
+            s0[j] += (double)du;
+            s1[j] = fma((double)du, (double)xh, s1[j]);
+            s2[j] += pos ? 0.0 : (double)ga[j] * (double)u;
+        }
+    }
+    __device__ __forceinline__ void block_store(double* red, double* part, int QC, int C, int blk) const {
+        const int t = threadIdx.x;
+#pragma unroll
+        for (int j = 0; j < 4; ++j) {
+            red[(t * 4 + j) * 3] = s0[j];
+            red[(t * 4 + j) * 3 + 1] = s1[j];
+            red[(t * 4 + j) * 3 + 2] = s2[j];
+        }
+        __syncthreads();
+        for (int i = t; i < C * 3; i += 256) {
+            const int c = i / 3, k = i - 3 * c, q = c >> 2, j = c & 3;
+            double v = 0.0;
+            for (int l = q; l < 256; l += QC) v += red[(l * 4 + j) * 3 + k];
+            part[((size_t)blk * C + c) * 3 + k] = v;
+        }
+    }
+};
+
+}
diff --git a/mri_epilepsy_diagnosis_amd/csrc/conv_pointwise.hip b/mri_epilepsy_diagnosis_amd/csrc/conv_pointwise.hip
--- a/mri_epilepsy_diagnosis_amd/csrc/conv_pointwise.hip
+++ b/mri_epilepsy_diagnosis_amd/csrc/conv_pointwise.hip
@@ -2,10 +2,10 @@
 
 namespace mri3d {
 
-template <typename T, int CO>
-__global__ void __launch_bounds__(256)
-pw_dgrad_kernel(const T* __restrict__ dy, const float* __restrict__ w, const float* __restrict__ bias,
-                T* __restrict__ dx, int64_t nvox, int Ci, int Co, int x_ld, int y_ld) {
+template <typename T, int CO, bool RED>
+__device__ __forceinline__ void pw_dgrad_body(const T* __restrict__ dy, const float* __restrict__ w, const float* __restrict__ bias,
+                                              T* __restrict__ dx, int64_t nvox, int Ci, int Co, int x_ld, int y_ld,
+                                              const NormRedArgs* red_args, double* red_lds) {
     const int QC = Ci >> 2;
     const int q = threadIdx.x % QC, vl = threadIdx.x / QC, VL = 256 / QC;
     float4 wq[CO];
@@ -18,13 +18,18 @@
                            : make_float4(0.f, 0.f, 0.f, 0.f);
     constexpr int U = 4;
     const int64_t stride = (int64_t)gridDim.x * VL;
+    NormRedLane red;
+    if constexpr (RED) red.init(*red_args, 4 * q);
     for (int64_t v0 = (int64_t)blockIdx.x * VL + vl; v0 < nvox; v0 += stride * U) {
         float gv[U][CO];
+        float4 red_x[RED ? U : 1];
 #pragma unroll
         for (int u = 0; u < U; ++u) {
             const int64_t v = v0 + u * stride;
 #pragma unroll
             for (int co = 0; co < CO; ++co) gv[u][co] = (v < nvox && co < Co) ? ldf(dy + v * y_ld + co) : 0.f;
+            if constexpr (RED)
+                red_x[u] = v < nvox ? ldf4(red_args->x + v * red_args->x_ld + 4 * q) : make_float4(0.f, 0.f, 0.f, 0.f);
         }
 #pragma unroll
         for (int u = 0; u < U; ++u) {
@@ -39,8 +44,25 @@
                 acc.w = fmaf(gv[u][co], wq[co].w, acc.w);
             }
             stf4(dx + v * x_ld + 4 * q, acc);
-        }
-    }
+            if constexpr (RED) red.add(red_x[u], acc);
+        }
+    }
+    if constexpr (RED) red.block_store(red_lds, red_args->part, QC, Ci, (int)blockIdx.x);
+}
+
+template <typename T, int CO>
+__global__ void __launch_bounds__(256)
+pw_dgrad_kernel(const T* __restrict__ dy, const float* __restrict__ w, const float* __restrict__ bias,
+                T* __restrict__ dx, int64_t nvox, int Ci, int Co, int x_ld, int y_ld) {
+    pw_dgrad_body<T, CO, false>(dy, w, bias, dx, nvox, Ci, Co, x_ld, y_ld, nullptr, nullptr);
+}
+
+template <int CO>
+__global__ void __launch_bounds__(256)
+pw_dgrad_normred_kernel(const float* __restrict__ dy, const float* __restrict__ w, float* __restrict__ dx, int64_t nvox, int Ci,
+                        int Co, int x_ld, int y_ld, const NormRedArgs r) {
+    __shared__ double red_lds[256 * 12];
+    pw_dgrad_body<float, CO, true>(dy, w, nullptr, dx, nvox, Ci, Co, x_ld, y_ld, &r, red_lds);
 }
 
 template <typename T, int CO>
@@ -235,6 +257,30 @@
     });
 #undef PW_DGRAD
     return check_launch("conv3d_dgrad(pointwise)");
+}
+
+int conv_pointwise_dgrad_normred_blocks(const Mri3dConvGeom& g, const void* dx, const Mri3dNormRed* r) {
+    if (g.dtype != MRI3D_F32 || !conv_pointwise_supported(g, MRI3D_PASS_DGRAD) || !aligned_vec4(g.dtype, dx) ||
+        !normred_desc_ok(r, g.ci))
+        return 0;
+    const int64_t nvox = (int64_t)g.n * g.di * g.hi * g.wi;
+    const int VL = 256 / (g.ci >> 2);
+    return (int)std::max<int64_t>(1, std::min<int64_t>(cdiv64(nvox, (int64_t)VL * 4), 2048));
+}
+
+int conv_pointwise_dgrad_normred(const Mri3dConvGeom& g, const void* dy, const float* w, void* dx, const Mri3dNormRed* r,
+                                 hipStream_t s) {
+    const int grid = conv_pointwise_dgrad_normred_blocks(g, dx, r);
+    MRI3D_REQUIRE(grid > 0, MRI3D_ENOTSUP, "conv3d_dgrad_normred(pointwise): not served (query mri3d_conv3d_dgrad_normred_blocks)");
+    const int64_t nvox = (int64_t)g.n * g.di * g.hi * g.wi;
+#define PW_DGRAD_RED(CO)                                                                                               \
+    hipLaunchKernelGGL((pw_dgrad_normred_kernel<CO>), dim3(grid), dim3(256), 0, s, (const float*)dy, w, (float*)dx, nvox, g.ci, \
+                       g.co, g.x_ld, g.y_ld, normred_args(*r))
+    if (g.co <= 2) PW_DGRAD_RED(2);
+    else if (g.co <= 4) PW_DGRAD_RED(4);
+    else PW_DGRAD_RED(8);
+#undef PW_DGRAD_RED
+    return check_launch("conv3d_dgrad_normred(pointwise)");
 }
 
 int conv_pointwise_fwd(const Mri3dConvGeom& g, const void* x, const float* w, const float* bias, void* y, hipStream_t s) {
diff --git a/mri_epilepsy_diagnosis_amd/csrc/norm.hip b/mri_epilepsy_diagnosis_amd/csrc/norm.hip
--- a/mri_epilepsy_diagnosis_amd/csrc/norm.hip
+++ b/mri_epilepsy_diagnosis_amd/csrc/norm.hip
@@ -659,3 +659,40 @@
     });
     return check_launch("norm_act_bwd");
 }
+
+extern "C" int mri3d_norm_act_bwd_from_partials(const Mri3dNormGeom* g, int training, const void* x, const void* dy,
+                                                const double* partials, int32_t nblk, const float* mean, const float* invstd,
+                                                const float* gamma, const float* beta, const float* alpha, void* dx,
+                                                float* dgamma, float* dbeta, float* dalpha, void* workspace, size_t ws_bytes,
+                                                mri3d_stream_t stream) {
+    int rc = norm_check(g, "norm_act_bwd_from_partials");
+    if (rc) return rc;
+    MRI3D_REQUIRE(x && dy && dx && partials && nblk > 0, MRI3D_EINVAL, "norm_act_bwd_from_partials: null pointer / no partials");
+    MRI3D_REQUIRE(!g->instance && g->group_c == 0, MRI3D_ENOTSUP,
+                  "norm_act_bwd_from_partials: batch statistics or none only (one group over N x voxels)");
+    MRI3D_REQUIRE((mean == nullptr) == (invstd == nullptr), MRI3D_EINVAL, "norm_act_bwd_from_partials: mean/invstd must both be set");
+    MRI3D_REQUIRE(!(training && mean == nullptr), MRI3D_EINVAL, "norm_act_bwd_from_partials: training mode needs statistics");
+    MRI3D_REQUIRE(g->act != MRI3D_ACT_PRELU || alpha, MRI3D_EINVAL, "norm_act_bwd_from_partials: PReLU needs alpha");
+    const size_t need = (size_t)g->c * 3 * sizeof(float);
+    MRI3D_REQUIRE(workspace && ws_bytes >= need && (reinterpret_cast<uintptr_t>(workspace) & 3) == 0, MRI3D_EWORKSPACE,
+                  "norm_act_bwd_from_partials: workspace %zu < %zu", ws_bytes, need);
+    hipStream_t s = static_cast<hipStream_t>(stream);
+    NormPlan p = norm_plan(*g, aligned_vec4(g->dtype, x, dy, dx));
+    dim3 grid(p.nblk, p.cy, p.groups);
+    float* sums = static_cast<float*>(workspace);
+    hipLaunchKernelGGL(norm_act_bwd_sums_kernel, dim3(cdiv(g->c, 256 / kFinQL)), dim3(256), 0, s, partials, sums, g->c, nblk, 1);
+    MRI3D_DISPATCH_DTYPE(g->dtype, T, {
+        const T* xf = static_cast<const T*>(x);
+        const T* df = static_cast<const T*>(dy);
+        T* of = static_cast<T*>(dx);
+        if (p.vec == 4)
+            hipLaunchKernelGGL((norm_act_bwd_apply_kernel<T, 4>), grid, dim3(256), 0, s, xf, df, of, sums, mean, invstd,
+                               gamma, beta, alpha, g->alpha_n, g->act, g->slope, training, g->c, g->x_ld, g->y_ld, p.gvox,
+                               p.CL, p.VT, g->group_c, dgamma, dbeta, dalpha);
+        else if (p.vec == 1)
+            hipLaunchKernelGGL((norm_act_bwd_apply_kernel<T, 1>), grid, dim3(256), 0, s, xf, df, of, sums, mean, invstd,
+                               gamma, beta, alpha, g->alpha_n, g->act, g->slope, training, g->c, g->x_ld, g->y_ld, p.gvox,
+                               p.CL, p.VT, g->group_c, dgamma, dbeta, dalpha);
+    });
+    return check_launch("norm_act_bwd_from_partials");
+}
diff --git a/mri_epilepsy_diagnosis_amd/csrc/resample.hip b/mri_epilepsy_diagnosis_amd/csrc/resample.hip
--- a/mri_epilepsy_diagnosis_amd/csrc/resample.hip
+++ b/mri_epilepsy_diagnosis_amd/csrc/resample.hip
@@ -99,10 +99,12 @@
     }
 }
 
-template <typename T, int VEC>
-__global__ void __launch_bounds__(256)
-maxpool_bwd_kernel(Mri3dPoolGeom g, const T* __restrict__ dy, const uint8_t* __restrict__ idx,
-                   T* __restrict__ dx, int hch, const T* __restrict__ addend, int a_ld) {
+template <typename T, int VEC, bool RED>
+__device__ __forceinline__ void maxpool_bwd_body(const Mri3dPoolGeom& g, const T* __restrict__ dy, const uint8_t* __restrict__ idx,
+                                                 T* __restrict__ dx, int hch, const T* __restrict__ addend, int a_ld,
+                                                 const NormRedArgs* red_args, double* red_lds) {
+    NormRedLane red;
+    if constexpr (RED) red.init(*red_args, (int)(threadIdx.x % (unsigned)(g.c / VEC)) * VEC);
     const unsigned CV = g.c / VEC;
     const int hchunks = (g.hi + hch - 1) / hch;
     const int slabs = g.n * g.di * hchunks;
@@ -120,6 +122,8 @@
             float acc[VEC];
 #pragma unroll
             for (int j = 0; j < VEC; ++j) acc[j] = 0.f;
+            float4 red_x = make_float4(0.f, 0.f, 0.f, 0.f);
+            if constexpr (RED) red_x = ldf4(red_args->x + (ibase + pix) * red_args->x_ld + cv * VEC);
             if (addend != nullptr) {
                 V<VEC> av;
                 av.load(addend + (ibase + pix) * a_ld + cv * VEC);
@@ -163,8 +167,24 @@
 #pragma unroll
             for (int j = 0; j < VEC; ++j) o.v[j] = acc[j];
             o.store(dx + (ibase + pix) * g.x_ld + cv * VEC);
-        }
-    }
+            if constexpr (RED) red.add(red_x, make_float4(acc[0], acc[1], acc[2], acc[3]));
+        }
+    }
+    if constexpr (RED) red.block_store(red_lds, red_args->part, (int)CV, g.c, (int)blockIdx.x);
+}
+
+template <typename T, int VEC>
+__global__ void __launch_bounds__(256)
+maxpool_bwd_kernel(Mri3dPoolGeom g, const T* __restrict__ dy, const uint8_t* __restrict__ idx,
+                   T* __restrict__ dx, int hch, const T* __restrict__ addend, int a_ld) {
+    maxpool_bwd_body<T, VEC, false>(g, dy, idx, dx, hch, addend, a_ld, nullptr, nullptr);
+}
+
+__global__ void __launch_bounds__(256)
+maxpool_bwd_normred_kernel(Mri3dPoolGeom g, const float* __restrict__ dy, const uint8_t* __restrict__ idx,
+                           float* __restrict__ dx, int hch, const float* __restrict__ addend, int a_ld, const NormRedArgs r) {
+    __shared__ double red_lds[256 * 12];
+    maxpool_bwd_body<float, 4, true>(g, dy, idx, dx, hch, addend, a_ld, &r, red_lds);
 }
 
 template <typename T, int VEC>
@@ -854,6 +874,41 @@
                                (const T*)addend, a_ld);
     });
     return check_launch("maxpool3d_bwd");
+}
+
+static int maxpool_bwd_normred_plan(const Mri3dPoolGeom* g, const void* dy, const uint8_t* idx, const void* addend, int32_t a_ld,
+                                    const void* dx, const Mri3dNormRed* r, int& hch) {
+    if (!g || !dy || !idx || !dx || !addend || g->dtype != MRI3D_F32 || g->c <= 0 || !normred_desc_ok(r, g->c)) return 0;
+    const int cv = g->c / 4;
+    if (cv > 256 || 256 % cv != 0) return 0;
+    const bool v4 = vec_ok(g->dtype, g->c, g->x_ld, g->y_ld, dx, dy) && (reinterpret_cast<uintptr_t>(idx) & 3) == 0 &&
+                    a_ld >= g->c && a_ld % 4 == 0 && aligned_vec4(g->dtype, addend);
+    if (!v4) return 0;
+    int grid;
+    slab_plan(g->n * g->di, g->hi, g->wi, cv, hch, grid);
+    return grid;
+}
+
+extern "C" int32_t mri3d_maxpool3d_bwd_add_normred_blocks(const Mri3dPoolGeom* g, const void* dy, const uint8_t* idx,
+                                                          const void* addend, int32_t addend_ld, const void* dx,
+                                                          const Mri3dNormRed* r) {
+    int hch;
+    if (!g || pool_check(g, "maxpool3d_bwd_add_normred_blocks") != MRI3D_OK) return 0;
+    return maxpool_bwd_normred_plan(g, dy, idx, addend, addend_ld, dx, r, hch);
+}
+
+extern "C" int mri3d_maxpool3d_bwd_add_normred(const Mri3dPoolGeom* g, const void* dy, const uint8_t* idx, const void* addend,
+                                               int32_t addend_ld, void* dx, const Mri3dNormRed* r, mri3d_stream_t stream) {
+    int rc = pool_check(g, "maxpool3d_bwd_add_normred");
+    if (rc) return rc;
+    MRI3D_REQUIRE(dy && dx && idx && addend && normred_partials_ok(r), MRI3D_EINVAL, "maxpool3d_bwd_add_normred: null pointer");
+    int hch = 0;
+    const int grid = maxpool_bwd_normred_plan(g, dy, idx, addend, addend_ld, dx, r, hch);
+    MRI3D_REQUIRE(grid > 0, MRI3D_ENOTSUP,
+                  "maxpool3d_bwd_add_normred: geometry / alignment not served (query mri3d_maxpool3d_bwd_add_normred_blocks)");
+    hipLaunchKernelGGL(maxpool_bwd_normred_kernel, dim3(grid), dim3(256), 0, static_cast<hipStream_t>(stream), *g,
+                       (const float*)dy, idx, (float*)dx, hch, (const float*)addend, addend_ld, normred_args(*r));
+    return check_launch("maxpool3d_bwd_add_normred");
 }
 
 extern "C" int mri3d_maxpool3d_bwd(const Mri3dPoolGeom* g, const void* dy, const uint8_t* idx, void* dx,
diff --git a/mri_epilepsy_diagnosis_amd/ops.py b/mri_epilepsy_diagnosis_amd/ops.py
--- a/mri_epilepsy_diagnosis_amd/ops.py
+++ b/mri_epilepsy_diagnosis_amd/ops.py
@@ -5,7 +5,7 @@
 
 from . import _lib
 from ._lib import (ACT_LEAKY, ACT_NONE, ACT_PRELU, ACT_RELU, BF16, F32, PASS_DGRAD, PASS_FWD, PASS_WGRAD, UP_NEAREST,
-                   UP_TRILINEAR, ConvGeom, DiceGeom, NormGeom, PoolGeom, UpGeom, check)
+                   UP_TRILINEAR, ConvGeom, DiceGeom, NormGeom, NormRed, PoolGeom, UpGeom, check)
 
 CL3D = torch.channels_last_3d
 
@@ -298,6 +298,48 @@
                     ci if x_ld is None else x_ld, co if y_ld is None else y_ld, dtype)
 
 
+class _NormRedHolder:
+
+    def __init__(self, x, x_ld, mean, invstd, gamma, beta, alpha, alpha_n, act, slope):
+        self.x, self.x_ld, self.mean, self.invstd, self.gamma, self.beta, self.alpha = x, x_ld, mean, invstd, gamma, beta, alpha
+        self.alpha_n, self.act, self.slope = alpha_n, act, slope
+        self.claims = 0
+        self.part = self.grad = self.key = None
+        self.nblk = 0
+
+    def claim(self):
+        self.claims += 1
+        return self
+
+    def usable(self, dy):
+        return self.claims == 1 and self.x is not None and self.part is None and dy.dtype == torch.float32 and dy.is_cuda
+
+    def desc(self, part=None):
+        return NormRed(_addr(self.x), _addr(self.mean), _addr(self.invstd), _addr(self.gamma), _addr(self.beta),
+                       _addr(self.alpha) if self.act == ACT_PRELU else None, _addr(part), self.x_ld, self.alpha_n, self.act,
+                       float(self.slope))
+
+    def fill(self, part, nblk, grad):
+        self.part, self.nblk, self.grad = part, nblk, grad
+        self.key = (grad.data_ptr(), tuple(grad.shape), tuple(grad.stride()), grad._version)
+
+    def matches(self, dy):
+        return (self.part is not None and self.claims == 1
+                and (dy.data_ptr(), tuple(dy.shape), tuple(dy.stride()), dy._version) == self.key)
+
+    def release(self):
+        self.x = self.mean = self.invstd = self.gamma = self.beta = self.alpha = self.part = self.grad = None
+
+
+def _addr(t):
+    return None if t is None else t.data_ptr()
+
+
+def _normred_tag(x):
+    h = getattr(x, "_mri3d_normred", None)
+    return h.claim() if h is not None else None
+
+
 def _conv_fwd(g, x, w, b):
     L = _lib.lib()
     y = _new((g.n, g.co, g.dout, g.ho, g.wo), x)
@@ -317,6 +359,28 @@
     with _timed(lambda: _conv_tag("dgrad", g), lambda: _conv_work(g, "dgrad")):
         check(L.mri3d_conv3d_dgrad(ctypes.byref(g), _ptr(dy), _ptr(w), _ptr(b), _ptr(dx), _ptr(ws), ws.numel(),
                                    _stream()), "conv3d_dgrad")
+    return dx
+
+
+def _conv_dgrad_normred(g, dy, w, like, red):
+    L = _lib.lib()
+    dx = _new((g.n, g.ci, g.di, g.hi, g.wi), like)
+    ws = _workspace(L.mri3d_conv3d_workspace_bytes(ctypes.byref(g), PASS_DGRAD), dy.device)
+    d0 = red.desc()
+    blocks = L.mri3d_conv3d_dgrad_normred_blocks(ctypes.byref(g), _ptr(dy), _ptr(dx), _ptr(ws), ctypes.byref(d0))
+    if blocks <= 0:
+        return None
+    part = torch.empty(blocks * g.ci * 3, dtype=torch.float64, device=dy.device)
+    d = red.desc(part)
+
+    def work():
+        wk = dict(_conv_work(g, "dgrad"))
+        wk["bytes"] = wk.get("bytes", 0.0) + 4.0 * dx.numel()
+        return wk
+    with _timed(lambda: _conv_tag("dgrad", g) + " +bn-bwd-sums", work):
+        check(L.mri3d_conv3d_dgrad_normred(ctypes.byref(g), _ptr(dy), _ptr(w), _ptr(dx), _ptr(ws), ws.numel(), ctypes.byref(d),
+                                           _stream()), "conv3d_dgrad_normred")
+    red.fill(part, blocks, dx)
     return dx
 
 
@@ -390,12 +454,13 @@
 
 class _Conv3dFn(torch.autograd.Function):
     @staticmethod
-    def forward(ctx, x, weight, bias, stride, padding, dilation, stats_holder=None):
+    def forward(ctx, x, weight, bias, stride, padding, dilation, stats_holder=None, red=None):
         _require_device(x)
         _require_param(weight, bias)
         x, x_ld = _nd(x)
         w = weight.contiguous()
         g = _conv_geom(x.shape, w.shape, stride, padding, dilation, x_ld=x_ld, dtype=_dt(x))
+        ctx.red = red
         y = None
         if stats_holder is not None:
             L = _lib.lib()
@@ -425,7 +490,11 @@
         if ctx.needs_input_grad[0]:
             gd = _conv_geom(x.shape, w.shape, (g.sd, g.sh, g.sw), (g.pd, g.ph, g.pw), (g.dd, g.dh, g.dw), y_ld=y_ld,
                             dtype=g.dtype)
-            dx = _conv_dgrad(gd, dy, w, None, x)
+            red = ctx.red
+            if red is not None and red.usable(dy):
+                dx = _conv_dgrad_normred(gd, dy, w, x, red)
+            if dx is None:
+                dx = _conv_dgrad(gd, dy, w, None, x)
         if ctx.needs_input_grad[1] or (ctx.has_bias and ctx.needs_input_grad[2]):
             gw = _conv_geom(x.shape, w.shape, (g.sd, g.sh, g.sw), (g.pd, g.ph, g.pw), (g.dd, g.dh, g.dw), x_ld=g.x_ld,
                             y_ld=y_ld, dtype=g.dtype)
@@ -441,7 +510,7 @@
             dw, db = _conv_wgrad(gw, xw, dyw, w, ctx.has_bias, dw_out, db_out)
             dw = _sink_done(wp, dw, dw_out) if ctx.needs_input_grad[1] else None
             db = _sink_done(bp, db, db_out) if want_b else None
-        return dx, dw, db, None, None, None, None
+        return dx, dw, db, None, None, None, None, None
 
 
 class _Conv3dCatFn(torch.autograd.Function):
@@ -533,7 +602,7 @@
     if _autocast_dtype is not None and x.dtype != _autocast_dtype:
         x = convert(x, _autocast_dtype)
     holder = [] if bn_stats else None
-    y = _Conv3dFn.apply(x, weight, bias, _triple(stride), _triple(padding), _triple(dilation), holder)
+    y = _Conv3dFn.apply(x, weight, bias, _triple(stride), _triple(padding), _triple(dilation), holder, _normred_tag(x))
     if holder:
         y._mri3d_bn_stats = holder[0]
     return y
@@ -693,7 +762,7 @@
 
     @staticmethod
     def forward(ctx, x, gamma, beta, alpha, running_mean, running_var, stats_mode, momentum, eps, act, slope, out, group_c=0,
-                fused_stats=None):
+                fused_stats=None, red_out=None):
         _require_device(x)
         _require_param(gamma, beta, alpha)
         ctx.params = (gamma, beta, alpha)
@@ -774,6 +843,12 @@
                   "norm_act_fwd")
         ctx.save_for_backward(x, mean, invstd, gamma, beta, alpha)
         ctx.geom = g
+        ctx.red = None
+        if red_out is not None and stats_mode in ("batch", "none") and x.dtype == torch.float32:
+            det = lambda t: None if t is None else t.detach()
+            ctx.red = _NormRedHolder(x.detach(), x_ld, mean, invstd, det(gamma), det(beta), det(alpha), alpha_n, act_code,
+                                     float(slope))
+            red_out.append(ctx.red)
         ctx.training_stats = stats_mode in ("batch", "instance", "group")
         ctx.sync = _sync_bn_reducer if stats_mode == "sync" else None
         return y
@@ -810,6 +885,21 @@
         else:
             dbeta_k, dgamma_k = dbeta, dgamma
         ws = _workspace(L.mri3d_norm_workspace_bytes(ctypes.byref(g)), x.device)
+        red = ctx.red
+        if red is not None and sync is None and red.matches(dy):
+            part, nblk = red.part, red.nblk
+            with _timed(lambda: "norm_act_bwd(sums from dy's producer) c%d vox%d n%d" % (g.c, g.vox, g.n),
+                        lambda: {"flops": 0.0, "bytes": 3 * _esz(x) * x.numel()}):
+                check(L.mri3d_norm_act_bwd_from_partials(ctypes.byref(g), 1 if ctx.training_stats else 0, _ptr(x), _ptr(dy),
+                                                         _ptr(part), nblk, _ptr(mean), _ptr(invstd), _ptr(gamma), _ptr(beta),
+                                                         _ptr(alpha) if prelu else None, _ptr(dx), _ptr(dgamma_k), _ptr(dbeta_k),
+                                                         _ptr(dalpha), _ptr(ws), ws.numel(), _stream()),
+                      "norm_act_bwd_from_partials")
+            red.release()
+            return (dx, _sink_done(pg, dgamma, sg), _sink_done(pb, dbeta, sb), _sink_done(pa, dalpha, sa), None, None, None, None,
+                    None, None, None, None, None, None, None)
+        if red is not None:
+            red.release()
         with _timed(lambda: "norm_act_bwd c%d vox%d n%d" % (g.c, g.vox, g.n), lambda: {"flops": 0.0, "bytes": 5 * _esz(x) * x.numel()}):
             check(L.mri3d_norm_act_bwd(ctypes.byref(g), 1 if ctx.training_stats else 0, _ptr(x), _ptr(dy), _ptr(mean),
                                        _ptr(invstd), _ptr(gamma), _ptr(beta), _ptr(alpha) if prelu else None, _ptr(dx),
@@ -829,7 +919,7 @@
             check(L.mri3d_add_channels(_ptr(dx), _ptr(corr), _ptr(dx), g.n * g.vox, g.c, g.c, g.c, g.c, g.dtype, _stream()),
                   "add_channels")
         return (dx, _sink_done(pg, dgamma, sg), _sink_done(pb, dbeta, sb), _sink_done(pa, dalpha, sa), None, None, None, None,
-                None, None, None, None, None, None)
+                None, None, None, None, None, None, None)
 
 
 def norm_act(x, gamma=None, beta=None, alpha=None, running_mean=None, running_var=None, stats_mode="batch",
@@ -837,8 +927,12 @@
     if momentum is None:
         raise RuntimeError("cumulative moving average (momentum=None) is not supported")
     fused = getattr(x, "_mri3d_bn_stats", None) if stats_mode == "batch" else None
-    return _NormActFn.apply(x, gamma, beta, alpha, running_mean, running_var, stats_mode, momentum, eps, act, slope, out,
-                            group_c, fused)
+    red = [] if (stats_mode in ("batch", "none") and x.is_cuda and torch.is_grad_enabled()) else None
+    y = _NormActFn.apply(x, gamma, beta, alpha, running_mean, running_var, stats_mode, momentum, eps, act, slope, out,
+                         group_c, fused, red)
+    if red:
+        y._mri3d_normred = red[0]
+    return y
 
 
 def activation(x, act, alpha=None, slope=0.01):
@@ -932,16 +1026,17 @@
 class _MaxPoolSkipFn(torch.autograd.Function):
 
     @staticmethod
-    def forward(ctx, x, kernel, stride, padding):
+    def forward(ctx, x, kernel, stride, padding, red=None):
         y = _MaxPool3dFn.forward(ctx, x, kernel, stride, padding)
+        ctx.red = red
         return y, x.view_as(x)
 
     @staticmethod
     def backward(ctx, dy, dskip):
         if dskip is None:
-            return _MaxPool3dFn.backward(ctx, dy)
+            return _MaxPool3dFn.backward(ctx, dy) + (None,)
         if dy is None:
-            return dskip, None, None, None
+            return dskip, None, None, None, None
         L = _lib.lib()
         (idx,) = ctx.saved_tensors
         dy, dy_ld = _nd(dy)
@@ -953,16 +1048,31 @@
         g0 = ctx.geom
         g = PoolGeom(g0.n, g0.di, g0.hi, g0.wi, g0.dout, g0.ho, g0.wo, g0.c, g0.kd, g0.kh, g0.kw, g0.sd, g0.sh, g0.sw,
                      g0.pd, g0.ph, g0.pw, g0.c, dy_ld, _dt(dy))
+        red = ctx.red
+        blocks = 0
+        if red is not None and red.usable(dy):
+            d0 = red.desc()
+            blocks = L.mri3d_maxpool3d_bwd_add_normred_blocks(ctypes.byref(g), _ptr(dy), _ptr(idx), _ptr(dskip), ds_ld, _ptr(dx),
+                                                              ctypes.byref(d0))
+        if blocks > 0:
+            part = torch.empty(blocks * g.c * 3, dtype=torch.float64, device=dy.device)
+            d = red.desc(part)
+            with _timed(lambda: "maxpool_bwd+skip +bn-bwd-sums c%d" % g.c,
+                        lambda: {"flops": 0.0, "bytes": _esz(dy) * 3 * dx.numel() + (_esz(dy) + 1) * dy.numel()}):
+                check(L.mri3d_maxpool3d_bwd_add_normred(ctypes.byref(g), _ptr(dy), _ptr(idx), _ptr(dskip), ds_ld, _ptr(dx),
+                                                        ctypes.byref(d), _stream()), "maxpool3d_bwd_add_normred")
+            red.fill(part, blocks, dx)
+            return dx, None, None, None, None
         with _timed(lambda: "maxpool_bwd+skip c%d" % g.c, lambda: {"flops": 0.0, "bytes": _esz(dy) * 2 * dx.numel() + (_esz(dy) + 1) * dy.numel()}):
             check(L.mri3d_maxpool3d_bwd_add(ctypes.byref(g), _ptr(dy), _ptr(idx), _ptr(dskip), ds_ld, _ptr(dx), _stream()),
                   "maxpool3d_bwd_add")
-        return dx, None, None, None
+        return dx, None, None, None, None
 
 
 def max_pool3d_skip(x, kernel_size, stride=None, padding=0):
     k = _triple(kernel_size)
     s = _triple(stride) if stride is not None else k
-    return _MaxPoolSkipFn.apply(x, k, s, _triple(padding))
+    return _MaxPoolSkipFn.apply(x, k, s, _triple(padding), _normred_tag(x))
 
 
 def max_pool3d(x, kernel_size, stride=None, padding=0):
```

Result: no change. 66.23 volumes/s, median of 6 (+0.5%).
